# Da-Tsuchi/KLab_MultiModalModel

Hardware: AMD Instinct MI355X
Metric: caption-train samples/sec (224px img, 64-tok tgt) (higher is better)
Workload: dtype bf16; 1 GPU; BASELINE configs[1]: Swin-V2(C=64,(2,2,6,2),224,w7) frozen + T5-small, fwd+bwd+Adam, T5 dropout 0.1 on, random-init weights; global_batch=64, per_gpu_batch=64, src_len=9, tgt_len=64, parallelism=dp1, hipgraph=False, optimizer=klab.optim.FusedAdam (Adam update of ref/train.py:28, one kernel)

## Files before the change

include/klab_mm.h:

```cpp
#ifndef KLAB_MM_H
#define KLAB_MM_H
#include <stddef.h>
#include <stdint.h>

#ifdef __cplusplus
extern "C" {
#endif

#define KLAB_OK 0
#define KLAB_ERR_UNSUPPORTED (-2)
#define KLAB_ERR_BADARG (-3)

#define KLAB_F32 0
#define KLAB_BF16 1
#define KLAB_FP8 2

#define KLAB_ACT_NONE 0
#define KLAB_ACT_RELU 1
#define KLAB_ACT_GELU 2

#define KLAB_AUX_NONE 0
#define KLAB_AUX_NONZERO 1
#define KLAB_AUX_DGELU 2

// ... 77 lines not shown
int klab_t5_attn_fwd(const klab_attn_args* a, void* stream);
int klab_t5_attn_bwd(const klab_attn_args* a, void* stream);
typedef struct klab_attn_fused_args {
  const float* x; const float* gamma; float eps; int d_model;
  const void* w;
  void* xn; float* rstd;
  void* proj; long ldproj;
  int cross;
  klab_attn_args attn;
} klab_attn_fused_args;
int klab_t5_attn_fused_fwd(const klab_attn_fused_args* a, void* stream);
typedef struct klab_attn_bwd_fused_args {
  const void* dy; long lddy;
  const void* w;
  int d_model;
  klab_attn_args attn;
} klab_attn_bwd_fused_args;
int klab_t5_attn_bwd_fused(const klab_attn_bwd_fused_args* a, void* stream);
int klab_dbias_reduce(const void* ds_ws, int dtype, float* dbias, int nbatch, int H, int Lq, int Lk, void* stream);

typedef struct klab_swin_attn_args {
  int dtype;
  const void* qkv; void* ctx; const float* bias; const float* logit_scale; float* lse;
  int B, R, w, shift, H, C;
  const void* dctx; void* dqkv; float* dbias; float* dlogit_scale;
  void* bwd_ws; size_t bwd_ws_bytes;
  const float* bias_table; float* dbias_table;
  const float* v_bias; float* dv_bias;
} klab_swin_attn_args;
int klab_swin_attn_fwd(const klab_swin_attn_args* a, void* stream);
size_t klab_swin_attn_bwd_ws_bytes(int dtype, int B, int R, int w, int H, int C);
int klab_swin_qkv_attn_fused(const void* x, const void* wqkv, const float* bqkv, void* ctx, const float* bias, const float* logit_scale,
                             int dtype, int B, int R, int w, int shift, int H, int C, void* stream);
size_t klab_swin_bias_image_bytes(int w, int shift, int H);
int klab_swin_bias_image(const float* bias, float* image, int R, int w, int shift, int H, void* stream);
int klab_swin_qkv_attn_fused_img(const void* x, const void* wqkv, const float* bqkv, void* ctx, const float* image, const float* logit_scale,
                                 int dtype, int B, int R, int w, int shift, int H, int C, void* stream);
int klab_swin_attn_bwd(const klab_swin_attn_args* a, void* stream);
int klab_swin_cpb_bias(const float* coords, const int* index, const float* w0, const float* b0, const float* w2,
                       float* table, float* hidden, float* bias, int ntab, int n, int heads, int nhidden, void* stream);
int klab_swin_cpb_table(const float* coords, const float* w0, const float* b0, const float* w2, float* table, float* hidden,
                        float* bias_table, int ntab, int heads, int nhidden, void* stream);
int klab_swin_cpb_table_bwd(const float* dbias_table, const float* bias_table, const float* coords, const float* hidden, const float* w2,
                            float* dtable, float* dw0, float* db0, float* dw2, int ntab, int heads, int nhidden, void* stream);

typedef struct klab_image_desc { long long offset; int height, width; } klab_image_desc;
size_t klab_image_preprocess_ws_bytes(int n_images, int max_h, int mid);
int klab_image_preprocess(const unsigned char* src, const klab_image_desc* desc_dev, int n_images, int max_h, int max_w, int mid,
                          int out_size, int filter_a, int filter_b, double rescale, const float* mean3, const float* std3,
                          float* pixel_values, void* ws, size_t ws_bytes, void* stream);
#define KLAB_IMAGE_FLIP_LR 1
typedef struct klab_image_crop_desc { long long offset; int height, width, pitch, flags; } klab_image_crop_desc;
int klab_image_preprocess_crop(const unsigned char* src, const klab_image_crop_desc* desc_dev, int n_images, int max_crop_h,
                               int max_crop_w, int mid, int out_size, int filter_a, int filter_b, double rescale, const float* mean3,
                               const float* std3, float* pixel_values, void* ws, size_t ws_bytes, void* stream);

#define KLAB_JPEG_GRAY 0
#define KLAB_JPEG_YCC 1
#define KLAB_JPEG_RGB 2
typedef struct klab_jpeg_info {
  int width, height, ncomp, precision, progressive, supported, colour;
  int hmax, vmax, mcus_x, mcus_y;
  int hs[3], vs[3], bw[3], bh[3], tq[3];
  long long coef_blocks;
} klab_jpeg_info;
typedef struct klab_jpeg_item { klab_jpeg_info info; long long coef_block0; long long rgb_off; } klab_jpeg_item;
int klab_jpeg_read_info(const unsigned char* data, size_t n, klab_jpeg_info* info);
int klab_jpeg_entropy_decode(const unsigned char* data, size_t n, short* coefs, unsigned short* qt, klab_jpeg_info* info);
int klab_jpeg_entropy_decode_batch(const unsigned char* const* data, const size_t* sizes, int n, short* const* coefs,
                                   unsigned short* qt, klab_jpeg_info* infos, int* rcs, int n_threads);
size_t klab_jpeg_decode_ws_bytes(const klab_jpeg_item* items, int n);
int klab_jpeg_decode_device(const short* coefs_dev, const unsigned short* qt_dev, const klab_jpeg_item* items,
                            const klab_jpeg_item* items_dev, int n, unsigned char* rgb_dev, void* ws, size_t ws_bytes, void* stream);

int klab_cast_pack(const void* desc_dev, int ndesc, long total4, void* dst, int dtype, void* stream);
int klab_embed_fwd(const long long* ids, int shift_right, int L, int start_id, int pad_id, const float* table, int vocab,
                   float* out, int rows, int d, float drop_p, const uint32_t* seed_dev, uint32_t tag, int* err_flag,
                   void* stream);
int klab_embed_bwd(const long long* ids, int shift_right, int L, int start_id, int pad_id, const float* dh, float* dtable,
                   int vocab, int rows, int d, float drop_p, const uint32_t* seed_dev, uint32_t tag, void* stream);
int klab_relbias_fwd(const float* table, const int* bucket, float* bias, int heads, int Lq, int Lk, void* stream);
int klab_relbias_bwd(const float* dbias, const int* bucket, float* dtable, int heads, int Lq, int Lk, int nbuckets,
                     void* stream);
int klab_ce_count(const long long* labels, int rows, float* inv_n, void* stream);
int klab_ce_fwd(void* logits, long ld, int dtype, const long long* labels, int rows, int V, float* inv_n, float* loss_row,
                float* loss, int write_grad, void* stream);
int klab_ce_wsum(const long long* labels, const float* weights, int rows, float* inv_w, void* stream);
int klab_ce_fwd_opts(void* logits, long ld, int dtype, const long long* labels, const float* weights, int rows, int V, float eps, float z,
                     float* inv_w, float* loss_row, float* loss, int write_grad, void* stream);
int klab_im2col_patch(const float* pixels, void* out, int dtype, int B, int Cin, int Himg, int P, void* stream);
int klab_im2col_patch_ld(const float* pixels, void* out, int dtype, int B, int Cin, int Himg, int P, int ldo, void* stream);
int klab_merge_gather(const float* x, void* out, int dtype, int B, int R, int C, void* stream);
int klab_merge_scatter(const float* dmerged, float* dx, int B, int R, int C, void* stream);
int klab_colsum(const void* dy, long ld, int dtype, int M, int N, float* out, void* stream);
int klab_convert(const float* x, void* y, int dtype, long n, float scale, void* stream);
int klab_add_f32(float* y, const float* x, long n, void* stream);

int klab_gelu_fwd(const void* x, void* y, int dtype, long n, void* stream);
int klab_geglu_fwd(const void* ab, long ldab, void* h, long ldh, int dtype, int M, int F, float drop_p, const uint32_t* seed_dev,
                   uint32_t drop_tag, void* stream);
int klab_geglu_bwd(const void* dh, long lddh, const void* ab, long ldab, void* dab, long lddab, int dtype, int M, int F, float drop_p,
                   const uint32_t* seed_dev, uint32_t drop_tag, void* stream);
int klab_swin_proj_ln_fused(const void* x, const float* shortcut, const void* w, const float* b, const float* gamma, const float* beta,
                            float* out, void* outt, int dtype, int M, int C, float eps, void* stream);
int klab_swin_mlp_fused(const void* x, const float* shortcut, const void* w1, const float* b1, const void* w2, const float* b2,
                        const float* gamma, const float* beta, float* out, void* outt, int dtype, int M, int C, float eps,
                        void* stream);
int klab_swin_patch_embed_fused(const float* pixels, const void* w, int ldw, const float* bias, const float* gamma, const float* beta,
                                float* out, void* outt, int dtype, int B, int in_ch, int image_size, int patch, int C, float eps, void* stream);
int klab_swin_linear_ln_fused(const void* x, const float* shortcut, const void* w, const float* bias, const float* gamma,
                              const float* beta, float* out, void* outt, int dtype, int M, int K, int C, float eps, void* stream);
int klab_swin_cpb_bias_bwd(const float* dbias, const float* bias, const int* index, const float* coords, const float* hidden,
                           const float* w0, const float* w2, float* dtable, float* dw0, float* db0, float* dw2, int ntab, int n,
                           int heads, int nhidden, void* stream);
int klab_swin_cpb_bias_bwd_pz(const float* dbias, const float* bias, const int* index, const float* coords, const float* hidden,
                              const float* w0, const float* w2, float* dtable, float* dw0, float* db0, float* dw2, int ntab, int n,
                              int heads, int nhidden, int dtable_zeroed, void* stream);

typedef struct klab_swin_cfg {
  int image_size, patch, in_ch, embed_dim, n_stages;
  int depths[8], heads[8];
  int window;
  int pretrained_window[8];
  int mlp_ratio, qkv_bias;
  float ln_eps;
} klab_swin_cfg;
typedef struct klab_t5_cfg {
  int vocab, d_model, d_kv, n_heads, d_ff, n_layers, n_dec_layers, rel_buckets, rel_max_dist;
  float dropout, ln_eps;
  int start_id, pad_id, scale_decoder_outputs;
  int ffn_gated;
  int tie_lm_head;
} klab_t5_cfg;
typedef struct klab_model_cfg {
  klab_swin_cfg swin;
  klab_t5_cfg lang, main;
  int dtype;
  int train_swin;
} klab_model_cfg;
typedef struct klab_engine klab_engine;

int klab_sizeof_t5_cfg(void);
int klab_sizeof_model_cfg(void);
int klab_sizeof_sample_args(void);
int klab_sizeof_logits_proc_args(void);
int klab_sizeof_gen_cfg(void);
klab_engine* klab_engine_create(const klab_model_cfg* cfg);
void klab_engine_destroy(klab_engine* e);
int klab_engine_num_params(const klab_engine* e, int model);
int klab_engine_param_info(const klab_engine* e, int model, int i, char* name, int name_cap, long* shape4, int* ndim,
                           long* grad_off );
long klab_engine_grad_elems(const klab_engine* e, int model);
int klab_engine_num_buckets(const klab_engine* e, int segment);
int klab_engine_bucket(const klab_engine* e, int segment, int i, long* off, long* len);
int klab_engine_bucket_wait(klab_engine* e, int segment, int i, void* stream);
int klab_engine_set_bucket_events(klab_engine* e, int on);
int klab_engine_segment(const klab_engine* e, int seg, int* model, long* off, long* len);
int klab_engine_set_captions(klab_engine* e, int n);
size_t klab_engine_workspace_bytes(klab_engine* e, int B, int Ls, int Lt);
size_t klab_engine_workspace_bytes_n(klab_engine* e, int B, int Ls, int Lt, int n);
int klab_engine_bind(klab_engine* e, int B, int Ls, int Lt, void* workspace, size_t ws_bytes, const void* const* swin_params,
                     const void* const* lang_params, const void* const* main_params, float* main_grads, float* swin_grads,
                     const int* lang_bucket, const int* enc_bucket, const int* dec_bucket, const void* const* swin_coords,
                     const void* const* swin_index, void* stream);
int klab_engine_forward(klab_engine* e, const float* pixels, const long long* src_ids, const long long* tgt_ids, int training,
                        uint32_t seed, int want_grad, void* stream);
int klab_engine_set_graph(klab_engine* e, int on);
int klab_engine_get_rng(klab_engine* e, uint32_t* base, uint32_t* counter, void* stream);
int klab_engine_set_rng(klab_engine* e, uint32_t base, uint32_t counter, void* stream);
int klab_engine_adam_step(klab_engine* e, float* m, float* v, float lr, float beta1, float beta2, float eps, float weight_decay,
                          float bias_corr1, float bias_corr2, void* stream);
int klab_adam_step(const void* desc_dev, int ndesc, long total4, const float* grads, float* m, float* v, void* arena, int dtype, float lr,
// ... 149 lines not shown
```

klab_multimodalmodel_amd/_lib.py:

```python
import ctypes as C
import os

HERE = os.path.dirname(os.path.abspath(__file__))
LIB_PATH = os.environ.get("KLAB_LIB", os.path.join(HERE, "libklab_mm.so"))

F32, BF16, FP8 = 0, 1, 2
ACT_NONE, ACT_RELU, ACT_GELU = 0, 1, 2
AUX_NONE, AUX_NONZERO, AUX_DGELU = 0, 1, 2
ERR_UNSUPPORTED, ERR_BADARG = -2, -3

vp, i32, i64, f32, u32 = C.c_void_p, C.c_int, C.c_long, C.c_float, C.c_uint32


class GemmArgs(C.Structure):
    _fields_ = [("M", i32), ("N", i32), ("K", i32), ("dtype", i32),
                ("A", vp), ("lda", i64), ("a_kmajor", i32),
                ("B", vp), ("ldb", i64), ("b_kmajor", i32),
                ("C", vp), ("ldc", i64), ("c_dtype", i32), ("accumulate", i32),
                ("alpha", f32), ("alpha_dev", vp), ("bias", vp), ("act", i32),
                ("aux", vp), ("ldaux", i64), ("aux_mode", i32), ("aux_scale", f32),
                ("residual", vp), ("ldr", i64), ("r_dtype", i32),
                ("drop_p", f32), ("seed_dev", vp), ("drop_tag", u32), ("name_tag", i32), ("atomic_ok", i32)]


# ... 80 lines not shown
GEN_PICK, GEN_SAMPLE, GEN_BEAM, GEN_FORCE = 0, 1, 2, 3


class GenCfg(C.Structure):
    _fields_ = [("mode", i32), ("n", i32), ("max_length", i32), ("eos_id", i32), ("pad_id", i32),
                ("temperature", f32), ("top_k", i32), ("top_p", f32), ("seed", C.c_uint64),
                ("length_penalty", f32), ("early_stopping", i32), ("procs", C.POINTER(LogitsProcCfg)), ("want_logprobs", i32)]


SIGNATURES = {
    "klab_version": [],
    "klab_gemm": [C.POINTER(GemmArgs), vp],
    "klab_gemm_probe_enable": [i32],
    "klab_gemm_probe_read": [vp, vp, vp],
    "klab_rmsnorm_fwd": [vp, vp, vp, i32, vp, vp, i32, i32, f32, i32, i32, i32, f32, vp, u32, vp],
    "klab_rmsnorm_bwd": [vp, vp, vp, vp, vp, vp, vp, i32, vp, i32, i32, i32, i32, i32, f32, u32, f32, u32, vp, vp],
    "klab_rmsnorm_bwd_part": [vp, vp, vp, vp, vp, vp, vp, i32, vp, i32, i32, i32, i32, i32, f32, u32, f32, u32, vp, vp],
    "klab_rmsnorm_part_rows": [i32],
    "klab_colpart_reduce": [vp, i64, i32, i32, vp, i32, vp],
    "klab_adam_step": [vp, i32, i64, vp, vp, vp, vp, i32, f32, f32, f32, f32, f32, f32, f32, vp],
    "klab_adam_step_range": [vp, i32, i64, i64, vp, vp, vp, vp, i32, f32, f32, f32, f32, f32, f32, f32, vp],
    "klab_adamw_step_range": [vp, i32, vp, C.POINTER(AdamWGroup), i32, i64, i64, vp, vp, vp, vp, i32, vp],
    "klab_ema_update_range": [vp, i32, i64, i64, vp, f32, vp],
    "klab_ema_swap_range": [vp, i32, i64, i64, vp, vp, i32, vp],
    "klab_adafactor_plan": [i32, vp, vp, vp, vp, vp],
    "klab_adafactor_step": [vp, i32, i64, i64, vp, vp, vp, vp, vp, vp, i32, f32, f32, f32, f32, f32, f32, f32, f32, f32, i32, vp],
    "klab_grad_norm_chunk": [],
    "klab_grad_norm": [vp, i32, i32, vp, i64, vp, vp],
    "klab_grad_clip": [vp, i32, vp, f32, vp, vp],
    "klab_layernorm_fwd": [vp, i32, vp, vp, vp, vp, vp, i32, vp, vp, i32, i32, f32, i32, i32, i32, f32, vp, u32, vp],
    "klab_layernorm_bwd": [vp, vp, i32, vp, vp, vp, vp, vp, vp, i32, i32, i32, i32, i32, f32, vp, u32, vp],
    "klab_rmsnorm_fwd_q8": [vp, vp, vp, vp, vp, vp, i32, i32, f32, f32, vp, u32, vp],
    "klab_layernorm_fwd_q8": [vp, vp, vp, vp, vp, vp, vp, vp, vp, vp, i32, i32, f32, vp],
    "klab_gelu_fwd": [vp, vp, i32, i64, vp],
    "klab_gelu_fwd_q8": [vp, vp, vp, vp, i32, i32, vp],
    "klab_geglu_fwd": [vp, i64, vp, i64, i32, i32, i32, f32, vp, u32, vp],
    "klab_geglu_bwd": [vp, i64, vp, i64, vp, i64, i32, i32, i32, f32, vp, u32, vp],
    "klab_layernorm_bwd_bias": [vp, vp, i32, vp, vp, vp, vp, vp, vp, vp, i32, i32, i32, i32, i32, f32, vp, u32, vp],
    "klab_t5_attn_fwd": [C.POINTER(AttnArgs), vp],
    "klab_t5_attn_bwd": [C.POINTER(AttnArgs), vp],
    "klab_t5_attn_fused_fwd": [C.POINTER(AttnFusedArgs), vp],
    "klab_t5_attn_bwd_fused": [C.POINTER(AttnBwdFusedArgs), vp],
    "klab_t5_beam_decode_attn": [i32, vp, i64, vp, vp, i64, i64, i32, vp, i64, vp, i64, vp, i64, i32, i32, i32, i32, vp],
    "klab_t5_decode_attn_map": [i32, vp, i64, i32, vp, i64, i64, i32, vp, i64, vp, vp, i64, i32, i32, i32, i32, vp],
    "klab_beam_topk": [i32, vp, i64, i32, vp, i32, i32, i32, vp, vp, vp, vp, vp],
    "klab_beam_update": [C.POINTER(BeamUpdateArgs), i32, vp],
    "klab_beam_init": [C.POINTER(BeamUpdateArgs), i32, i32, vp],
    "klab_beam_copy_rows": [i32, vp, i64, i32, vp, i64, i32, i32, vp],
    "klab_sample_rows": [C.POINTER(SampleArgs), vp],
    "klab_logits_process_rows": [C.POINTER(LogitsProcArgs), vp],
    "klab_gen_finalize": [vp, i64, vp, i64, i32, i32, i32, i32, f32, i32, vp, vp, vp, vp],
    "klab_sizeof_sample_args": [],
    "klab_sizeof_logits_proc_args": [],
    "klab_sizeof_gen_cfg": [],
    "klab_force_rows": [C.POINTER(ForceArgs), vp],
    "klab_sizeof_force_args": [],
    "klab_beam_topk_scores": [vp, i64, i32, vp, i32, i32, i32, vp, vp, vp, vp, vp],
    "klab_dbias_reduce": [vp, i32, vp, i32, i32, i32, i32, vp],
    "klab_swin_mlp_fused": [vp, vp, vp, vp, vp, vp, vp, vp, vp, vp, i32, i32, i32, f32, vp],
    "klab_gemm_grouped": [vp, i32, vp],
    "klab_gemm_grouped_tiles": [vp, i32, i32, vp],
    "klab_gemm_fp8": [C.POINTER(GemmArgs), vp, vp, i64, vp],
    "klab_quant_fp8_rows": [vp, i64, i32, i32, vp, i64, vp, vp],
    "klab_quant_fp8_arena": [vp, i32, i64, vp, vp, vp, vp],
    "klab_swin_qkv_attn_fused": [vp, vp, vp, vp, vp, vp, i32, i32, i32, i32, i32, i32, i32, vp],
    "klab_swin_bias_image_bytes": [i32, i32, i32],
    "klab_swin_bias_image": [vp, vp, i32, i32, i32, i32, vp],
    "klab_swin_qkv_attn_fused_img": [vp, vp, vp, vp, vp, vp, i32, i32, i32, i32, i32, i32, i32, vp],
    "klab_swin_linear_ln_fused": [vp, vp, vp, vp, vp, vp, vp, vp, i32, i32, i32, i32, f32, vp],
    "klab_swin_patch_embed_fused": [vp, vp, i32, vp, vp, vp, vp, vp, i32, i32, i32, i32, i32, i32, f32, vp],
    "klab_swin_proj_ln_fused": [vp, vp, vp, vp, vp, vp, vp, vp, i32, i32, i32, f32, vp],
    "klab_swin_attn_fwd": [C.POINTER(SwinAttnArgs), vp],
    "klab_swin_attn_bwd": [C.POINTER(SwinAttnArgs), vp],
    "klab_swin_attn_bwd_ws_bytes": [i32, i32, i32, i32, i32, i32],
    "klab_swin_cpb_bias": [vp, vp, vp, vp, vp, vp, vp, vp, i32, i32, i32, i32, vp],
    "klab_swin_cpb_table": [vp, vp, vp, vp, vp, vp, vp, i32, i32, i32, vp],
    "klab_swin_cpb_table_bwd": [vp, vp, vp, vp, vp, vp, vp, vp, vp, i32, i32, i32, vp],
    "klab_swin_cpb_bias_bwd_pz": [vp, vp, vp, vp, vp, vp, vp, vp, vp, vp, vp, i32, i32, i32, i32, i32, vp],
    "klab_cast_pack": [vp, i32, i64, vp, i32, vp],
    "klab_embed_fwd": [vp, i32, i32, i32, i32, vp, i32, vp, i32, i32, f32, vp, u32, vp, vp],
    "klab_embed_bwd": [vp, i32, i32, i32, i32, vp, vp, i32, i32, i32, f32, vp, u32, vp],
    "klab_relbias_fwd": [vp, vp, vp, i32, i32, i32, vp],
    "klab_relbias_bwd": [vp, vp, vp, i32, i32, i32, i32, vp],
    "klab_ce_fwd": [vp, i64, i32, vp, i32, i32, vp, vp, vp, i32, vp],
    "klab_ce_count": [vp, i32, vp, vp],
    "klab_ce_wsum": [vp, vp, i32, vp, vp],
    "klab_ce_fwd_opts": [vp, i64, i32, vp, vp, i32, i32, f32, f32, vp, vp, vp, i32, vp],
    "klab_engine_set_loss_options": [vp, f32, f32, vp],
    "klab_engine_set_captions": [vp, i32],
    "klab_im2col_patch": [vp, vp, i32, i32, i32, i32, i32, vp],
    "klab_im2col_patch_ld": [vp, vp, i32, i32, i32, i32, i32, i32, vp],
    "klab_merge_gather": [vp, vp, i32, i32, i32, i32, vp],
    "klab_merge_scatter": [vp, vp, i32, i32, i32, vp],
    "klab_colsum": [vp, i64, i32, i32, i32, vp, vp],
    "klab_convert": [vp, vp, i32, i64, f32, vp],
    "klab_add_f32": [vp, vp, i64, vp],
    "klab_image_preprocess_ws_bytes": [i32, i32, i32],
    "klab_segv_trace_install": [i32],
    "klab_segv_set_context": [C.c_char_p],
    "klab_image_preprocess": [vp, vp, i32, i32, i32, i32, i32, i32, i32, C.c_double, vp, vp, vp, vp, C.c_size_t, vp],
    "klab_image_preprocess_crop": [vp, vp, i32, i32, i32, i32, i32, i32, i32, C.c_double, vp, vp, vp, vp, C.c_size_t, vp],
    "klab_jpeg_read_info": [vp, C.c_size_t, vp],
    "klab_jpeg_entropy_decode": [vp, C.c_size_t, vp, vp, vp],
    "klab_jpeg_entropy_decode_batch": [vp, vp, i32, vp, vp, vp, vp, i32],
    "klab_jpeg_decode_ws_bytes": [vp, i32],
    "klab_jpeg_decode_device": [vp, vp, vp, vp, i32, vp, vp, C.c_size_t, vp],
}


class JpegInfo(C.Structure):
    _fields_ = [("width", i32), ("height", i32), ("ncomp", i32), ("precision", i32), ("progressive", i32), ("supported", i32),
                ("colour", i32), ("hmax", i32), ("vmax", i32), ("mcus_x", i32), ("mcus_y", i32), ("hs", i32 * 3), ("vs", i32 * 3),
                ("bw", i32 * 3), ("bh", i32 * 3), ("tq", i32 * 3), ("coef_blocks", C.c_longlong)]


class JpegItem(C.Structure):
    _fields_ = [("info", JpegInfo), ("coef_block0", C.c_longlong), ("rgb_off", C.c_longlong)]

_lib = None


class KlabError(RuntimeError):
    pass


def load():
    global _lib
    if _lib is not None:
        return _lib
    if not os.path.exists(LIB_PATH):
        raise KlabError(f"{LIB_PATH} is missing: run `python -m klab_multimodalmodel_amd.build` "
                        "(hipcc --offload-arch=gfx950). There is no CPU fallback.")
    import torch
    lib = C.CDLL(LIB_PATH)
    for name, argt in SIGNATURES.items():
        fn = getattr(lib, name)
        fn.argtypes = argt
        fn.restype = C.c_size_t if name.endswith("_bytes") else i32
    _lib = lib
    return lib


def check(rc, what=""):
    if rc == 0:
        return
    if rc == ERR_UNSUPPORTED:
        raise NotImplementedError(f"klab: unsupported shape/alignment in {what}")
    if rc == ERR_BADARG:
        raise ValueError(f"klab: bad argument to {what}")
    raise KlabError(f"klab: {what} failed with hipError {rc}")


def ptr(t):
    return None if t is None else t.data_ptr()


def dtype_code(torch_dtype):
    import torch
    if torch_dtype == torch.float32:
        return F32
    if torch_dtype == torch.bfloat16:
        return BF16
    if torch_dtype == "fp8":
        return FP8
    raise ValueError(f"unsupported dtype {torch_dtype}")


def stream_ptr():
    import torch
    return torch.cuda.current_stream().cuda_stream
# ... 1 lines not shown
```

klab_multimodalmodel_amd/csrc/ce_opts.hip:

```cpp
#include <math.h>

#include "common.h"
#include "klab_mm.h"

namespace klab {
namespace {

struct CeOpts {
  float ome;
  float epsv;
  float z;
};

__global__ __launch_bounds__(256) void ce_wsum_kernel(const long long* __restrict__ labels, const float* __restrict__ weights, int rows,
                                                      float* __restrict__ inv_w) {
  __shared__ float red[4];
  float a = 0.f;
  for (int i = threadIdx.x; i < rows; i += 256) a += labels[i] != -100 ? (weights ? weights[i] : 1.f) : 0.f;
  a = wave_sum(a);
  if ((threadIdx.x & 63) == 0) red[threadIdx.x >> 6] = a;
  __syncthreads();
  if (threadIdx.x == 0) {
    const float W = red[0] + red[1] + red[2] + red[3];
    inv_w[0] = W > 0.f ? 1.f / W : 0.f;
  }
}

__device__ __forceinline__ float row_loss(float lse, float xlab, float sx, const CeOpts& o) {
  float l = lse - o.ome * xlab;
  l -= o.epsv * sx;
  l += (o.z * lse) * lse;
  return l;
}

struct GradCoef {
  float gk, ge, k, g;
};
__device__ __forceinline__ GradCoef grad_coef(float lse, float g, const CeOpts& o) {
  const float k = 1.f + 2.f * (o.z * lse);
  return GradCoef{g * k, g * o.epsv, k, g};
}
__device__ __forceinline__ float grad_at_label(float pr, const GradCoef& q, const CeOpts& o) {
  float t = pr * q.k - o.ome;
  t -= o.epsv;
  return t * q.g;
}

template <typename T, bool SX>
__global__ __launch_bounds__(256) void ce_opts_kernel(T* __restrict__ logits, long ld, const long long* __restrict__ labels,
                                                      const float* __restrict__ weights, int V, CeOpts o, const float* __restrict__ inv_w,
                                                      float* __restrict__ loss_row, int write_grad) {
  constexpr int VEC = Vec16<T>::N;
  using VT = typename Vec16<T>::type;
  __shared__ float red[12];
  const long row = blockIdx.x;
  const int tid = threadIdx.x;
  T* x = logits + row * ld;
  const long long lab = labels[row];
  const bool valid = lab != -100;
  const float g = write_grad && valid ? (weights ? weights[row] : 1.f) * inv_w[0] : 0.f;
  float m = -INFINITY, s = 0.f, sx = 0.f;
  for (int c = tid * VEC; c < V; c += 256 * VEC) {
    VT v = *reinterpret_cast<const VT*>(x + c);
    float mx = to_f32(v[0]);
#pragma unroll
    for (int u = 1; u < VEC; ++u) mx = fmaxf(mx, to_f32(v[u]));
    const float mn = fmaxf(m, mx);
    float a = 0.f;
#pragma unroll
    for (int u = 0; u < VEC; ++u) {
      a += __expf(to_f32(v[u]) - mn);
      if constexpr (SX) sx += to_f32(v[u]);
    }
    s = s * __expf(m - mn) + a;
    m = mn;
  }
  float wm = wave_max(m);
  float ws = wave_sum(m == -INFINITY ? 0.f : s * __expf(m - wm));
  const float wx = SX ? wave_sum(sx) : 0.f;
  if ((tid & 63) == 0) { red[tid >> 6] = wm; red[4 + (tid >> 6)] = ws; red[8 + (tid >> 6)] = wx; }
  __syncthreads();
  const float bm = fmaxf(fmaxf(red[0], red[1]), fmaxf(red[2], red[3]));
  float bs = 0.f;
#pragma unroll
  for (int w = 0; w < 4; ++w) bs += red[w] == -INFINITY ? 0.f : red[4 + w] * __expf(red[w] - bm);
  const float lse = bm + __logf(bs);
  const float bsx = red[8] + red[9] + red[10] + red[11];
  if (tid == 0) loss_row[row] = valid ? row_loss(lse, to_f32(x[lab]), bsx, o) : 0.f;
  if (!write_grad) return;
  __syncthreads();
  const GradCoef q = grad_coef(lse, g, o);
  const int labi = (int)lab;
  for (int c = tid * VEC; c < V; c += 256 * VEC) {
    VT v = *reinterpret_cast<const VT*>(x + c);
    VT out;
#pragma unroll
    for (int u = 0; u < VEC; ++u) out[u] = from_f32<T>(__expf(to_f32(v[u]) - lse) * q.gk - q.ge);
    const unsigned at = (unsigned)(labi - c);
    if (at < (unsigned)VEC) {
#pragma unroll
      for (int u = 0; u < VEC; ++u)
        if (u == (int)at) out[u] = from_f32<T>(grad_at_label(__expf(to_f32(v[u]) - lse), q, o));
    }
    *reinterpret_cast<VT*>(x + c) = out;
  }
}

template <typename T, int NIT, bool SX>
__global__ __launch_bounds__(256) void ce_opts_onepass_kernel(T* __restrict__ logits, long ld, const long long* __restrict__ labels,
                                                              const float* __restrict__ weights, int V, CeOpts o,
                                                              const float* __restrict__ inv_w, float* __restrict__ loss_row, int write_grad) {
  constexpr int VEC = Vec16<T>::N;
  using VT = typename Vec16<T>::type;
  __shared__ float red[12];
  __shared__ float xlab;
  const long row = blockIdx.x;
  const int tid = threadIdx.x;
  T* x = logits + row * ld;
  const long long lab = labels[row];
  const int labi = (int)lab;
  const bool valid = lab != -100;
  VT v[NIT];
#pragma unroll
  for (int it = 0; it < NIT; ++it) {
    const int c = (it * 256 + tid) * VEC;
    if (c < V) v[it] = *reinterpret_cast<const VT*>(x + c);
  }
  const float g = write_grad && valid ? (weights ? weights[row] : 1.f) * inv_w[0] : 0.f;
  float m = -INFINITY;
#pragma unroll
  for (int it = 0; it < NIT; ++it) {
    const int c = (it * 256 + tid) * VEC;
    if (c < V) {
#pragma unroll
      for (int u = 0; u < VEC; ++u) m = fmaxf(m, to_f32(v[it][u]));
    }
  }
  const float wm = wave_max(m);
  if ((tid & 63) == 0) red[tid >> 6] = wm;
  __syncthreads();
  const float bm = fmaxf(fmaxf(red[0], red[1]), fmaxf(red[2], red[3]));
  float sum = 0.f, sx = 0.f;
#pragma unroll
  for (int it = 0; it < NIT; ++it) {
    const int c = (it * 256 + tid) * VEC;
    if (c < V) {
#pragma unroll
      for (int u = 0; u < VEC; ++u) {
        const float xv = to_f32(v[it][u]);
        sum += __expf(xv - bm);
        if constexpr (SX) sx += xv;
      }
      const unsigned at = (unsigned)(labi - c);
      if (at < (unsigned)VEC) {
#pragma unroll
        for (int u = 0; u < VEC; ++u)
          if (u == (int)at) xlab = to_f32(v[it][u]);
      }
    }
  }
  const float ws = wave_sum(sum);
  const float wx = SX ? wave_sum(sx) : 0.f;
  if ((tid & 63) == 0) { red[4 + (tid >> 6)] = ws; red[8 + (tid >> 6)] = wx; }
  __syncthreads();
  const float lse = bm + __logf(red[4] + red[5] + red[6] + red[7]);
  const float bsx = red[8] + red[9] + red[10] + red[11];
  if (tid == 0) loss_row[row] = valid ? row_loss(lse, xlab, bsx, o) : 0.f;
  if (!write_grad) return;
  const GradCoef q = grad_coef(lse, g, o);
#pragma unroll
  for (int it = 0; it < NIT; ++it) {
    const int c = (it * 256 + tid) * VEC;
    if (c < V) {
      VT out;
#pragma unroll
      for (int u = 0; u < VEC; ++u) out[u] = from_f32<T>(__expf(to_f32(v[it][u]) - lse) * q.gk - q.ge);
      const unsigned at = (unsigned)(labi - c);
      if (at < (unsigned)VEC) {
#pragma unroll
        for (int u = 0; u < VEC; ++u)
          if (u == (int)at) out[u] = from_f32<T>(grad_at_label(__expf(to_f32(v[it][u]) - lse), q, o));
      }
      *reinterpret_cast<VT*>(x + c) = out;
    }
  }
}

__global__ __launch_bounds__(256) void ce_wreduce_kernel(const float* __restrict__ loss_row, const float* __restrict__ weights, int rows,
                                                         const float* __restrict__ inv_w, float* __restrict__ loss) {
  __shared__ float red[4];
  float a = 0.f;
  for (int i = threadIdx.x; i < rows; i += 256) a += weights ? weights[i] * loss_row[i] : loss_row[i];
  a = wave_sum(a);
  if ((threadIdx.x & 63) == 0) red[threadIdx.x >> 6] = a;
  __syncthreads();
  if (threadIdx.x == 0) loss[0] = (red[0] + red[1] + red[2] + red[3]) * inv_w[0];
}

template <bool SX>
void launch_rows(void* logits, long ld, int dtype, const long long* labels, const float* weights, int rows, int V, const CeOpts& o,
                 const float* inv_w, float* loss_row, int write_grad, hipStream_t s) {
  if (dtype == KLAB_BF16 && V <= 256 * 8 * 16 && V > 256 * 8 * 8)
    hipLaunchKernelGGL((ce_opts_onepass_kernel<bf16_t, 16, SX>), dim3(rows), dim3(256), 0, s, (bf16_t*)logits, ld, labels, weights, V, o, inv_w, loss_row, write_grad);
  else if (dtype == KLAB_BF16 && V <= 256 * 8 * 8)
    hipLaunchKernelGGL((ce_opts_onepass_kernel<bf16_t, 8, SX>), dim3(rows), dim3(256), 0, s, (bf16_t*)logits, ld, labels, weights, V, o, inv_w, loss_row, write_grad);
  else if (dtype == KLAB_BF16)
    hipLaunchKernelGGL((ce_opts_kernel<bf16_t, SX>), dim3(rows), dim3(256), 0, s, (bf16_t*)logits, ld, labels, weights, V, o, inv_w, loss_row, write_grad);
  else
    hipLaunchKernelGGL((ce_opts_kernel<float, SX>), dim3(rows), dim3(256), 0, s, (float*)logits, ld, labels, weights, V, o, inv_w, loss_row, write_grad);
}

}
}

using namespace klab;

extern "C" int klab_ce_wsum(const long long* labels, const float* weights, int rows, float* inv_w, void* stream) {
  if (!labels || !inv_w || rows <= 0) return KLAB_ERR_BADARG;
  hipLaunchKernelGGL(ce_wsum_kernel, dim3(1), dim3(256), 0, (hipStream_t)stream, labels, weights, rows, inv_w);
  KLAB_LAUNCH_CHECK();
  return KLAB_OK;
}

extern "C" int klab_ce_fwd_opts(void* logits, long ld, int dtype, const long long* labels, const float* weights, int rows, int V, float eps,
                                float z, float* inv_w, float* loss_row, float* loss, int write_grad, void* stream) {
  if (!logits || !labels || !inv_w || !loss_row || !loss || rows <= 0 || V <= 0) return KLAB_ERR_BADARG;
  if (!(eps >= 0.f && eps < 1.f) || !(z >= 0.f) || !isfinite(z)) return KLAB_ERR_BADARG;
  const int vec = dtype == KLAB_BF16 ? 8 : 4;
  if (V % vec || ld % vec) return KLAB_ERR_UNSUPPORTED;
  hipStream_t s = (hipStream_t)stream;
  if (!(write_grad & 2)) {
    hipLaunchKernelGGL(ce_wsum_kernel, dim3(1), dim3(256), 0, s, labels, weights, rows, inv_w);
    KLAB_LAUNCH_CHECK();
  }
  write_grad &= 1;
  const CeOpts o{1.f - eps, eps / (float)V, z};
  if (eps != 0.f) launch_rows<true>(logits, ld, dtype, labels, weights, rows, V, o, inv_w, loss_row, write_grad, s);
  else launch_rows<false>(logits, ld, dtype, labels, weights, rows, V, o, inv_w, loss_row, write_grad, s);
  KLAB_LAUNCH_CHECK();
  hipLaunchKernelGGL(ce_wreduce_kernel, dim3(1), dim3(256), 0, s, loss_row, weights, rows, inv_w, loss);
  KLAB_LAUNCH_CHECK();
  return KLAB_OK;
}
```

klab_multimodalmodel_amd/csrc/common.h:

```cpp
#pragma once
#include <hip/hip_runtime.h>
#include <stdint.h>
#include <stdlib.h>

#define KLAB_OK 0
#define KLAB_ERR_UNSUPPORTED (-2)
#define KLAB_ERR_BADARG (-3)

#define KLAB_F32 0
#define KLAB_BF16 1

typedef __bf16 bf16_t;
typedef __attribute__((ext_vector_type(8))) __bf16 bf16x8;
typedef __attribute__((ext_vector_type(4))) __bf16 bf16x4;
typedef __attribute__((ext_vector_type(4))) float f32x4;

#define KLAB_LAUNCH_CHECK()                          \
  do {                                               \
    hipError_t e__ = hipGetLastError();              \
    if (e__ != hipSuccess) return (int)e__;          \
  } while (0)

namespace klab {

inline bool env_on(const char* name) {
  const char* v = getenv(name);
  return !v || atoi(v) != 0;
}

int ensure_dyn_lds(const void* kernel, size_t bytes);

constexpr int ZERO_RANGES_MAX = 16;
int zero_ranges(float* const* ptrs, const long* counts, int n, hipStream_t s);

template <typename T> struct TypeTag;
template <> struct TypeTag<float> { static constexpr int id = KLAB_F32; };
template <> struct TypeTag<bf16_t> { static constexpr int id = KLAB_BF16; };

__device__ __forceinline__ float to_f32(float x) { return x; }
__device__ __forceinline__ float to_f32(bf16_t x) { return (float)x; }
template <typename T> __device__ __forceinline__ T from_f32(float x);
template <> __device__ __forceinline__ float from_f32<float>(float x) { return x; }
template <> __device__ __forceinline__ bf16_t from_f32<bf16_t>(float x) { return (bf16_t)x; }

__device__ __forceinline__ uint32_t mix32(uint32_t x) {
  x ^= x >> 16; x *= 0x85EBCA6Bu; x ^= x >> 13; x *= 0xC2B2AE35u; x ^= x >> 16;
  return x;
}
struct DropCtx {
  uint32_t key;
  uint32_t thresh;
  float scale;
  bool on;
};
__device__ __forceinline__ DropCtx make_drop(const uint32_t* seed_dev, uint32_t tag, float p) {
  DropCtx d;
  d.on = (p > 0.f) && (seed_dev != nullptr);
  d.key = 0; d.thresh = 0; d.scale = 1.f;
  if (d.on) {
    d.key = mix32(seed_dev[0] * 0x9E3779B1u + tag * 0x7FEB352Du + 0x165667B1u);
    double t = (double)p * 4294967296.0;
    d.thresh = t >= 4294967295.0 ? 0xFFFFFFFFu : (uint32_t)t;
    d.scale = 1.f / (1.f - p);
  }
  return d;
}
__device__ __forceinline__ float drop_mult(const DropCtx& d, uint64_t idx) {
  if (!d.on) return 1.f;
  uint32_t h = mix32((uint32_t)idx * 0x9E3779B1u + d.key);
  const uint32_t hi = (uint32_t)(idx >> 32);
  if (hi) h = mix32(h ^ (hi * 0x85EBCA77u + 0x27D4EB2Fu));
  return h < d.thresh ? 0.f : d.scale;
}
__device__ __forceinline__ DropCtx drop_slab(DropCtx d, uint32_t slab) {
  if (d.on) d.key = mix32(d.key ^ (slab * 0x85EBCA77u + 0x27D4EB2Fu));
  return d;
}
__device__ __forceinline__ float drop_mult32(const DropCtx& d, uint32_t off) {
  if (!d.on) return 1.f;
  return mix32(off * 0x9E3779B1u + d.key) < d.thresh ? 0.f : d.scale;
}
__device__ __forceinline__ float drop_mult32_nb(const DropCtx& d, uint32_t off) {
  return mix32(off * 0x9E3779B1u + d.key) < d.thresh ? 0.f : d.scale;
}

__device__ __forceinline__ float wave_sum(float v) {
#pragma unroll
  for (int o = 32; o > 0; o >>= 1) v += __shfl_xor(v, o, 64);
  return v;
}
__device__ __forceinline__ float wave_max(float v) {
#pragma unroll
  for (int o = 32; o > 0; o >>= 1) v = fmaxf(v, __shfl_xor(v, o, 64));
  return v;
}
template <int G> __device__ __forceinline__ float group_sum(float v) {
#pragma unroll
  for (int o = G / 2; o > 0; o >>= 1) v += __shfl_xor(v, o, 64);
  return v;
}
template <int G> __device__ __forceinline__ float group_max(float v) {
#pragma unroll
  for (int o = G / 2; o > 0; o >>= 1) v = fmaxf(v, __shfl_xor(v, o, 64));
  return v;
}

__device__ __forceinline__ float gelu_erf(float x) { return 0.5f * x * (1.f + erff(x * 0.70710678118654752440f)); }
__device__ __forceinline__ float erf_fast(float x) {
  const float ax = fabsf(x);
  const float t = __frcp_rn(fmaf(0.3275911f, ax, 1.f));
  float pl = fmaf(1.061405429f, t, -1.453152027f);
  pl = fmaf(pl, t, 1.421413741f);
  pl = fmaf(pl, t, -0.284496736f);
  pl = fmaf(pl, t, 0.254829592f);
  const float y = 1.f - pl * t * __expf(-ax * ax);
  return copysignf(y, x);
}
typedef __attribute__((ext_vector_type(2))) float f32x2;
template <typename V> __device__ __forceinline__ V gelu_poly(V x) {
  V s = x * x;
  s = __builtin_elementwise_min(s, V(20.48f));
  V q = V(7.318504830e-11f);
  q = q * s + V(-7.769299870e-09f);
  q = q * s + V(3.614930506e-07f);
  q = q * s + V(-9.785327165e-06f);
  q = q * s + V(1.732400560e-04f);
  q = q * s + V(-2.146258019e-03f);
  q = q * s + V(1.943818480e-02f);
  q = q * s + V(-1.324543953e-01f);
  q = q * s + V(7.977233529e-01f);
  V e = __builtin_elementwise_max(__builtin_elementwise_min(x * q, V(1.f)), V(-1.f));
  const V hx = x * V(0.5f);
  return hx * e + hx;
}
template <typename T> __device__ __forceinline__ float gelu_for(float x) {
  if constexpr (sizeof(T) == 2) return gelu_poly<float>(x);
  else return gelu_erf(x);
}
__device__ __forceinline__ float gelu_erf_grad(float x) {
  float cdf = 0.5f * (1.f + erff(x * 0.70710678118654752440f));
  float pdf = 0.39894228040143267794f * __expf(-0.5f * x * x);
  return cdf + x * pdf;
}

template <typename T> struct Vec16;
template <> struct Vec16<float> { typedef f32x4 type; static constexpr int N = 4; };
template <> struct Vec16<bf16_t> { typedef bf16x8 type; static constexpr int N = 8; };

}
```

klab_multimodalmodel_amd/csrc/engine.cpp:

```cpp
#include <hip/hip_runtime.h>
#include <math.h>
#include <stdio.h>
#include <string.h>

#include <algorithm>
#include <string>
#include <utility>
#include <vector>

#include "gemm_shared.h"
#include "klab_mm.h"

namespace {

#define RC(x)                 \
  do {                        \
    int rc__ = (x);           \
    if (rc__ != 0) return rc__; \
  } while (0)

struct ParamInfo {
  std::string name;
  std::vector<long> shape;
  long numel = 0;
// ... 51 lines not shown
};
struct ForcedTable {
  const long long* tok = nullptr;
  long ld = 0;
  int n = 0;
};
struct AttnMaps {
  float* p = nullptr;
  size_t bytes = 0;
};
struct GenRun {
  klab_gen_cfg cfg{};
  ProcSet lp;
  ForcedTable forced;
  AttnMaps maps;
  int cur = 0;
};

}

struct klab_engine {
  klab_model_cfg cfg;
  std::vector<ParamInfo> P[3];
  SwinIdx si; T5Idx li, mi;
  long grad_elems[3] = {0, 0, 0};
  long seg_zero_off[3] = {0, 0, 0}, seg_zero_len[3] = {0, 0, 0};
  long seg_off[3] = {0, 0, 0}, seg_len[3] = {0, 0, 0};
  long warena_elems = 0, farena_elems = 0;
  long kvall_w_off = -1, kvall_g_off = -1;
  struct Bucket { long off, len; };
  std::vector<Bucket> buckets[3];
  std::vector<hipEvent_t> bucket_ev[3];
  bool bucket_ev_live[3] = {false, false, false};
  bool bucket_events_on = false;
  int pe_k0 = 0, pe_kp = 0;
  bool bound = false;
  int B = 0, Ls = 0, Lt = 0, Le = 0, Nimg = 0;
  int ncap_next = 1, ncap = 1, Bd = 0;
  size_t es = 4;
  std::vector<const float*> W[3];
  float* G[3] = {nullptr, nullptr, nullptr};
  void* warena = nullptr; float* farena = nullptr;
  bool fp8 = false;
  void* w8 = nullptr; float* wscale = nullptr; void* qdesc = nullptr; int n_qdesc = 0; long q_rows = 0;
  void* x8 = nullptr; float* xscale = nullptr; long x8_bytes = 0, xscale_rows = 0;
  void* x8s = nullptr; float* xscales = nullptr; long x8s_bytes = 0, xscales_rows = 0;
  const void* q8_src[2] = {nullptr, nullptr}; int q8_rows[2] = {0, 0}, q8_k[2] = {0, 0};
  void* cast_desc = nullptr; int n_cast = 0; long cast_total4 = 0;
  void* adam_desc = nullptr; int n_adam = 0; long adam_total4 = 0, adam_split4 = 0;
  std::vector<long> adam_ptrs; int n_adam_seg0 = 0;
  void* af_desc = nullptr; int n_af = 0; long af_totals[4] = {0, 0, 0, 0};
  float* rms_part = nullptr; long rms_part_stride = 0; float** rms_dst_dev[2] = {nullptr, nullptr}; int rms_ncalls[2] = {0, 0};
  void* cast_desc_frozen = nullptr; int n_cast_frozen = 0; long cast_total4_frozen = 0;
  bool frozen_valid = false;
  void* fcast_desc = nullptr; int n_fcast = 0; long fcast_total4 = 0;
  uint32_t* seed_dev = nullptr; int* err_dev = nullptr;
  const int *enc_bucket = nullptr, *dec_bucket = nullptr, *lang_bucket = nullptr;
  std::vector<const float*> swin_coords; std::vector<const int*> swin_index; std::vector<int> swin_ntab;
  T5StackBufs lang, enc, dec;
  GenRun gen;
  ForcedTable forced_armed;
  AttnMaps attn_armed;
  void* kv_all = nullptr; void* dkv_all = nullptr;
  void* logits = nullptr; float *loss_row = nullptr, *inv_n = nullptr, *loss = nullptr;
  float *dh_a = nullptr, *dh_b = nullptr, *dxn = nullptr, *denc = nullptr;
  void *dctx = nullptr, *ds_ws = nullptr;
  void* dh_ff = nullptr;
  std::vector<void*> dy_pool, dhmid_pool, dqkv_pool, dqc_pool;
  std::vector<hipEvent_t> evpool; int ev_next = 0;
  void *cols = nullptr, *pe_out = nullptr; float *pe_mean = nullptr, *pe_rstd = nullptr; float* x0 = nullptr; void* x0t = nullptr;
  std::vector<SwinStageBufs> sw;
  float *sw_fmean = nullptr, *sw_frstd = nullptr;
  float *sdh_a = nullptr, *sdh_b = nullptr, *sdm = nullptr; void *sdy = nullptr, *sdctx = nullptr, *sdqkv = nullptr, *sda = nullptr;
  void* sattn_ws = nullptr; size_t sattn_ws_bytes = 0;
  float *sdbias = nullptr, *sdtable = nullptr, *sdbtab = nullptr;
  long sdb_stride = 0, sdt_stride = 0; size_t sdz_bytes = 0;
  void *sdyA[2] = {nullptr, nullptr}, *sdyB[2] = {nullptr, nullptr}, *sdaP[2] = {nullptr, nullptr}, *sdqkvP[2] = {nullptr, nullptr};
  hipEvent_t swin_done_ev[2] = {nullptr, nullptr};
  hipStream_t side = nullptr; hipEvent_t ev_fork = nullptr, ev_join = nullptr;
  hipEvent_t ev_zero = nullptr;
  bool seg1_zeroed = false;
  bool dbias_zeroed[2] = {false, false};
  bool denc_in_dxn = false;
  float* loss_out = nullptr;
  float loss_eps = 0.f, loss_z = 0.f;
  const float* loss_w_armed = nullptr;
  float *loss_w_buf = nullptr, *inv_w = nullptr;
  bool bias_ready[3] = {false, false, false};
  bool dec_embed_ready = false;
  bool inv_n_ready = false;
  bool kv_wgrad_done = false;
  struct WritePlan {
    bool valid = false, graph = false, kv = false;
    bool head_store = false, any_store = false;
    std::vector<char> store[2];
    std::vector<std::pair<long, long>> stored;
    std::vector<std::pair<long, long>> clear[2];
  } wplan;
  hipStream_t own = nullptr; hipEvent_t ev_in = nullptr, ev_out = nullptr;
  bool use_graph = false;
  struct GraphSlot { hipGraphExec_t exec = nullptr; int uses = 0; bool failed = false; } gs[7];
  float* pixels_buf = nullptr; long long *src_buf = nullptr, *tgt_buf = nullptr; float* dloss_buf = nullptr;
  const float* pixels_cur = nullptr;
  uint32_t seed_base = 0; bool seed_set = false;
  bool probe_on = false;
  struct Probe { std::vector<hipEvent_t> a, b; std::vector<double> flops; int n = 0; } probe[2];
  float p_train = 0.f;
  const long long* last_tgt = nullptr;
};

namespace {

int add_param(std::vector<ParamInfo>& v, const std::string& name, std::vector<long> shape) {
  ParamInfo p;
  p.name = name; p.shape = shape; p.numel = 1;
  for (long s : shape) p.numel *= s;
  v.push_back(p);
  return (int)v.size() - 1;
}

void build_t5_params(const klab_t5_cfg& c, bool encoder_only, std::vector<ParamInfo>& v, T5Idx& ix) {
  const long d = c.d_model, inner = (long)c.n_heads * c.d_kv, ff = c.d_ff;
  ix.shared = add_param(v, "shared.weight", {c.vocab, d});
  ix.lm_head = (!encoder_only && !c.tie_lm_head) ? add_param(v, "lm_head.weight", {c.vocab, d}) : -1;
  ix.head = ix.lm_head >= 0 ? ix.lm_head : ix.shared;
  auto stack = [&](const char* pre, int nl, bool dec, std::vector<T5LayerIdx>& L, int& fin) {
    for (int i = 0; i < nl; ++i) {
      T5LayerIdx l;
      memset(&l, -1, sizeof(l));
      std::string bp = std::string(pre) + "block." + std::to_string(i) + ".";
      std::string ap = bp + "layer.0.SelfAttention.";
      l.q = add_param(v, ap + "q.weight", {inner, d});
      l.k = add_param(v, ap + "k.weight", {inner, d});
      l.v = add_param(v, ap + "v.weight", {inner, d});
      l.o = add_param(v, ap + "o.weight", {d, inner});
      if (i == 0) l.relb = add_param(v, ap + "relative_attention_bias.weight", {c.rel_buckets, c.n_heads});
      l.ln0 = add_param(v, bp + "layer.0.layer_norm.weight", {d});
      int li = 1;
      if (dec) {
        std::string cp = bp + "layer.1.EncDecAttention.";
        l.cq = add_param(v, cp + "q.weight", {inner, d});
        l.ck = add_param(v, cp + "k.weight", {inner, d});
        l.cv = add_param(v, cp + "v.weight", {inner, d});
        l.co = add_param(v, cp + "o.weight", {d, inner});
        l.ln1 = add_param(v, bp + "layer.1.layer_norm.weight", {d});
        li = 2;
      }
      std::string fp = bp + "layer." + std::to_string(li) + ".";
      if (c.ffn_gated) {
        l.wi = add_param(v, fp + "DenseReluDense.wi_0.weight", {ff, d});
        l.wi1 = add_param(v, fp + "DenseReluDense.wi_1.weight", {ff, d});
      } else {
        l.wi = add_param(v, fp + "DenseReluDense.wi.weight", {ff, d});
      }
      l.wo = add_param(v, fp + "DenseReluDense.wo.weight", {d, ff});
      l.ln2 = add_param(v, fp + "layer_norm.weight", {d});
      L.push_back(l);
    }
    fin = add_param(v, std::string(pre) + "final_layer_norm.weight", {d});
  };
  if (!encoder_only) stack("decoder.", c.n_dec_layers, true, ix.dec, ix.dec_final);
  stack("encoder.", c.n_layers, false, ix.enc, ix.enc_final);
}

void build_swin_params(const klab_swin_cfg& c, std::vector<ParamInfo>& v, SwinIdx& ix) {
  const long C0 = c.embed_dim;
// ... 732 lines not shown
        g.aux = b.hmid; g.ldaux = ff; g.aux_mode = KLAB_AUX_NONZERO; g.aux_scale = inv_keep;
        RC(klab_gemm(&g, c.ws()));
      }
      RC(wq.push(dhmid, ff, b.xn3, d, M, ff, d, G(l.wi), st));
      RC(linear_dgrad(c, dhmid, ff, M, ff, P[l.wi].warena_off, d, e->dxn, KLAB_F32));
    }
    {
      const uint32_t tprev = dec ? tag_of(stack_id, i, SITE_XOUT) : tag_of(stack_id, i, SITE_ATTN_OUT);
      dy = next_dy();
      RC(rms_bwd(e->dxn, s.h[j], W[l.ln2], b.rstd3, dh_cur, dh_oth, dy, l.ln2, 0.f, 0, p, tprev));
      float* t = dh_cur; dh_cur = dh_oth; dh_oth = t;
    }
    if (dec) {
      --j;
      void* dqc = e->dqc_pool[i];
      RC(wq.push(dy, d, b.ctx2, inner, M, d, inner, G(l.co), st));
      dctx_ready = false;
      klab_attn_args a;
      memset(&a, 0, sizeof(a));
      a.dtype = c.dt; a.q = b.qc; a.ldq = inner;
      a.k = eoff(c, (void*)kv_all, (long)i * 2 * inner); a.ldk = kv_ld;
      a.v = eoff(c, (void*)kv_all, (long)i * 2 * inner + inner); a.ldv = kv_ld;
      a.ctx = b.ctx2; a.ldo = inner; a.lse = b.lse2; a.B = B / qgrp; a.H = H; a.Lq = qgrp * Lq; a.Lk = Lkv; a.dk = dk;
      a.drop_p = p; a.seed_dev = e->seed_dev; a.drop_tag = tag_of(stack_id, i, SITE_XPROB);
      a.dctx = e->dctx; a.lddo = inner; a.dq = dqc; a.lddq = inner;
      a.dk_out = eoff(c, dkv_all, (long)i * 2 * inner); a.lddk = kv_ld;
      a.dv = eoff(c, dkv_all, (long)i * 2 * inner + inner); a.lddv = kv_ld;
      RC(attn_bwd(a, P[l.co].warena_off, qgrp == 1));
      if (kv_in_queue) {
        RC(wq.push(eoff(c, dkv_all, (long)i * 2 * inner), kv_ld, e->enc.out_t, d, (B / qgrp) * Lkv, 2 * inner, d, Gflat + e->kvall_g_off + (long)i * 2 * inner * d, st));
        e->kv_wgrad_done = true;
      }
      RC(wq.push(dqc, inner, b.xn2, d, M, inner, d, G(l.cq), st));
      RC(linear_dgrad(c, dqc, inner, M, inner, P[l.cq].warena_off, d, e->dxn, KLAB_F32));
      dy = next_dy();
      RC(rms_bwd(e->dxn, s.h[j], W[l.ln1], b.rstd2, dh_cur, dh_oth, dy, l.ln1, 0.f, 0, p, tag_of(stack_id, i, SITE_ATTN_OUT)));
      float* t = dh_cur; dh_cur = dh_oth; dh_oth = t;
    }
    --j;
    RC(wq.push(dy, d, b.ctx, inner, M, d, inner, G(l.o), st));
    dctx_ready = false;
    {
      klab_attn_args a;
      memset(&a, 0, sizeof(a));
      a.dtype = c.dt; a.q = b.qkv; a.ldq = 3 * inner; a.k = eoff(c, b.qkv, inner); a.ldk = 3 * inner;
      a.v = eoff(c, b.qkv, 2 * inner); a.ldv = 3 * inner; a.bias = s.bias; a.causal = dec ? 1 : 0;
      a.ctx = b.ctx; a.ldo = inner; a.lse = b.lse; a.B = B; a.H = H; a.Lq = Lq; a.Lk = Lq; a.dk = dk;
      a.drop_p = p; a.seed_dev = e->seed_dev; a.drop_tag = tag_of(stack_id, i, SITE_PROB);
      a.dctx = e->dctx; a.lddo = inner; a.dq = dqkv; a.lddq = 3 * inner;
      a.dk_out = eoff(c, dqkv, inner); a.lddk = 3 * inner; a.dv = eoff(c, dqkv, 2 * inner); a.lddv = 3 * inner;
      a.dbias = s.dbias;
      int arc = KLAB_ERR_UNSUPPORTED;
      if (c.dt == KLAB_BF16 && deferred == (int)L.size() - 1 - i) {
        a.ds_defer = 1;
        a.ds_ws = (char*)e->ds_ws + (size_t)deferred * B * H * Lq * ((Lq + 31) & ~31) * c.es;
        arc = attn_bwd(a, P[l.o].warena_off);
        if (arc == 0) ++deferred;
      }
      if (arc == KLAB_ERR_UNSUPPORTED) { a.ds_defer = 0; a.ds_ws = nullptr; arc = attn_bwd(a, P[l.o].warena_off); }
      RC(arc);
    }
    RC(wq.push(dqkv, 3 * inner, b.xn1, d, M, 3 * inner, d, G(l.q), st));
    RC(linear_dgrad(c, dqkv, 3 * inner, M, 3 * inner, P[l.q].warena_off, d, e->dxn, KLAB_F32));
    {
      const bool first = (i == 0);
      if (!first) dy = next_dy();
      RC(rms_bwd(e->dxn, s.h[j], W[l.ln0], b.rstd1, dh_cur, dh_oth, first ? nullptr : dy, l.ln0, 0.f, 0, first ? 0.f : p,
                 first ? 0u : tag_of(stack_id, i - 1, SITE_FFN_OUT)));
      float* t = dh_cur; dh_cur = dh_oth; dh_oth = t;
    }
    bool launched = false;
    RC(wq.flush(c, flush_at[i] != 0, &launched));
    pending_buckets.push_back((int)L.size() - 1 - i);
    if (launched) {
      const int seg = dec ? 0 : 1;
      for (int bi : pending_buckets)
        if (e->bucket_events_on && Gflat == e->G[2] && !e->use_graph && bi < (int)e->bucket_ev[seg].size())
          RC((int)hipEventRecord(e->bucket_ev[seg][bi], e->side));
      pending_buckets.clear();
      if (i == 0 && e->bucket_events_on && Gflat == e->G[2] && !e->use_graph && (int)L.size() - 1 < (int)e->bucket_ev[seg].size())
        e->bucket_ev_live[seg] = true;
    }
  }
  if (part_ok && rms_calls) {
    if (rms_calls != e->rms_ncalls[stk]) return KLAB_ERR_BADARG;
    RC(klab_colpart_reduce(e->rms_part, e->rms_part_stride, klab_rmsnorm_part_rows(M), d, e->rms_dst_dev[stk], rms_calls, c.ws()));
  }
  if (deferred) RC(klab_dbias_reduce(e->ds_ws, c.dt, s.dbias, deferred * B, H, Lq, Lq, c.ws()));
  RC(klab_relbias_bwd(s.dbias, s.bucket, G(L[0].relb), H, Lq, Lq, cfg.rel_buckets, c.ws()));
  *dh_out = dh_cur;
  return 0;
}

int swin_forward(const Ctx& c, const float* pixels, float p_in, bool refresh_bias) {
  klab_engine* e = c.e;
  const klab_swin_cfg& s = e->cfg.swin;
  const auto& P = e->P[0];
  const auto& W = e->W[0];
  const int B = e->B, R0 = s.image_size / s.patch, K0 = s.in_ch * s.patch * s.patch, C0 = s.embed_dim;
  const long M0 = (long)B * R0 * R0;
  const int Kp = e->pe_kp;
  (void)K0;
  static const bool fused_pe = klab::env_on("KLAB_SWIN_FUSED_EMBED");
  int perc = KLAB_ERR_UNSUPPORTED;
  if (!e->cfg.train_swin && fused_pe && !e->fp8 && Kp >= 64)
    perc = klab_swin_patch_embed_fused(pixels, woff(c, P[e->si.pew].warena_off), Kp, W[e->si.peb], W[e->si.penw], W[e->si.penb], e->x0, e->x0t, c.dt,
                                       B, s.in_ch, s.image_size, s.patch, C0, s.ln_eps, c.ws());
  if (perc != 0 && perc != KLAB_ERR_UNSUPPORTED) return perc;
  if (perc != 0) {
  RC(klab_im2col_patch_ld(pixels, e->cols, c.dt, B, s.in_ch, s.image_size, s.patch, Kp, c.ws()));
  {
    klab_gemm_args g = G0(c, (int)M0, C0, Kp, e->cols, Kp, 1, woff(c, P[e->si.pew].warena_off), Kp, 1, e->pe_out, C0, c.dt);
    g.bias = W[e->si.peb];
    RC(klab_gemm(&g, c.ws()));
  }
  RC(klab_layernorm_fwd(e->pe_out, c.dt, W[e->si.penw], W[e->si.penb], nullptr, e->x0, e->x0t, c.dt, e->pe_mean, e->pe_rstd, (int)M0, C0,
                        s.ln_eps, 0, 0, 0, 0.f, nullptr, 0, c.ws()));
  }
  float* x = e->x0;
  void* xt = e->x0t;
  long bias_off = 0;
  for (int st = 0; st < s.n_stages; ++st) {
    SwinStageBufs& sb = e->sw[st];
    for (size_t k = 0; k < sb.blk.size(); ++k) {
      SwinBlockBufs& q = sb.blk[k];
      const SwinBlockIdx& ix = e->si.st[st].blk[k];
      const int C = q.C, M = (int)q.M, F = s.mlp_ratio * C, n = q.w * q.w;
      q.x_in = x; q.xt_in = xt;
      if (refresh_bias) {
        if (q.btab)
          RC(klab_swin_cpb_table(e->swin_coords[st], W[ix.c0w], W[ix.c0b], W[ix.c2w], q.table, q.hidden, q.btab, e->swin_ntab[st], q.H, 512,
                                 c.ws()));
        else
          RC(klab_swin_cpb_bias(e->swin_coords[st], e->swin_index[st], W[ix.c0w], W[ix.c0b], W[ix.c2w], q.table, q.hidden, q.bias,
                                e->swin_ntab[st], n, q.H, 512, c.ws()));
        if (q.bimg) RC(klab_swin_bias_image(q.bias, q.bimg, q.R, q.w, q.shift, q.H, c.ws()));
      }
      const float* qkvb = ix.qb >= 0 ? e->farena + bias_off : nullptr;
      bias_off += 3 * C;
      int qrc = KLAB_ERR_UNSUPPORTED;
      if (q.bimg)
        qrc = klab_swin_qkv_attn_fused_img(xt, woff(c, P[ix.qw].warena_off), qkvb, q.ctx, q.bimg, W[ix.ls], c.dt, B, q.R, q.w, q.shift, q.H, C,
                                           c.ws());
      else if (!e->cfg.train_swin && q.bias)
        qrc = klab_swin_qkv_attn_fused(xt, woff(c, P[ix.qw].warena_off), qkvb, q.ctx, q.bias, W[ix.ls], c.dt, B, q.R, q.w, q.shift, q.H, C,
                                       c.ws());
      if (qrc != 0 && qrc != KLAB_ERR_UNSUPPORTED) return qrc;
      if (qrc != 0) {
        RC(linear_fwd(c, xt, M, C, P[ix.qw].warena_off, 3 * C, q.qkv, 3 * C, c.dt, qkvb));
        klab_swin_attn_args a;
        memset(&a, 0, sizeof(a));
        a.dtype = c.dt; a.qkv = q.qkv; a.ctx = q.ctx; a.bias = q.bias; a.bias_table = q.btab; a.logit_scale = W[ix.ls]; a.lse = q.lse;
        a.B = B; a.R = q.R; a.w = q.w; a.shift = q.shift; a.H = q.H; a.C = C;
        a.bwd_ws = e->sattn_ws; a.bwd_ws_bytes = e->sattn_ws_bytes;
        a.v_bias = qkvb ? qkvb + 2 * C : nullptr;
        RC(klab_swin_attn_fwd(&a, c.ws()));
      }
      int prc = KLAB_ERR_UNSUPPORTED;
      if (!e->cfg.train_swin)
        prc = klab_swin_proj_ln_fused(q.ctx, x, woff(c, P[ix.pw].warena_off), W[ix.pb], W[ix.ln1w], W[ix.ln1b], q.h1, q.h1t, c.dt, M, C, s.ln_eps,
                                      c.ws());
      if (prc != 0 && prc != KLAB_ERR_UNSUPPORTED) return prc;
      static const bool fused_lin_ln = klab::env_on("KLAB_SWIN_FUSED_LIN_LN");
      const bool wide_ln = !e->cfg.train_swin && !e->fp8 && fused_lin_ln;
      if (prc != 0 && wide_ln) {
        prc = klab_swin_linear_ln_fused(q.ctx, x, woff(c, P[ix.pw].warena_off), W[ix.pb], W[ix.ln1w], W[ix.ln1b], q.h1, q.h1t, c.dt, M, C, C,
                                        s.ln_eps, c.ws());
        if (prc != 0 && prc != KLAB_ERR_UNSUPPORTED) return prc;
      }
      if (prc != 0) {
        RC(linear_fwd(c, q.ctx, M, C, P[ix.pw].warena_off, C, q.po, C, c.dt, W[ix.pb]));
        RC(ln_fwd_for_linear(c, q.po, W[ix.ln1w], W[ix.ln1b], x, q.h1, q.h1t, q.mean1, q.rstd1, M, C, s.ln_eps));
// ... 153 lines not shown
}
extern "C" size_t klab_engine_workspace_bytes(klab_engine* e, int B, int Ls, int Lt) {
  return e ? klab_engine_workspace_bytes_n(e, B, Ls, Lt, e->ncap_next) : 0;
}

extern "C" int klab_engine_set_captions(klab_engine* e, int n) {
  if (!e || n < 1) return KLAB_ERR_BADARG;
  e->ncap_next = n;
  return KLAB_OK;
}

extern "C" int klab_engine_bind(klab_engine* e, int B, int Ls, int Lt, void* workspace, size_t ws_bytes, const void* const* swin_params,
                                const void* const* lang_params, const void* const* main_params, float* main_grads, float* swin_grads,
                                const int* lang_bucket, const int* enc_bucket, const int* dec_bucket, const void* const* swin_coords,
                                const void* const* swin_index, void* stream) {
  if (!e || !workspace || !swin_params || !lang_params || !main_params || !main_grads) return KLAB_ERR_BADARG;
  if (e->cfg.train_swin && !swin_grads) return KLAB_ERR_BADARG;
  uint32_t carry[3] = {0, 0, 0};
  bool carry_rng = false;
  if (e->bound) {
    e->bound = false;
    drain_engine(e);
    if (e->seed_set && e->seed_dev) carry_rng = hipMemcpy(carry, e->seed_dev, sizeof(carry), hipMemcpyDeviceToHost) == hipSuccess;
  }
  const size_t need = plan_workspace(e, workspace, B, Ls, Lt);
  e->ncap_next = 1;
  if (need > ws_bytes) return KLAB_ERR_BADARG;
  const void* const* src[3] = {swin_params, lang_params, main_params};
  for (int m = 0; m < 3; ++m) {
    e->W[m].resize(e->P[m].size());
    for (size_t i = 0; i < e->P[m].size(); ++i) {
      e->W[m][i] = (const float*)src[m][i];
      if (!e->W[m][i]) return KLAB_ERR_BADARG;
    }
  }
  e->G[0] = swin_grads; e->G[2] = main_grads;
  e->lang_bucket = lang_bucket; e->enc_bucket = enc_bucket; e->dec_bucket = dec_bucket;
  e->lang.bucket = lang_bucket; e->enc.bucket = enc_bucket; e->dec.bucket = dec_bucket;
  const klab_swin_cfg& s = e->cfg.swin;
  e->swin_coords.resize(s.n_stages); e->swin_index.resize(s.n_stages); e->swin_ntab.resize(s.n_stages);
  const int R0 = s.image_size / s.patch;
  for (int st = 0; st < s.n_stages; ++st) {
    e->swin_coords[st] = (const float*)swin_coords[st];
    e->swin_index[st] = (const int*)swin_index[st];
    const int R = R0 >> st, w = R < s.window ? R : s.window;
    if (w <= 0) return KLAB_ERR_UNSUPPORTED;
    e->swin_ntab[st] = (2 * w - 1) * (2 * w - 1);
  }
  hipStream_t hs = (hipStream_t)stream;
  for (int grp = 0; grp < 2; ++grp) {
    std::vector<long> d;
    long pre = 0; int n = 0;
    for (int m = 0; m < 3; ++m) {
      const bool frozen = (m == 1) || (m == 0 && !e->cfg.train_swin);
      if (frozen != (grp == 1)) continue;
      for (size_t i = 0; i < e->P[m].size(); ++i) {
        const ParamInfo& p = e->P[m][i];
        if (p.warena_off < 0) continue;
        if (p.numel % 4) return KLAB_ERR_UNSUPPORTED;
        if (m == 0 && (int)i == e->si.pew && e->pe_kp != e->pe_k0) {
          if (e->pe_k0 % 4) return KLAB_ERR_UNSUPPORTED;
          for (int r = 0; r < e->cfg.swin.embed_dim; ++r) {
            d.push_back((long)(e->W[m][i] + (long)r * e->pe_k0)); d.push_back(p.warena_off + (long)r * e->pe_kp); d.push_back(pre);
            pre += e->pe_k0 / 4; ++n;
          }
          continue;
        }
        d.push_back((long)e->W[m][i]); d.push_back(p.warena_off); d.push_back(pre);
        pre += p.numel / 4; ++n;
      }
    }
    const size_t grp_cap = e->P[0].size() + e->P[1].size() + e->P[2].size() + e->cfg.swin.embed_dim + 1;
    void* dst = grp == 0 ? e->cast_desc : (void*)((char*)e->cast_desc + sizeof(long) * 3 * grp_cap);
    if (grp == 1) { e->cast_desc_frozen = dst; e->n_cast_frozen = n; e->cast_total4_frozen = pre; }
    if (n == 0) { if (grp == 0) { e->n_cast = 0; e->cast_total4 = 0; } continue; }
    hipError_t er0 = hipMemcpyAsync(dst, d.data(), d.size() * sizeof(long), hipMemcpyHostToDevice, hs);
    if (er0 != hipSuccess) return (int)er0;
    er0 = hipStreamSynchronize(hs);
    if (er0 != hipSuccess) return (int)er0;
    if (grp == 1) continue;
    e->n_cast = n; e->cast_total4 = pre;
  }
  e->frozen_valid = false;
  e->seg1_zeroed = e->dbias_zeroed[0] = e->dbias_zeroed[1] = e->denc_in_dxn = false;
  e->bias_ready[0] = e->bias_ready[1] = e->bias_ready[2] = e->dec_embed_ready = e->inv_n_ready = e->kv_wgrad_done = false;
  e->wplan.valid = false;
  e->loss_out = nullptr;
  e->loss_w_armed = nullptr;
  e->forced_armed = ForcedTable();
  e->attn_armed = AttnMaps();
  e->gen.maps = AttnMaps();
  if (e->pe_kp != e->pe_k0)
    RC((int)hipMemsetAsync((char*)e->warena + (size_t)e->P[0][e->si.pew].warena_off * e->es, 0,
                           (size_t)e->cfg.swin.embed_dim * e->pe_kp * e->es, hs));
  {
    std::vector<long> d;
    long pre = 0; int n = 0;
    for (size_t i = 0; i < e->P[0].size(); ++i) {
      const ParamInfo& p = e->P[0][i];
      if (p.farena_off < 0) continue;
      if (p.numel % 4) return KLAB_ERR_UNSUPPORTED;
      d.push_back((long)e->W[0][i]); d.push_back(p.farena_off); d.push_back(pre);
      pre += p.numel / 4; ++n;
    }
    e->n_fcast = n; e->fcast_total4 = pre;
    RC((int)hipMemsetAsync(e->farena, 0, (size_t)e->farena_elems * 4, hs));
    if (n) {
      hipError_t er = hipMemcpyAsync(e->fcast_desc, d.data(), d.size() * sizeof(long), hipMemcpyHostToDevice, hs);
      if (er != hipSuccess) return (int)er;
      er = hipStreamSynchronize(hs);
      if (er != hipSuccess) return (int)er;
    }
  }
  if (e->fp8) {
    std::vector<long> d;
    long row0 = 0; int n = 0;
    for (int m = 0; m < 3; ++m)
      for (size_t i = 0; i < e->P[m].size(); ++i) {
        const ParamInfo& p = e->P[m][i];
        if (p.warena_off < 0 || p.shape.empty() || (m == 0 && (int)i == e->si.pew)) continue;
        const long rows = p.shape[0], K = p.numel / rows;
        if (!fp8_weight_ok(K) || (p.warena_off & 15)) continue;
        d.push_back(p.warena_off); d.push_back(rows); d.push_back(K); d.push_back(row0);
        row0 += rows; ++n;
      }
    e->n_qdesc = n; e->q_rows = row0;
    if (n) {
      hipError_t er = hipMemcpyAsync(e->qdesc, d.data(), d.size() * sizeof(long), hipMemcpyHostToDevice, hs);
      if (er != hipSuccess) return (int)er;
      er = hipStreamSynchronize(hs);
      if (er != hipSuccess) return (int)er;
    }
  }
  std::vector<long> adam_tab;
  {
    std::vector<long> d;
    long pre = 0; int n = 0;
    bool ok = true;
    for (int seg = 0; seg < 2 && ok; ++seg) {
      if (seg == 1) { e->adam_split4 = pre; e->n_adam_seg0 = n; }
      for (size_t i = 0; i < e->P[2].size(); ++i) {
        const ParamInfo& p = e->P[2][i];
        if (p.grad_off < 0 || (p.grad_off >= e->seg_off[1]) != (seg == 1)) continue;
        if (p.numel % 4 || (p.grad_off & 3) || (p.warena_off >= 0 && (p.warena_off & 3))) { ok = false; break; }
        d.push_back((long)e->W[2][i]); d.push_back(p.grad_off); d.push_back(p.warena_off); d.push_back(pre);
        pre += p.numel / 4; ++n;
      }
    }
    e->n_adam = ok ? n : 0; e->adam_total4 = pre;
    e->adam_ptrs.clear();
    for (int k = 0; k < e->n_adam; ++k) e->adam_ptrs.push_back(d[(size_t)k * 4]);
    if (e->n_adam) {
      hipError_t er = hipMemcpyAsync(e->adam_desc, d.data(), d.size() * sizeof(long), hipMemcpyHostToDevice, hs);
      if (er != hipSuccess) return (int)er;
    }
    adam_tab.swap(d);
  }
  {
    std::vector<long> rows, cols, idx;
    std::vector<int> fact;
    for (int seg = 0; seg < 2; ++seg)
      for (size_t i = 0; i < e->P[2].size(); ++i) {
        const ParamInfo& p = e->P[2][i];
        if (p.grad_off < 0 || (p.grad_off >= e->seg_off[1]) != (seg == 1)) continue;
        const long c = p.shape.empty() ? 1 : p.shape.back();
        fact.push_back(p.shape.size() >= 2); rows.push_back(p.shape.size() >= 2 ? p.numel / c : 1);
        cols.push_back(p.shape.size() >= 2 ? c : p.numel); idx.push_back((long)i);
      }
    const int n = (int)idx.size();
    std::vector<long> plan((size_t)n * 4), d;
    e->n_af = 0;
    if (e->n_adam == n && n > 0 && klab_adafactor_plan(n, rows.data(), cols.data(), fact.data(), plan.data(), e->af_totals) == KLAB_OK) {
      for (int k = 0; k < n; ++k) {
        const ParamInfo& p = e->P[2][idx[k]];
        const long v[10] = {(long)e->W[2][idx[k]], p.grad_off, p.warena_off, rows[k], cols[k], plan[k * 4 + 0], plan[k * 4 + 1],
                            plan[k * 4 + 2], plan[k * 4 + 3], (long)fact[k]};
        d.insert(d.end(), v, v + 10);
      }
      hipError_t er = hipMemcpyAsync(e->af_desc, d.data(), d.size() * sizeof(long), hipMemcpyHostToDevice, hs);
      if (er != hipSuccess) return (int)er;
      e->n_af = n;
    }
    if (e->n_adam) {
      hipError_t er = hipStreamSynchronize(hs);
      if (er != hipSuccess) return (int)er;
    }
  }
  for (int st = 0; st < 2; ++st) {
    const bool dec = st == 1;
    const auto& L = dec ? e->mi.dec : e->mi.enc;
    std::vector<float*> dst;
    float* Gm = e->G[2];
    dst.push_back(Gm + e->P[2][dec ? e->mi.dec_final : e->mi.enc_final].grad_off);
    for (int i = (int)L.size() - 1; i >= 0; --i) {
      dst.push_back(Gm + e->P[2][L[i].ln2].grad_off);
      if (dec) dst.push_back(Gm + e->P[2][L[i].ln1].grad_off);
      dst.push_back(Gm + e->P[2][L[i].ln0].grad_off);
    }
    e->rms_ncalls[st] = (int)dst.size();
    hipError_t er = hipMemcpyAsync(e->rms_dst_dev[st], dst.data(), dst.size() * sizeof(float*), hipMemcpyHostToDevice, hs);
    if (er != hipSuccess) return (int)er;
    er = hipStreamSynchronize(hs);
    if (er != hipSuccess) return (int)er;
  }
  RC((int)hipMemsetAsync(e->seed_dev, 0, 512, hs));
  for (auto& g : e->gs) {
    if (g.exec) hipGraphExecDestroy(g.exec);
    g = klab_engine::GraphSlot();
  }
  e->seed_set = false;
  if (carry_rng) {
    RC((int)hipMemcpyAsync(e->seed_dev, carry, sizeof(carry), hipMemcpyHostToDevice, hs));
    RC((int)hipStreamSynchronize(hs));
    e->seed_set = true;
  }
  if (!e->side) {
    RC((int)hipStreamCreateWithFlags(&e->side, hipStreamNonBlocking));
    RC((int)hipEventCreateWithFlags(&e->ev_fork, hipEventDisableTiming));
    RC((int)hipEventCreateWithFlags(&e->ev_join, hipEventDisableTiming));
    RC((int)hipEventCreateWithFlags(&e->ev_zero, hipEventDisableTiming));
    RC((int)hipStreamCreateWithFlags(&e->own, hipStreamNonBlocking));
    e->evpool.resize(256);
    for (auto& ev : e->evpool) RC((int)hipEventCreateWithFlags(&ev, hipEventDisableTiming));
    RC((int)hipEventCreateWithFlags(&e->ev_in, hipEventDisableTiming));
    RC((int)hipEventCreateWithFlags(&e->ev_out, hipEventDisableTiming));
    for (auto& ev : e->swin_done_ev) RC((int)hipEventCreateWithFlags(&ev, hipEventDisableTiming));
    for (int sg = 0; sg < 3; ++sg) {
      e->bucket_ev[sg].assign(e->buckets[sg].size(), nullptr);
      for (auto& ev : e->bucket_ev[sg]) RC((int)hipEventCreateWithFlags(&ev, hipEventDisableTiming));
    }
  }
  for (int sg = 0; sg < 3; ++sg) e->bucket_ev_live[sg] = false;
  e->bound = true;
  return 0;
}

namespace {

__global__ void seed_set_kernel(uint32_t* st, uint32_t base) { st[1] = base; st[2] = 0; }
__global__ void seed_restore_kernel(uint32_t* st, uint32_t base, uint32_t counter) { st[1] = base; st[2] = counter; }
__global__ void seed_step_kernel(uint32_t* st) {
  const uint32_t n = st[2] + 1;
  st[2] = n;
  uint32_t x = st[1] + 0x9E3779B1u * n;
  x ^= x >> 16; x *= 0x85EBCA6Bu; x ^= x >> 13; x *= 0xC2B2AE35u; x ^= x >> 16;
  st[0] = x;
}

inline hipStream_t enter_stream(klab_engine* e, hipStream_t caller, int& rc) {
  rc = 0;
  if (!e->use_graph || caller != nullptr) return caller;
  rc = (int)hipEventRecord(e->ev_in, caller);
  if (!rc) rc = (int)hipStreamWaitEvent(e->own, e->ev_in, 0);
  return e->own;
}
inline int leave_stream(klab_engine* e, hipStream_t caller, hipStream_t used) {
  if (used == caller) return 0;
  int rc = (int)hipEventRecord(e->ev_out, used);
  if (!rc) rc = (int)hipStreamWaitEvent(caller, e->ev_out, 0);
  return rc;
}

template <typename F>
int run_graphed(klab_engine* e, int slot, hipStream_t s, F body) {
  klab_engine::GraphSlot& g = e->gs[slot];
  if (!e->use_graph || g.failed) return body();
  if (g.exec) return (int)hipGraphLaunch(g.exec, s);
  if (g.uses++ == 0) return body();
  hipError_t er = hipStreamBeginCapture(s, hipStreamCaptureModeThreadLocal);
  if (er != hipSuccess) { g.failed = true; return body(); }
  const int rc = body();
  hipGraph_t graph = nullptr;
  er = hipStreamEndCapture(s, &graph);
  if (rc != 0 || er != hipSuccess || !graph) {
    if (graph) hipGraphDestroy(graph);
    g.failed = true;
    return rc != 0 ? rc : body();
  }
  er = hipGraphInstantiate(&g.exec, graph, nullptr, nullptr, 0);
  hipGraphDestroy(graph);
  if (er != hipSuccess) { g.exec = nullptr; g.failed = true; return body(); }
  return (int)hipGraphLaunch(g.exec, s);
}

int forward_part_a(klab_engine* e, hipStream_t stream, float p, bool refresh_frozen, bool trainable_current, bool encoder_current = false) {
  Ctx c{e, stream, e->cfg.dtype, e->es};
  const klab_model_cfg& cfg = e->cfg;
  const float* pixels = e->pixels_cur;
  const long long *src_ids = e->src_buf, *tgt_ids = e->tgt_buf;
  hipLaunchKernelGGL(seed_step_kernel, dim3(1), dim3(1), 0, c.s, e->seed_dev);
  if (e->n_cast && !trainable_current) RC(klab_cast_pack(e->cast_desc, e->n_cast, e->cast_total4, e->warena, c.dt, c.ws()));
  if (refresh_frozen || e->cfg.train_swin) {
    if (refresh_frozen && e->n_cast_frozen)
      RC(klab_cast_pack(e->cast_desc_frozen, e->n_cast_frozen, e->cast_total4_frozen, e->warena, c.dt, c.ws()));
    if (e->n_fcast) RC(klab_cast_pack(e->fcast_desc, e->n_fcast, e->fcast_total4, e->farena, KLAB_F32, c.ws()));
  }
  if (e->fp8 && e->n_qdesc) RC(klab_quant_fp8_arena(e->qdesc, e->n_qdesc, e->q_rows, e->warena, e->w8, e->wscale, c.ws()));
  const int B = e->B, Bd = e->Bd, d = cfg.main.d_model;
  if (!encoder_current) {
  RC((int)hipEventRecord(e->ev_fork, c.s));
  RC(swin_forward(c, pixels, p, refresh_frozen || e->cfg.train_swin));
  RC((int)hipStreamWaitEvent(e->side, e->ev_fork, 0));
  {
    Ctx cs{e, e->side, e->cfg.dtype, e->es};
    static const bool early = klab::env_on("KLAB_EARLY_SMALL");
    if (early && !e->use_graph) {
      const int H = cfg.main.n_heads;
      RC(klab_relbias_fwd(e->W[2][e->mi.enc[0].relb], e->enc.bucket, e->enc.bias, H, e->enc.Lseq, e->enc.Lseq, cs.ws()));
      RC(klab_relbias_fwd(e->W[2][e->mi.dec[0].relb], e->dec.bucket, e->dec.bias, H, e->dec.Lseq, e->dec.Lseq, cs.ws()));
      e->bias_ready[STACK_ENC] = e->bias_ready[STACK_DEC] = true;
      RC(klab_embed_fwd(tgt_ids, 1, e->Lt, cfg.main.start_id, cfg.main.pad_id, e->W[2][e->mi.shared], cfg.main.vocab, e->dec.h[0], Bd * e->Lt, d, p,
                        e->seed_dev, tag_of(STACK_DEC, 0, SITE_IN), e->err_dev, cs.ws()));
      e->dec_embed_ready = true;
      RC(klab_ce_count(tgt_ids, Bd * e->Lt, e->inv_n, cs.ws()));
      e->inv_n_ready = true;
    }
    RC(klab_embed_fwd(src_ids, 0, e->Ls, 0, 0, e->W[1][e->li.shared], cfg.lang.vocab, e->lang.h[0], B * e->Ls, d, 0.f, nullptr, 0, e->err_dev,
                      cs.ws()));
    RC(t5_stack_forward(cs, cfg.lang, e->P[1], e->W[1], e->li.enc, e->li.enc_final, e->lang, false, STACK_LANG, 0.f, B, nullptr, 0, 0,
                        e->enc.h[0], e->Ls, e->Le, e->Nimg, p));
    RC((int)hipEventRecord(e->ev_join, e->side));
  }
  RC((int)hipStreamWaitEvent(c.s, e->ev_join, 0));
  RC(t5_stack_forward(c, cfg.main, e->P[2], e->W[2], e->mi.enc, e->mi.enc_final, e->enc, false, STACK_ENC, p, B, nullptr, 0, 0, nullptr, 0, 0, 0,
                      p));
  }
  const int inner = cfg.main.n_heads * cfg.main.d_kv, nld = cfg.main.n_dec_layers;
  if (e->dec_embed_ready) e->dec_embed_ready = false;
  else RC(klab_embed_fwd(tgt_ids, 1, e->Lt, cfg.main.start_id, cfg.main.pad_id, e->W[2][e->mi.shared], cfg.main.vocab, e->dec.h[0], Bd * e->Lt, d, p,
                         e->seed_dev, tag_of(STACK_DEC, 0, SITE_IN), e->err_dev, c.ws()));
  if (!encoder_current)
    RC(linear_fwd(c, e->enc.out_t, B * e->Le, d, e->kvall_w_off, nld * 2 * inner, e->kv_all, (long)nld * 2 * inner, c.dt));
  RC(t5_stack_forward(c, cfg.main, e->P[2], e->W[2], e->mi.dec, e->mi.dec_final, e->dec, true, STACK_DEC, p, Bd, e->kv_all, e->Le,
                      (long)nld * 2 * inner, nullptr, 0, 0, 0, p, e->ncap));
  return 0;
}

}

extern "C" int klab_engine_adam_step(klab_engine* e, float* m, float* v, float lr, float beta1, float beta2, float eps, float weight_decay,
                                     float bias_corr1, float bias_corr2, void* stream) {
  if (!e || !e->bound || !m || !v || !e->G[2]) return KLAB_ERR_BADARG;
  if (!e->n_adam) return KLAB_ERR_UNSUPPORTED;
  return klab_adam_step(e->adam_desc, e->n_adam, e->adam_total4, e->G[2], m, v, e->warena, e->cfg.dtype, lr, beta1, beta2, eps, weight_decay,
                        bias_corr1, bias_corr2, stream);
}

extern "C" int klab_engine_adafactor_state_elems(klab_engine* e, long* state_elems, long* scalar_elems, long* scratch_elems) {
  if (!e || !state_elems || !scalar_elems || !scratch_elems) return KLAB_ERR_BADARG;
  if (!e->n_af) return KLAB_ERR_UNSUPPORTED;
  *state_elems = e->af_totals[0]; *scalar_elems = e->af_totals[3]; *scratch_elems = e->af_totals[2];
  return KLAB_OK;
}

extern "C" int klab_engine_adafactor_layout(klab_engine* e, int max_n, long* out) {
  if (!e || !out) return KLAB_ERR_BADARG;
  if (!e->n_af) return KLAB_ERR_UNSUPPORTED;
  if (max_n < e->n_af) return KLAB_ERR_BADARG;
  hipError_t er = hipMemcpy(out, e->af_desc, sizeof(long) * 10 * e->n_af, hipMemcpyDeviceToHost);
  return er != hipSuccess ? (int)er : e->n_af;
}

extern "C" int klab_engine_adafactor_step(klab_engine* e, float* state, float* m, float* scalars, float* scratch, float beta2t,
                                          float one_minus_beta2t, float eps0, float eps1, float rel_step, float clip_threshold, float beta1,
                                          float one_minus_beta1, float weight_decay, int scale_parameter, void* stream) {
  if (!e || !e->bound || !state || !scalars || !scratch || !e->G[2]) return KLAB_ERR_BADARG;
  if (!e->n_af) return KLAB_ERR_UNSUPPORTED;
  return klab_adafactor_step(e->af_desc, e->n_af, e->af_totals[0], e->af_totals[1], e->G[2], state, m, scalars, scratch, e->warena, e->cfg.dtype,
                             beta2t, one_minus_beta2t, eps0, eps1, rel_step, clip_threshold, beta1, one_minus_beta1, weight_decay, scale_parameter, stream);
}

extern "C" int klab_engine_adam_step_segment(klab_engine* e, int segment, float* m, float* v, float lr, float beta1, float beta2, float eps,
                                             float weight_decay, float bias_corr1, float bias_corr2, void* stream) {
  if (!e || !e->bound || !m || !v || !e->G[2] || segment < 0 || segment > 1) return KLAB_ERR_BADARG;
  if (!e->n_adam) return KLAB_ERR_UNSUPPORTED;
  const long b4 = segment == 0 ? 0 : e->adam_split4, e4 = segment == 0 ? e->adam_split4 : e->adam_total4;
  return klab_adam_step_range(e->adam_desc, e->n_adam, b4, e4, e->G[2], m, v, e->warena, e->cfg.dtype, lr, beta1, beta2, eps, weight_decay,
                              bias_corr1, bias_corr2, stream);
}

extern "C" int klab_engine_adam_layout(klab_engine* e, int max_n, long* param_ptrs, int* n_segment0) {
  if (!e || !e->bound || !param_ptrs || !n_segment0) return KLAB_ERR_BADARG;
  if (!e->n_adam) return KLAB_ERR_UNSUPPORTED;
  if (max_n < e->n_adam) return KLAB_ERR_BADARG;
  for (int k = 0; k < e->n_adam; ++k) param_ptrs[k] = e->adam_ptrs[k];
  *n_segment0 = e->n_adam_seg0;
  return e->n_adam;
}

extern "C" int klab_engine_adamw_step(klab_engine* e, int segment, float* m, float* v, const int* group_of_dev, const klab_adamw_group* groups,
                                      int ngroups, void* stream) {
  if (!e || !e->bound || !m || !v || !e->G[2] || segment < -1 || segment > 1) return KLAB_ERR_BADARG;
  if (!e->n_adam) return KLAB_ERR_UNSUPPORTED;
  const long b4 = segment == 1 ? e->adam_split4 : 0, e4 = segment == 0 ? e->adam_split4 : e->adam_total4;
  return klab_adamw_step_range(e->adam_desc, e->n_adam, group_of_dev, groups, ngroups, b4, e4, e->G[2], m, v, e->warena, e->cfg.dtype, stream);
}

extern "C" int klab_engine_ema_update(klab_engine* e, float* ema, float w, void* stream) {
  if (!e || !e->bound || !ema) return KLAB_ERR_BADARG;
  if (!e->n_adam) return KLAB_ERR_UNSUPPORTED;
  return klab_ema_update_range(e->adam_desc, e->n_adam, 0, e->adam_total4, ema, w, stream);
}

extern "C" int klab_engine_ema_swap(klab_engine* e, float* ema, void* stream) {
  if (!e || !e->bound || !ema) return KLAB_ERR_BADARG;
  if (!e->n_adam) return KLAB_ERR_UNSUPPORTED;
  return klab_ema_swap_range(e->adam_desc, e->n_adam, 0, e->adam_total4, ema, e->warena, e->cfg.dtype, stream);
}

extern "C" int klab_engine_get_rng(klab_engine* e, uint32_t* base, uint32_t* counter, void* stream) {
  if (!e || !e->bound || !base || !counter) return KLAB_ERR_BADARG;
  uint32_t st[3] = {0, 0, 0};
  RC((int)hipMemcpyAsync(st, e->seed_dev, sizeof(st), hipMemcpyDeviceToHost, (hipStream_t)stream));
  RC((int)hipStreamSynchronize((hipStream_t)stream));
  *base = e->seed_set ? st[1] : e->seed_base;
  *counter = e->seed_set ? st[2] : 0;
  return KLAB_OK;
}
extern "C" int klab_engine_set_rng(klab_engine* e, uint32_t base, uint32_t counter, void* stream) {
  if (!e || !e->bound) return KLAB_ERR_BADARG;
  hipLaunchKernelGGL(seed_restore_kernel, dim3(1), dim3(1), 0, (hipStream_t)stream, e->seed_dev, base, counter);
  e->seed_base = base; e->seed_set = true;
  return KLAB_OK;
}

extern "C" int klab_engine_set_graph(klab_engine* e, int on) {
  if (!e) return KLAB_ERR_BADARG;
  e->use_graph = on != 0;
  return 0;
}

extern "C" int klab_engine_forward(klab_engine* e, const float* pixels, const long long* src_ids, const long long* tgt_ids, int training,
                                   uint32_t seed, int want_grad, void* stream) {
  if (!e || !e->bound || !pixels || !src_ids || !tgt_ids) return KLAB_ERR_BADARG;
  int erc = 0;
  const hipStream_t xs = enter_stream(e, (hipStream_t)stream, erc);
  if (erc) return erc;
  Ctx c{e, xs, e->cfg.dtype, e->es};
  const klab_model_cfg& cfg = e->cfg;
  const float p = (training & 1) ? cfg.main.dropout : 0.f;
  const bool refresh_frozen = !((training & 2) && e->frozen_valid);
  e->p_train = p;
  e->last_tgt = e->tgt_buf;
  const int B = e->B, d = cfg.main.d_model;
  if (e->use_graph) {
    RC((int)hipMemcpyAsync(e->pixels_buf, pixels, (size_t)B * cfg.swin.in_ch * cfg.swin.image_size * cfg.swin.image_size * 4,
                           hipMemcpyDeviceToDevice, c.s));
    e->pixels_cur = e->pixels_buf;
  } else {
    e->pixels_cur = pixels;
  }
  RC((int)hipMemcpyAsync(e->src_buf, src_ids, (size_t)B * e->Ls * 8, hipMemcpyDeviceToDevice, c.s));
  RC((int)hipMemcpyAsync(e->tgt_buf, tgt_ids, (size_t)e->Bd * e->Lt * 8, hipMemcpyDeviceToDevice, c.s));
  const float* loss_w = nullptr;
  if (e->loss_w_armed) {
    const float* src_w = e->loss_w_armed;
    e->loss_w_armed = nullptr;
    RC((int)hipMemcpyAsync(e->loss_w_buf, src_w, (size_t)e->Bd * e->Lt * 4, hipMemcpyDeviceToDevice, c.s));
    loss_w = e->loss_w_buf;
  }
  if (!e->seed_set || seed != e->seed_base) {
    hipLaunchKernelGGL(seed_set_kernel, dim3(1), dim3(1), 0, c.s, e->seed_dev, seed);
    e->seed_base = seed; e->seed_set = true;
  }
  const bool tcur = (training & 4) && !e->use_graph;
  const bool ecur = (training & 8) && !(training & 1) && !want_grad && !e->use_graph && e->frozen_valid && !refresh_frozen;
  if (refresh_frozen) {
    RC(forward_part_a(e, c.s, p, true, tcur));
    e->frozen_valid = true;
  } else if (ecur) {
    RC(forward_part_a(e, c.s, p, false, true, true));
  } else {
    RC(run_graphed(e, (training & 1) ? 1 : 0, c.s, [&]() { return forward_part_a(e, c.s, p, false, tcur); }));
  }
  {
    const int Md = e->Bd * e->Lt, V = cfg.main.vocab;
    klab_gemm_args g = G0(c, Md, V, d, e->dec.out_t, d, 1, woff(c, e->P[2][e->mi.head].warena_off), d, 1, e->logits, V, c.dt);
    g.alpha = cfg.main.scale_decoder_outputs ? 1.f / sqrtf((float)d) : 1.f;
    g.name_tag = 1;
    klab_engine::Probe& pr = e->probe[0];
    const bool probe = e->probe_on && pr.n < (int)pr.a.size();
    if (probe) { klab::tl_launch_probe.a = pr.a[pr.n]; klab::tl_launch_probe.b = pr.b[pr.n]; }
    RC(fwd_gemm(c, g, e->P[2][e->mi.head].warena_off));
    if (probe) {
      if (klab::tl_launch_probe.a) klab::tl_launch_probe.a = nullptr;
      else pr.flops[pr.n++] = 2.0 * Md * (double)V * d;
    }
    const bool counted = e->inv_n_ready && !e->use_graph;
    e->inv_n_ready = false;
    float* loss_dst = e->loss_out && !e->use_graph ? e->loss_out : e->loss;
    e->loss_out = nullptr;
    if (!loss_w && e->loss_eps == 0.f && e->loss_z == 0.f) {
      RC(run_graphed(e, want_grad ? 3 : 2, c.s, [&]() {
        return klab_ce_fwd(e->logits, V, c.dt, e->tgt_buf, Md, V, e->inv_n, e->loss_row, loss_dst, (want_grad ? 1 : 0) | (counted ? 2 : 0), c.ws());
      }));
    } else {
      RC(klab_ce_wsum(e->tgt_buf, loss_w, Md, e->inv_w, c.ws()));
      RC(klab_ce_fwd_opts(e->logits, V, c.dt, e->tgt_buf, loss_w, Md, V, e->loss_eps, e->loss_z, e->inv_w, e->loss_row, loss_dst,
                          (want_grad ? 1 : 0) | 2, c.ws()));
    }
  }
  return leave_stream(e, (hipStream_t)stream, xs);
}

extern "C" int klab_engine_probe_enable(klab_engine* e, int on) {
  if (!e) return KLAB_ERR_BADARG;
  if (on && e->probe[0].a.empty()) {
    const size_t cap[2] = {1024, 16384};
    for (int ch = 0; ch < 2; ++ch) {
      klab_engine::Probe& pr = e->probe[ch];
      pr.a.assign(cap[ch], nullptr); pr.b.assign(cap[ch], nullptr); pr.flops.assign(cap[ch], 0.0);
      for (size_t i = 0; i < cap[ch]; ++i)
        if (hipEventCreate(&pr.a[i]) != hipSuccess || hipEventCreate(&pr.b[i]) != hipSuccess) return KLAB_ERR_UNSUPPORTED;
    }
  }
  e->probe_on = on != 0;
  if (on) for (auto& pr : e->probe) pr.n = 0;
  return 0;
}
extern "C" int klab_engine_probe_read(klab_engine* e, int channel, int* launches, float* total_ms, double* flops_total) {
  if (!e || channel < 0 || channel > 1) return KLAB_ERR_BADARG;
  klab_engine::Probe& pr = e->probe[channel];
  float tot = 0.f;
  double fl = 0;
  for (int i = 0; i < pr.n; ++i) {
    float ms = 0.f;
    hipError_t er = hipEventElapsedTime(&ms, pr.a[i], pr.b[i]);
    if (er != hipSuccess) return (int)er;
    tot += ms;
    fl += pr.flops[i];
  }
  if (launches) *launches = pr.n;
  if (total_ms) *total_ms = tot;
  if (flops_total) *flops_total = fl;
  return 0;
}
extern "C" const float* klab_engine_loss_ptr(const klab_engine* e) { return e ? e->loss : nullptr; }
extern "C" int klab_engine_set_loss_out(klab_engine* e, float* out) {
  if (!e) return KLAB_ERR_BADARG;
  e->loss_out = e->use_graph ? nullptr : out;
  return e->loss_out ? 1 : 0;
}
extern "C" int klab_engine_set_loss_options(klab_engine* e, float eps, float z, const float* weights) {
  if (!e || !(eps >= 0.f && eps < 1.f) || !(z >= 0.f) || !isfinite(z)) return KLAB_ERR_BADARG;
  if (weights && !e->bound) return KLAB_ERR_BADARG;
  e->loss_eps = eps; e->loss_z = z;
  e->loss_w_armed = weights;
  return KLAB_OK;
}
extern "C" const int* klab_engine_err_ptr(const klab_engine* e) { return e ? e->err_dev : nullptr; }
extern "C" const uint32_t* klab_engine_rng_ptr(const klab_engine* e) { return e ? e->seed_dev : nullptr; }

extern "C" const void* klab_engine_buffer(const klab_engine* e, const char* name, long* rows, long* cols, int* dtype) {
  if (!e || !e->bound || !name) return nullptr;
  const int d = e->cfg.main.d_model;
  auto set = [&](long r, long c2, int dt) { if (rows) *rows = r; if (cols) *cols = c2; if (dtype) *dtype = dt; };
  if (!strcmp(name, "encoder_input")) { set((long)e->B * e->Le, d, KLAB_F32); return e->enc.h[0]; }
  if (!strcmp(name, "encoder_out")) { set((long)e->B * e->Le, d, e->cfg.dtype); return e->enc.out_t; }
  if (!strcmp(name, "decoder_out")) { set((long)e->Bd * e->Lt, d, e->cfg.dtype); return e->dec.out_t; }
  if (!strcmp(name, "logits")) { set((long)e->Bd * e->Lt, e->cfg.main.vocab, e->cfg.dtype); return e->logits; }
  if (!strcmp(name, "loss_row")) { set((long)e->Bd * e->Lt, 1, KLAB_F32); return e->loss_row; }
  return nullptr;
}

namespace {
struct DecodeRows {
  int M;
  float* h[2]; float* rstd;
  void *xn, *q, *ctx, *hmid, *out, *logits;
  void* ab = nullptr;
  void* cache; long cache_layer; int cache_rows;
  int kv_group = 1; const int* kv_slot = nullptr; long slot_ld = 0;
  float* maps = nullptr; const int* done = nullptr;
};

int decode_rows(klab_engine* e, const Ctx& c, int t, const long long* tokens, const DecodeRows& r) {
  const klab_t5_cfg& cfg = e->cfg.main;
  const auto& P = e->P[2];
  const auto& W = e->W[2];
  const int M = r.M, Lt = e->Lt, Le = e->Le, d = cfg.d_model, H = cfg.n_heads, dk = cfg.d_kv, inner = H * dk, ff = cfg.d_ff;
  const int nld = cfg.n_dec_layers;
  const long kv_ld = (long)nld * 2 * inner;
// ... 393 lines not shown
  if (w.head_store) w.stored.push_back({P[e->mi.head].grad_off, (long)cfg.vocab * d});
  for (int stk = 0; stk < 2; ++stk) {
    const bool dec = stk == 1;
    const std::vector<T5LayerIdx>& L = dec ? e->mi.dec : e->mi.enc;
    const WgradRelease rel = wgrad_release_plan(e, cfg, (int)L.size(), dec, dec && e->dkv_all != nullptr, e->G[2]);
    w.store[stk] = rel.store;
    for (size_t i = 0; i < L.size(); ++i) {
      if (!rel.store[i]) continue;
      const T5LayerIdx& l = L[i];
      w.stored.push_back({P[l.wo].grad_off, d * ff});
      w.stored.push_back({P[l.wi].grad_off, (cfg.ffn_gated ? 2 * ff : ff) * d});
      w.stored.push_back({P[l.o].grad_off, d * inner});
      w.stored.push_back({P[l.q].grad_off, 3 * inner * d});
      if (dec) {
        w.stored.push_back({P[l.co].grad_off, d * inner});
        w.stored.push_back({P[l.cq].grad_off, inner * d});
        if (rel.kv_in_queue) w.stored.push_back({e->kvall_g_off + (long)i * 2 * inner * d, 2 * inner * d});
      }
    }
  }
  std::sort(w.stored.begin(), w.stored.end());
  w.any_store = !w.stored.empty();
  for (int seg = 0; seg < 2; ++seg) {
    const long end = e->seg_off[seg] + e->seg_len[seg];
    long cur = e->seg_off[seg];
    for (const auto& s : w.stored) {
      if (s.first + s.second <= cur || s.first >= end) continue;
      if (s.first > cur) w.clear[seg].push_back({cur, s.first - cur});
      cur = s.first + s.second;
    }
    if (cur < end) w.clear[seg].push_back({cur, end - cur});
  }
  w.valid = true;
}
static bool wgrad_write_plan_current(const klab_engine* e) {
  return e->wplan.valid && e->wplan.graph == e->use_graph && e->wplan.kv == (e->dkv_all != nullptr);
}
static int clear_planned(klab_engine* e, int seg_lo, int seg_hi, bool with_dbias, hipStream_t s) {
  std::vector<float*> zp;
  std::vector<long> zn;
  for (int seg = seg_lo; seg <= seg_hi; ++seg)
    for (const auto& r : e->wplan.clear[seg]) { zp.push_back(e->G[2] + r.first); zn.push_back(r.second); }
  if (with_dbias) {
    const long H = e->cfg.main.n_heads;
    zp.push_back((float*)e->dec.dbias); zn.push_back(H * e->Lt * e->Lt);
    zp.push_back((float*)e->enc.dbias); zn.push_back(H * e->Le * e->Le);
  }
  return klab::zero_ranges(zp.data(), zn.data(), (int)zp.size(), s);
}

static int backward_segment(klab_engine* e, int segment, const float* dloss_dev, void* stream) {
  Ctx c{e, (hipStream_t)stream, e->cfg.dtype, e->es};
  const klab_model_cfg& cfg = e->cfg;
  const int B = e->B, d = cfg.main.d_model, inner = cfg.main.n_heads * cfg.main.d_kv, nld = cfg.main.n_dec_layers;
  const float p = e->p_train;
  float* Gm = e->G[2];
  e->bucket_ev_live[segment] = false;
  if (segment == 0) {
    e->ev_next = 0;
    const int Md = e->Bd * e->Lt, V = cfg.main.vocab;
    const float alpha = cfg.main.scale_decoder_outputs ? 1.f / sqrtf((float)d) : 1.f;
    Ctx cs{e, e->side, c.dt, c.es};
    static const bool zero_side = klab::env_on("KLAB_ZERO_ON_SIDE");
    const bool zside = zero_side && !e->use_graph;
    if (!wgrad_write_plan_current(e)) wgrad_write_plan(e);
    const bool ranged = e->wplan.any_store;
    if (zside) {
      RC(side_after_main(c));
      if (ranged) RC(clear_planned(e, 0, 1, true, e->side));
      else {
        RC((int)hipMemsetAsync(Gm + e->seg_off[0], 0, (size_t)e->seg_len[0] * 4, e->side));
        RC((int)hipMemsetAsync(Gm + e->seg_off[1], 0, (size_t)e->seg_len[1] * 4, e->side));
        RC((int)hipMemsetAsync(e->dec.dbias, 0, (size_t)cfg.main.n_heads * e->Lt * e->Lt * 4, e->side));
        RC((int)hipMemsetAsync(e->enc.dbias, 0, (size_t)cfg.main.n_heads * e->Le * e->Le * 4, e->side));
      }
      RC((int)hipEventRecord(e->ev_zero, e->side));
      e->seg1_zeroed = e->dbias_zeroed[0] = e->dbias_zeroed[1] = true;
    } else if (ranged) {
      RC(clear_planned(e, 0, 0, false, c.s));
    } else {
      RC((int)hipMemsetAsync(Gm + e->seg_off[0], 0, (size_t)e->seg_len[0] * 4, c.s));
    }
    {
      RC((int)hipMemsetAsync(e->dxn, 0, (size_t)Md * d * 4, c.s));
      klab_gemm_args g = G0(c, Md, d, V, e->logits, V, 1, woff(c, e->P[2][e->mi.head].warena_off), d, 0, e->dxn, d, KLAB_F32);
      g.alpha = alpha; g.alpha_dev = dloss_dev; g.accumulate = 1; g.atomic_ok = 1;
      RC(klab_gemm(&g, c.ws()));
    }
    if (zside) RC((int)hipStreamWaitEvent(c.s, e->ev_zero, 0));
    RC(side_after_main(c));
    {
      klab_gemm_args g = G0(cs, V, d, Md, e->logits, V, 0, e->dec.out_t, d, 0, Gm + e->P[2][e->mi.head].grad_off, d, KLAB_F32);
      g.alpha = alpha; g.alpha_dev = dloss_dev; g.accumulate = e->wplan.head_store ? 0 : 1; g.atomic_ok = 1;
      RC(klab_gemm(&g, cs.ws()));
    }
    float* dh0 = nullptr;
    RC(t5_stack_backward(c, cfg.main, e->P[2], e->W[2], Gm, e->mi.dec, e->mi.dec_final, e->dec, true, STACK_DEC, p, e->Bd, e->kv_all, e->dkv_all,
                         e->Le, (long)nld * 2 * inner, &dh0, e->ncap));
    RC(side_after_main(c));
    RC(klab_embed_bwd(e->last_tgt, 1, e->Lt, cfg.main.start_id, cfg.main.pad_id, dh0, Gm + e->P[2][e->mi.shared].grad_off, V, Md, d, p,
                      e->seed_dev, tag_of(STACK_DEC, 0, SITE_IN), cs.ws()));
    const int Me = B * e->Le, Nkv = nld * 2 * inner;
    if (e->kv_wgrad_done) e->kv_wgrad_done = false;
    else RC(linear_wgrad(cs, e->dkv_all, Nkv, e->enc.out_t, d, Me, Nkv, d, Gm + e->kvall_g_off));
    e->denc_in_dxn = !e->use_graph;
    RC(linear_dgrad(c, e->dkv_all, Nkv, Me, Nkv, e->kvall_w_off, d, e->denc_in_dxn ? e->dxn : e->denc, KLAB_F32));
    return main_after_side(c);
  }
  if (segment == 1) {
    e->ev_next = 0;
    if (!wgrad_write_plan_current(e)) { wgrad_write_plan(e); e->seg1_zeroed = false; }
    if (e->seg1_zeroed) e->seg1_zeroed = false;
    else if (e->wplan.any_store) RC(clear_planned(e, 1, 1, false, c.s));
    else RC((int)hipMemsetAsync(Gm + e->seg_off[1], 0, (size_t)e->seg_len[1] * 4, c.s));
    const int Me = B * e->Le;
    if (e->denc_in_dxn) e->denc_in_dxn = false;
    else RC((int)hipMemcpyAsync(e->dxn, e->denc, (size_t)Me * d * 4, hipMemcpyDeviceToDevice, c.s));
    float* dh0 = nullptr;
    RC(t5_stack_backward(c, cfg.main, e->P[2], e->W[2], Gm, e->mi.enc, e->mi.enc_final, e->enc, false, STACK_ENC, p, B, nullptr, nullptr, 0, 0,
                         &dh0));
    if (cfg.train_swin) RC((int)hipMemcpyAsync(e->denc, dh0, (size_t)Me * d * 4, hipMemcpyDeviceToDevice, c.s));
    return main_after_side(c);
  }
  if (segment == 2) {
    if (!cfg.train_swin) return 0;
    return swin_backward(c, e->denc, p);
  }
  return KLAB_ERR_BADARG;
}


extern "C" int klab_engine_backward(klab_engine* e, int segment, const float* dloss_dev, void* stream) {
  if (!e || !e->bound || segment < 0 || segment > 2) return KLAB_ERR_BADARG;
  int erc = 0;
  const hipStream_t s = enter_stream(e, (hipStream_t)stream, erc);
  if (erc) return erc;
  const float* dl = e->dloss_buf;
  if (segment == 0) {
    if (dloss_dev && !e->use_graph) dl = dloss_dev;
    else if (dloss_dev) RC((int)hipMemcpyAsync(e->dloss_buf, dloss_dev, 4, hipMemcpyDeviceToDevice, s));
    else { static const float one = 1.f; RC((int)hipMemcpyAsync(e->dloss_buf, &one, 4, hipMemcpyHostToDevice, s)); }
  }
  RC(run_graphed(e, 4 + segment, s, [&]() { return backward_segment(e, segment, dl, (void*)s); }));
  return leave_stream(e, (hipStream_t)stream, s);
}

namespace {

int swin_backward(const Ctx& c, const float* dh0, float p_in) {
  klab_engine* e = c.e;
  const klab_swin_cfg& s = e->cfg.swin;
  const auto& P = e->P[0];
  const auto& W = e->W[0];
  float* Gs = e->G[0];
  auto G = [&](int pi) { return Gs + P[pi].grad_off; };
  const int B = e->B, R0 = s.image_size / s.patch, C0 = s.embed_dim;
  RC((int)hipMemsetAsync(Gs + e->seg_off[2], 0, (size_t)e->seg_len[2] * 4, c.s));
  RC((int)hipMemsetAsync(e->sdbias, 0, e->sdz_bytes, c.s));
  const int last = s.n_stages - 1;
  const int Cl = C0 << last;
  const SwinStageBufs& lsb = e->sw[last];
  const float* xlast = lsb.blk.empty() ? (last > 0 ? e->sw[last - 1].xm : e->x0) : lsb.blk.back().h2;
  float* dh = e->sdh_a;
  float* dh2 = e->sdh_b;
  RC(klab_layernorm_bwd(dh0, xlast, KLAB_F32, W[e->si.lnw], e->sw_fmean, e->sw_frstd, dh, G(e->si.lnw), G(e->si.lnb), B * e->Nimg, Cl,
                        e->Nimg, e->Le, 0, p_in, e->seed_dev, tag_of(STACK_ENC, 0, SITE_IN), c.ws()));
  long bias_off_total = 0;
  for (int st = 0; st < s.n_stages; ++st) bias_off_total += 3L * (C0 << st) * s.depths[st];
  long bias_off = bias_off_total;
  (void)bias_off;
  int swin_bucket = 0, blk_no = 0;
  const bool side_on = e->sdyA[0] != nullptr;
  const Ctx cs{e, e->side, c.dt, c.es};
  for (int st = last; st >= 0; --st) {
    SwinStageBufs& sb = e->sw[st];
    const int R = R0 >> st, C = C0 << st;
    if (st < last) {
      const long M2 = (long)B * (R / 2) * (R / 2);
      RC(klab_layernorm_bwd(dh, sb.mo, c.dt, W[e->si.st[st].mnw], sb.mmean, sb.mrstd, e->sdy, G(e->si.st[st].mnw), G(e->si.st[st].mnb), (int)M2,
                            2 * C, 0, 0, 0, 0.f, nullptr, 0, c.ws()));
      RC(linear_wgrad(c, e->sdy, 2 * C, sb.mg, 4 * C, (int)M2, 2 * C, 4 * C, G(e->si.st[st].redw)));
      RC(linear_dgrad(c, e->sdy, 2 * C, (int)M2, 2 * C, P[e->si.st[st].redw].warena_off, 4 * C, e->sdm, KLAB_F32));
      RC(klab_merge_scatter(e->sdm, dh2, B, R, C, c.ws()));
      float* t = dh; dh = dh2; dh2 = t;
    }
    for (int k = (int)sb.blk.size() - 1; k >= 0; --k) {
      SwinBlockBufs& q = sb.blk[k];
      const SwinBlockIdx& ix = e->si.st[st].blk[k];
      const int M = (int)q.M, F = s.mlp_ratio * C, n = q.w * q.w;
      const int par = blk_no & 1;
      if (side_on && blk_no >= 2) RC((int)hipStreamWaitEvent(c.s, e->swin_done_ev[par], 0));
      void* dyA = side_on ? e->sdyA[par] : e->sdy;
      void* dyB = side_on ? e->sdyB[par] : e->sdy;
// ... 91 lines not shown
```

klab_multimodalmodel_amd/csrc/misc.hip:

```cpp
#include <math.h>

#include <map>
#include <mutex>

#include "common.h"
#include "klab_mm.h"

namespace klab {

int ensure_dyn_lds(const void* kernel, size_t bytes) {
  static std::mutex mu;
  static std::map<const void*, size_t> set;
  if (bytes > 160 * 1024) return KLAB_ERR_UNSUPPORTED;
  std::lock_guard<std::mutex> g(mu);
  auto it = set.find(kernel);
  if (it != set.end() && it->second >= bytes) return KLAB_OK;
  hipError_t e = hipFuncSetAttribute(kernel, hipFuncAttributeMaxDynamicSharedMemorySize, (int)bytes);
  if (e != hipSuccess) return (int)e;
  set[kernel] = bytes;
  return KLAB_OK;
}

struct CastDesc { const float* src; long dst_off; long n4_prefix; };

// ... 75 lines not shown
    for (int u = 0; u < U; ++u)
      if (pp[u]) {
        f32x4 po, mo, vo;
#pragma unroll
        for (int i = 0; i < 4; ++i) {
          const float g = gv[u][i] + h.weight_decay * pv[u][i];
          mo[i] = mv[u][i] + (1.f - h.beta1) * (g - mv[u][i]);
          vo[i] = h.beta2 * vv[u][i] + (1.f - h.beta2) * g * g;
          const float denom = sqrtf(vo[i]) * h.inv_sqrt_bc2 + h.eps;
          po[i] = pv[u][i] - h.lr_over_bc1 * (mo[i] / denom);
        }
        __builtin_nontemporal_store(po, reinterpret_cast<f32x4*>(pp[u]));
        __builtin_nontemporal_store(mo, reinterpret_cast<f32x4*>(m + go[u]));
        __builtin_nontemporal_store(vo, reinterpret_cast<f32x4*>(v + go[u]));
        if (ao[u] >= 0) {
          if constexpr (sizeof(T) == 2) *reinterpret_cast<bf16x4*>(arena + ao[u]) = bf16x4{(bf16_t)po[0], (bf16_t)po[1], (bf16_t)po[2], (bf16_t)po[3]};
          else *reinterpret_cast<f32x4*>(arena + ao[u]) = po;
        }
      }
  }
}

__global__ __launch_bounds__(256) void embed_fwd_kernel(const long long* __restrict__ ids, int shift_right, int L, int start_id, int pad_id,
                                                        const float* __restrict__ table, int vocab, float* __restrict__ out, int rows, int d,
                                                        float p, const uint32_t* seed, uint32_t tag, int* __restrict__ err) {
  const int lane = threadIdx.x & 63;
  const DropCtx dc = make_drop(seed, tag, p);
  for (long row = (long)blockIdx.x * 4 + (threadIdx.x >> 6); row < rows; row += (long)gridDim.x * 4) {
    long long id;
    if (shift_right) {
      const int t = row % L;
      id = t == 0 ? start_id : ids[row - 1];
      if (id == -100) id = pad_id;
    } else {
      id = ids[row];
    }
    if (id < 0 || id >= vocab) { if (lane == 0 && err) atomicOr(err, 1); id = 0; }
    const float* src = table + id * d;
    for (int c = lane * 4; c < d; c += 256) {
      f32x4 v = *reinterpret_cast<const f32x4*>(src + c);
#pragma unroll
      for (int i = 0; i < 4; ++i) v[i] *= drop_mult(dc, (uint64_t)row * d + c + i);
      *reinterpret_cast<f32x4*>(out + row * d + c) = v;
    }
  }
}

__global__ __launch_bounds__(256) void embed_bwd_kernel(const long long* __restrict__ ids, int shift_right, int L, int start_id, int pad_id,
                                                        const float* __restrict__ dh, float* __restrict__ dtable, int vocab, int rows, int d,
                                                        float p, const uint32_t* seed, uint32_t tag) {
  const int lane = threadIdx.x & 63;
  const DropCtx dc = make_drop(seed, tag, p);
  for (long row = (long)blockIdx.x * 4 + (threadIdx.x >> 6); row < rows; row += (long)gridDim.x * 4) {
    long long id;
    if (shift_right) {
      const int t = row % L;
      id = t == 0 ? start_id : ids[row - 1];
      if (id == -100) id = pad_id;
    } else {
      id = ids[row];
    }
    if (id < 0 || id >= vocab) continue;
    float* dst = dtable + id * d;
    for (int c = lane; c < d; c += 64) atomicAdd(dst + c, dh[row * d + c] * drop_mult(dc, (uint64_t)row * d + c));
  }
}

__global__ void relbias_fwd_kernel(const float* __restrict__ table, const int* __restrict__ bucket, float* __restrict__ bias, int H, int LL) {
  const long idx = (long)blockIdx.x * blockDim.x + threadIdx.x;
  if (idx >= (long)H * LL) return;
  const int h = idx / LL, ij = idx % LL;
  bias[idx] = table[bucket[ij] * H + h];
}
__global__ void relbias_bwd_kernel(const float* __restrict__ dbias, const int* __restrict__ bucket, float* __restrict__ dtable, int H, int LL, int nb) {
  __shared__ float acc[64];
  const int h = blockIdx.x;
  for (int i = threadIdx.x; i < 64; i += blockDim.x) acc[i] = 0.f;
  __syncthreads();
  for (int ij = threadIdx.x; ij < LL; ij += blockDim.x) atomicAdd(&acc[bucket[ij]], dbias[(long)h * LL + ij]);
  __syncthreads();
  for (int i = threadIdx.x; i < nb; i += blockDim.x) atomicAdd(dtable + i * H + h, acc[i]);
}

__global__ void ce_count_kernel(const long long* __restrict__ labels, int rows, float* __restrict__ inv_n) {
  __shared__ int red[4];
  int c = 0;
  for (int i = threadIdx.x; i < rows; i += blockDim.x) c += labels[i] != -100;
  for (int o = 32; o > 0; o >>= 1) c += __shfl_xor(c, o, 64);
  if ((threadIdx.x & 63) == 0) red[threadIdx.x >> 6] = c;
  __syncthreads();
  if (threadIdx.x == 0) {
    const int n = red[0] + red[1] + red[2] + red[3];
    inv_n[0] = n > 0 ? 1.f / (float)n : 0.f;
  }
}

template <typename T>
__global__ __launch_bounds__(256) void ce_fwd_kernel(T* __restrict__ logits, long ld, const long long* __restrict__ labels, int V,
                                                     const float* __restrict__ inv_n, float* __restrict__ loss_row, int write_grad) {
  constexpr int VEC = Vec16<T>::N;
  using VT = typename Vec16<T>::type;
  __shared__ float red[8];
  const long row = blockIdx.x;
  const int tid = threadIdx.x;
  T* x = logits + row * ld;
  const long long lab = labels[row];
  float m = -INFINITY, s = 0.f;
  for (int c = tid * VEC; c < V; c += 256 * VEC) {
    VT v = *reinterpret_cast<const VT*>(x + c);
    float mx = to_f32(v[0]);
#pragma unroll
    for (int u = 1; u < VEC; ++u) mx = fmaxf(mx, to_f32(v[u]));
    const float mn = fmaxf(m, mx);
    float a = 0.f;
#pragma unroll
    for (int u = 0; u < VEC; ++u) a += __expf(to_f32(v[u]) - mn);
    s = s * __expf(m - mn) + a;
    m = mn;
  }
  float wm = wave_max(m);
  float ws = wave_sum(m == -INFINITY ? 0.f : s * __expf(m - wm));
  if ((tid & 63) == 0) { red[tid >> 6] = wm; red[4 + (tid >> 6)] = ws; }
  __syncthreads();
  const float bm = fmaxf(fmaxf(red[0], red[1]), fmaxf(red[2], red[3]));
  float bs = 0.f;
#pragma unroll
  for (int w = 0; w < 4; ++w) bs += red[w] == -INFINITY ? 0.f : red[4 + w] * __expf(red[w] - bm);
  const float lse = bm + __logf(bs);
  const bool valid = lab != -100;
  if (tid == 0) loss_row[row] = valid ? (lse - to_f32(x[lab])) : 0.f;
  if (!write_grad) return;
  __syncthreads();
  const float g = valid ? inv_n[0] : 0.f;
  for (int c = tid * VEC; c < V; c += 256 * VEC) {
    VT v = *reinterpret_cast<const VT*>(x + c);
    VT o;
#pragma unroll
    for (int u = 0; u < VEC; ++u) {
      float pr = __expf(to_f32(v[u]) - lse);
      if (c + u == lab) pr -= 1.f;
      o[u] = from_f32<T>(pr * g);
    }
    *reinterpret_cast<VT*>(x + c) = o;
  }
}

template <typename T, int NIT>
__global__ __launch_bounds__(256) void ce_fwd_onepass_kernel(T* __restrict__ logits, long ld, const long long* __restrict__ labels, int V,
                                                             const float* __restrict__ inv_n, float* __restrict__ loss_row, int write_grad) {
  constexpr int VEC = Vec16<T>::N;
  using VT = typename Vec16<T>::type;
  __shared__ float red[8];
  __shared__ float xlab;
  const long row = blockIdx.x;
  const int tid = threadIdx.x;
  T* x = logits + row * ld;
  const long long lab = labels[row];
  VT v[NIT];
#pragma unroll
  for (int it = 0; it < NIT; ++it) {
    const int c = (it * 256 + tid) * VEC;
    if (c < V) v[it] = *reinterpret_cast<const VT*>(x + c);
  }
  float m = -INFINITY;
#pragma unroll
  for (int it = 0; it < NIT; ++it) {
    const int c = (it * 256 + tid) * VEC;
    if (c < V) {
#pragma unroll
      for (int u = 0; u < VEC; ++u) m = fmaxf(m, to_f32(v[it][u]));
    }
  }
  const float wm = wave_max(m);
  if ((tid & 63) == 0) red[tid >> 6] = wm;
  __syncthreads();
  const float bm = fmaxf(fmaxf(red[0], red[1]), fmaxf(red[2], red[3]));
  float sum = 0.f;
#pragma unroll
  for (int it = 0; it < NIT; ++it) {
    const int c = (it * 256 + tid) * VEC;
    if (c < V) {
#pragma unroll
      for (int u = 0; u < VEC; ++u) {
        sum += __expf(to_f32(v[it][u]) - bm);
        if (c + u == lab) xlab = to_f32(v[it][u]);
      }
    }
  }
  const float ws = wave_sum(sum);
  if ((tid & 63) == 0) red[4 + (tid >> 6)] = ws;
  __syncthreads();
  const float lse = bm + __logf(red[4] + red[5] + red[6] + red[7]);
  const bool valid = lab != -100;
  if (tid == 0) loss_row[row] = valid ? (lse - xlab) : 0.f;
  if (!write_grad) return;
  const float g = valid ? inv_n[0] : 0.f;
#pragma unroll
  for (int it = 0; it < NIT; ++it) {
    const int c = (it * 256 + tid) * VEC;
    if (c < V) {
      VT o;
#pragma unroll
      for (int u = 0; u < VEC; ++u) {
        float pr = __expf(to_f32(v[it][u]) - lse);
        if (c + u == lab) pr -= 1.f;
        o[u] = from_f32<T>(pr * g);
      }
      *reinterpret_cast<VT*>(x + c) = o;
    }
  }
}

__global__ void ce_reduce_kernel(const float* __restrict__ loss_row, int rows, const float* __restrict__ inv_n, float* __restrict__ loss) {
  __shared__ float red[4];
  float a = 0.f;
  for (int i = threadIdx.x; i < rows; i += blockDim.x) a += loss_row[i];
  a = wave_sum(a);
  if ((threadIdx.x & 63) == 0) red[threadIdx.x >> 6] = a;
  __syncthreads();
  if (threadIdx.x == 0) loss[0] = (red[0] + red[1] + red[2] + red[3]) * inv_n[0];
}

template <typename T>
__global__ __launch_bounds__(256) void im2col_kernel(const float* __restrict__ pix, T* __restrict__ out, int B, int Cin, int Himg, int P) {
  const int R = Himg / P;
  const int K = Cin * P * P;
  const long total = (long)B * R * R * K;
  for (long idx = (long)blockIdx.x * blockDim.x + threadIdx.x; idx < total; idx += (long)gridDim.x * blockDim.x) {
    const int k = idx % K;
    const long t = idx / K;
    const int px = k % P, py = (k / P) % P, c = k / (P * P);
    const int x = t % R, y = (t / R) % R;
    const long b = t / ((long)R * R);
    out[idx] = from_f32<T>(pix[((b * Cin + c) * Himg + (y * P + py)) * Himg + (x * P + px)]);
  }
}

template <typename T>
__global__ __launch_bounds__(256) void im2col4_kernel(const float* __restrict__ pix, T* __restrict__ out, int B, int Cin, int Himg, int ldo) {
  const int R = Himg / 4;
  const long npatch = (long)B * R * R;
  for (long t = (long)blockIdx.x * blockDim.x + threadIdx.x; t < npatch; t += (long)gridDim.x * blockDim.x) {
    const int x = t % R, y = (t / R) % R;
    const long b = t / ((long)R * R);
    T* o = out + t * ldo;
    for (int c = 0; c < Cin; ++c) {
      f32x4 v[4];
#pragma unroll
      for (int py = 0; py < 4; ++py) v[py] = *reinterpret_cast<const f32x4*>(pix + ((b * Cin + c) * Himg + (y * 4 + py)) * Himg + x * 4);
      if constexpr (sizeof(T) == 2) {
        *reinterpret_cast<bf16x8*>(o + c * 16) = bf16x8{(bf16_t)v[0][0], (bf16_t)v[0][1], (bf16_t)v[0][2], (bf16_t)v[0][3],
                                                        (bf16_t)v[1][0], (bf16_t)v[1][1], (bf16_t)v[1][2], (bf16_t)v[1][3]};
        *reinterpret_cast<bf16x8*>(o + c * 16 + 8) = bf16x8{(bf16_t)v[2][0], (bf16_t)v[2][1], (bf16_t)v[2][2], (bf16_t)v[2][3],
                                                            (bf16_t)v[3][0], (bf16_t)v[3][1], (bf16_t)v[3][2], (bf16_t)v[3][3]};
      } else {
#pragma unroll
        for (int py = 0; py < 4; ++py) *reinterpret_cast<f32x4*>(o + c * 16 + py * 4) = v[py];
      }
    }
    for (int k = Cin * 16; k < ldo; k += 8) {
      if constexpr (sizeof(T) == 2) *reinterpret_cast<bf16x8*>(o + k) = bf16x8{};
      else { *reinterpret_cast<f32x4*>(o + k) = f32x4{0.f, 0.f, 0.f, 0.f}; *reinterpret_cast<f32x4*>(o + k + 4) = f32x4{0.f, 0.f, 0.f, 0.f}; }
    }
  }
}

template <typename T>
__global__ __launch_bounds__(256) void merge_gather_kernel(const float* __restrict__ x, T* __restrict__ out, int B, int R, int C) {
  const int R2 = R / 2;
  const long total4 = (long)B * R2 * R2 * C;
  for (long g = (long)blockIdx.x * blockDim.x + threadIdx.x; g < total4; g += (long)gridDim.x * blockDim.x) {
    const int c4 = g % C;
    const long t = g / C;
    const int q = (c4 * 4) / C, c = (c4 * 4) % C;
    const int dy = q & 1, dx = q >> 1;
    const int x2 = t % R2, y2 = (t / R2) % R2;
    const long b = t / ((long)R2 * R2);
    const f32x4 v = *reinterpret_cast<const f32x4*>(x + ((b * R + (2 * y2 + dy)) * R + (2 * x2 + dx)) * C + c);
    T* o = out + t * 4L * C + c4 * 4;
    if constexpr (sizeof(T) == 2) *reinterpret_cast<bf16x4*>(o) = bf16x4{(bf16_t)v[0], (bf16_t)v[1], (bf16_t)v[2], (bf16_t)v[3]};
    else *reinterpret_cast<f32x4*>(o) = v;
  }
}
__global__ __launch_bounds__(256) void merge_scatter_kernel(const float* __restrict__ dm, float* __restrict__ dx, int B, int R, int C) {
  const int R2 = R / 2;
  const long total4 = (long)B * R2 * R2 * C;
  for (long g = (long)blockIdx.x * blockDim.x + threadIdx.x; g < total4; g += (long)gridDim.x * blockDim.x) {
    const int c4 = g % C;
    const long t = g / C;
    const int q = (c4 * 4) / C, c = (c4 * 4) % C;
    const int dy = q & 1, dxo = q >> 1;
    const int x2 = t % R2, y2 = (t / R2) % R2;
    const long b = t / ((long)R2 * R2);
    *reinterpret_cast<f32x4*>(dx + ((b * R + (2 * y2 + dy)) * R + (2 * x2 + dxo)) * C + c) =
        *reinterpret_cast<const f32x4*>(dm + t * 4L * C + c4 * 4);
  }
}

template <typename T>
// ... 99 lines not shown
  return KLAB_OK;
}

}

using namespace klab;

extern "C" int klab_cast_pack(const void* desc_dev, int ndesc, long total4, void* dst, int dtype, void* stream) {
  if (!desc_dev || !dst || ndesc <= 0) return KLAB_ERR_BADARG;
  hipStream_t s = (hipStream_t)stream;
  if (dtype == KLAB_BF16)
    hipLaunchKernelGGL(cast_pack_kernel<bf16_t>, dim3(stream_grid((total4 + 7) / 8)), dim3(256), 0, s, (const CastDesc*)desc_dev, ndesc, total4, (bf16_t*)dst);
  else
    hipLaunchKernelGGL(cast_pack_kernel<float>, dim3(stream_grid((total4 + 7) / 8)), dim3(256), 0, s, (const CastDesc*)desc_dev, ndesc, total4, (float*)dst);
  KLAB_LAUNCH_CHECK();
  return KLAB_OK;
}

extern "C" int klab_adam_step_range(const void* desc_dev, int ndesc, long begin4, long end4, const float* grads, float* m, float* v, void* arena,
                                    int dtype, float lr, float beta1, float beta2, float eps, float weight_decay, float bias_corr1,
                                    float bias_corr2, void* stream) {
  if (!desc_dev || ndesc <= 0 || !grads || !m || !v || !arena || bias_corr1 <= 0.f || bias_corr2 <= 0.f || begin4 < 0 || end4 < begin4)
    return KLAB_ERR_BADARG;
  if (end4 == begin4) return KLAB_OK;
  AdamHyper h{lr / bias_corr1, beta1, beta2, eps, weight_decay, 1.f / sqrtf(bias_corr2)};
  hipStream_t s = (hipStream_t)stream;
  constexpr int ADAM_GRID = 1024;
  constexpr int U = 4;
  long gl = ((end4 - begin4 + U - 1) / U + 255) / 256;
  const unsigned grid = (unsigned)(gl < 1 ? 1 : (gl > ADAM_GRID ? ADAM_GRID : gl));
  if (dtype == KLAB_BF16)
    hipLaunchKernelGGL((adam_step_kernel<bf16_t, U>), dim3(grid), dim3(256), 0, s, (const AdamDesc*)desc_dev, ndesc, begin4, end4, grads, m, v,
                       (bf16_t*)arena, h);
  else
    hipLaunchKernelGGL((adam_step_kernel<float, U>), dim3(grid), dim3(256), 0, s, (const AdamDesc*)desc_dev, ndesc, begin4, end4, grads, m, v,
                       (float*)arena, h);
  KLAB_LAUNCH_CHECK();
  return KLAB_OK;
}
extern "C" int klab_adam_step(const void* desc_dev, int ndesc, long total4, const float* grads, float* m, float* v, void* arena, int dtype,
                              float lr, float beta1, float beta2, float eps, float weight_decay, float bias_corr1, float bias_corr2,
                              void* stream) {
  return klab_adam_step_range(desc_dev, ndesc, 0, total4, grads, m, v, arena, dtype, lr, beta1, beta2, eps, weight_decay, bias_corr1, bias_corr2,
                              stream);
}

extern "C" int klab_embed_fwd(const long long* ids, int shift_right, int L, int start_id, int pad_id, const float* table, int vocab,
                              float* out, int rows, int d, float drop_p, const uint32_t* seed_dev, uint32_t tag, int* err_flag,
                              void* stream) {
  if (!ids || !table || !out || (d & 3)) return KLAB_ERR_BADARG;
  if (rows <= 0) return KLAB_OK;
  hipLaunchKernelGGL(embed_fwd_kernel, dim3(stream_grid((long)rows * 64)), dim3(256), 0, (hipStream_t)stream, ids, shift_right, L, start_id,
                     pad_id, table, vocab, out, rows, d, drop_p, seed_dev, tag, err_flag);
  KLAB_LAUNCH_CHECK();
  return KLAB_OK;
}

extern "C" int klab_embed_bwd(const long long* ids, int shift_right, int L, int start_id, int pad_id, const float* dh, float* dtable,
                              int vocab, int rows, int d, float drop_p, const uint32_t* seed_dev, uint32_t tag, void* stream) {
  if (!ids || !dh || !dtable) return KLAB_ERR_BADARG;
  if (rows <= 0) return KLAB_OK;
  hipLaunchKernelGGL(embed_bwd_kernel, dim3(stream_grid((long)rows * 64)), dim3(256), 0, (hipStream_t)stream, ids, shift_right, L, start_id,
                     pad_id, dh, dtable, vocab, rows, d, drop_p, seed_dev, tag);
  KLAB_LAUNCH_CHECK();
  return KLAB_OK;
}

extern "C" int klab_relbias_fwd(const float* table, const int* bucket, float* bias, int heads, int Lq, int Lk, void* stream) {
  if (!table || !bucket || !bias) return KLAB_ERR_BADARG;
  const long tot = (long)heads * Lq * Lk;
  hipLaunchKernelGGL(relbias_fwd_kernel, dim3((unsigned)((tot + 255) / 256)), dim3(256), 0, (hipStream_t)stream, table, bucket, bias, heads, Lq * Lk);
  KLAB_LAUNCH_CHECK();
  return KLAB_OK;
}

extern "C" int klab_relbias_bwd(const float* dbias, const int* bucket, float* dtable, int heads, int Lq, int Lk, int nbuckets, void* stream) {
  if (!dbias || !bucket || !dtable) return KLAB_ERR_BADARG;
  if (nbuckets > 64) return KLAB_ERR_UNSUPPORTED;
  hipLaunchKernelGGL(relbias_bwd_kernel, dim3(heads), dim3(256), 0, (hipStream_t)stream, dbias, bucket, dtable, heads, Lq * Lk, nbuckets);
  KLAB_LAUNCH_CHECK();
  return KLAB_OK;
}

extern "C" int klab_ce_count(const long long* labels, int rows, float* inv_n, void* stream) {
  if (!labels || !inv_n || rows <= 0) return KLAB_ERR_BADARG;
  hipLaunchKernelGGL(ce_count_kernel, dim3(1), dim3(256), 0, (hipStream_t)stream, labels, rows, inv_n);
  KLAB_LAUNCH_CHECK();
  return KLAB_OK;
}

extern "C" int klab_ce_fwd(void* logits, long ld, int dtype, const long long* labels, int rows, int V, float* inv_n, float* loss_row,
                           float* loss, int write_grad, void* stream) {
  if (!logits || !labels || !inv_n || !loss_row || !loss) return KLAB_ERR_BADARG;
  const int vec = dtype == KLAB_BF16 ? 8 : 4;
  if (V % vec || ld % vec) return KLAB_ERR_UNSUPPORTED;
  hipStream_t s = (hipStream_t)stream;
  if (!(write_grad & 2)) {
    hipLaunchKernelGGL(ce_count_kernel, dim3(1), dim3(256), 0, s, labels, rows, inv_n);
    KLAB_LAUNCH_CHECK();
  }
  write_grad &= 1;
  if (dtype == KLAB_BF16 && V <= 256 * 8 * 16 && V > 256 * 8 * 8)
    hipLaunchKernelGGL((ce_fwd_onepass_kernel<bf16_t, 16>), dim3(rows), dim3(256), 0, s, (bf16_t*)logits, ld, labels, V, inv_n, loss_row, write_grad);
  else if (dtype == KLAB_BF16 && V <= 256 * 8 * 8)
    hipLaunchKernelGGL((ce_fwd_onepass_kernel<bf16_t, 8>), dim3(rows), dim3(256), 0, s, (bf16_t*)logits, ld, labels, V, inv_n, loss_row, write_grad);
  else if (dtype == KLAB_BF16)
    hipLaunchKernelGGL(ce_fwd_kernel<bf16_t>, dim3(rows), dim3(256), 0, s, (bf16_t*)logits, ld, labels, V, inv_n, loss_row, write_grad);
  else
    hipLaunchKernelGGL(ce_fwd_kernel<float>, dim3(rows), dim3(256), 0, s, (float*)logits, ld, labels, V, inv_n, loss_row, write_grad);
  KLAB_LAUNCH_CHECK();
  hipLaunchKernelGGL(ce_reduce_kernel, dim3(1), dim3(256), 0, s, loss_row, rows, inv_n, loss);
  KLAB_LAUNCH_CHECK();
  return KLAB_OK;
}

extern "C" int klab_im2col_patch(const float* pixels, void* out, int dtype, int B, int Cin, int Himg, int P, void* stream) {
  if (!pixels || !out || Himg % P) return KLAB_ERR_BADARG;
  const long total = (long)B * (Himg / P) * (Himg / P) * Cin * P * P;
  hipStream_t s = (hipStream_t)stream;
  if (dtype == KLAB_BF16) hipLaunchKernelGGL(im2col_kernel<bf16_t>, dim3(stream_grid(total)), dim3(256), 0, s, pixels, (bf16_t*)out, B, Cin, Himg, P);
  else hipLaunchKernelGGL(im2col_kernel<float>, dim3(stream_grid(total)), dim3(256), 0, s, pixels, (float*)out, B, Cin, Himg, P);
  KLAB_LAUNCH_CHECK();
  return KLAB_OK;
}

extern "C" int klab_im2col_patch_ld(const float* pixels, void* out, int dtype, int B, int Cin, int Himg, int P, int ldo, void* stream) {
  if (!pixels || !out || Himg % P || ldo < Cin * P * P) return KLAB_ERR_BADARG;
  if (P != 4 || (Himg & 3) || (ldo & 7) || ((uintptr_t)pixels & 15) || ((uintptr_t)out & 15)) {
    if (ldo == Cin * P * P) return klab_im2col_patch(pixels, out, dtype, B, Cin, Himg, P, stream);
    return KLAB_ERR_UNSUPPORTED;
  }
  const long npatch = (long)B * (Himg / 4) * (Himg / 4);
  hipStream_t s = (hipStream_t)stream;
  if (dtype == KLAB_BF16) hipLaunchKernelGGL(im2col4_kernel<bf16_t>, dim3(stream_grid(npatch)), dim3(256), 0, s, pixels, (bf16_t*)out, B, Cin, Himg, ldo);
  else hipLaunchKernelGGL(im2col4_kernel<float>, dim3(stream_grid(npatch)), dim3(256), 0, s, pixels, (float*)out, B, Cin, Himg, ldo);
  KLAB_LAUNCH_CHECK();
  return KLAB_OK;
}

extern "C" int klab_merge_gather(const float* x, void* out, int dtype, int B, int R, int C, void* stream) {
  if (!x || !out || (R & 1) || (C & 3)) return KLAB_ERR_BADARG;
  const long total4 = (long)B * (R / 2) * (R / 2) * C;
  hipStream_t s = (hipStream_t)stream;
  if (dtype == KLAB_BF16) hipLaunchKernelGGL(merge_gather_kernel<bf16_t>, dim3(stream_grid(total4)), dim3(256), 0, s, x, (bf16_t*)out, B, R, C);
  else hipLaunchKernelGGL(merge_gather_kernel<float>, dim3(stream_grid(total4)), dim3(256), 0, s, x, (float*)out, B, R, C);
  KLAB_LAUNCH_CHECK();
  return KLAB_OK;
}

extern "C" int klab_merge_scatter(const float* dmerged, float* dx, int B, int R, int C, void* stream) {
  if (!dmerged || !dx || (R & 1) || (C & 3)) return KLAB_ERR_BADARG;
  const long total4 = (long)B * (R / 2) * (R / 2) * C;
  hipLaunchKernelGGL(merge_scatter_kernel, dim3(stream_grid(total4)), dim3(256), 0, (hipStream_t)stream, dmerged, dx, B, R, C);
  KLAB_LAUNCH_CHECK();
  return KLAB_OK;
}

extern "C" int klab_colsum(const void* dy, long ld, int dtype, int M, int N, float* out, void* stream) {
  if (!dy || !out) return KLAB_ERR_BADARG;
  int gy = (M + 255) / 256;
  gy = gy < 1 ? 1 : (gy > 256 ? 256 : gy);
  dim3 grid((N + 63) / 64, gy);
  hipStream_t s = (hipStream_t)stream;
  if (dtype == KLAB_BF16 && (N & 7) == 0 && (ld & 7) == 0 && ((uintptr_t)dy & 15) == 0) {
    int g8 = (M + 127) / 128;
    const int want = 2048 / (int)grid.x;
    g8 = g8 < 1 ? 1 : (g8 > want ? (want < 1 ? 1 : want) : g8);
    hipLaunchKernelGGL(colsum8_kernel, dim3(grid.x, g8), dim3(256), 0, s, (const bf16_t*)dy, ld, M, N, out);
    KLAB_LAUNCH_CHECK();
    return KLAB_OK;
  }
  if (dtype == KLAB_BF16) hipLaunchKernelGGL(colsum_kernel<bf16_t>, grid, dim3(256), 0, s, (const bf16_t*)dy, ld, M, N, out);
  else hipLaunchKernelGGL(colsum_kernel<float>, grid, dim3(256), 0, s, (const float*)dy, ld, M, N, out);
  KLAB_LAUNCH_CHECK();
  return KLAB_OK;
}

extern "C" int klab_convert(const float* x, void* y, int dtype, long n, float scale, void* stream) {
  if (!x || !y || (n & 3)) return KLAB_ERR_BADARG;
  hipStream_t s = (hipStream_t)stream;
  if (dtype == KLAB_BF16) hipLaunchKernelGGL(convert_kernel<bf16_t>, dim3(stream_grid(n / 4)), dim3(256), 0, s, x, (bf16_t*)y, n / 4, scale);
  else hipLaunchKernelGGL(convert_kernel<float>, dim3(stream_grid(n / 4)), dim3(256), 0, s, x, (float*)y, n / 4, scale);
  KLAB_LAUNCH_CHECK();
  return KLAB_OK;
}

extern "C" int klab_add_f32(float* y, const float* x, long n, void* stream) {
  if (!x || !y || (n & 3)) return KLAB_ERR_BADARG;
  hipLaunchKernelGGL(add_f32_kernel, dim3(stream_grid(n / 4)), dim3(256), 0, (hipStream_t)stream, y, x, n / 4);
  KLAB_LAUNCH_CHECK();
  return KLAB_OK;
}

__global__ __launch_bounds__(256) void gelu_fwd_q8_kernel(const bf16_t* __restrict__ x, bf16_t* __restrict__ y, unsigned char* __restrict__ y8,
                                                          float* __restrict__ yscale, int rows, int F) {
  constexpr int MAXV = 8;
// ... 61 lines not shown
```

klab_multimodalmodel_amd/ops.py:

```python
import ctypes as C

import torch

from . import _lib as L


def _seed_ptr(seed):
    return None if seed is None else seed.data_ptr()


def _gemm_args(A, B, C_out, *, M, N, K, a_kmajor=True, b_kmajor=True, lda=None, ldb=None, ldc=None, alpha=1.0,
               alpha_dev=None, bias=None, act=L.ACT_NONE, aux=None, aux_mode=L.AUX_NONE, aux_scale=1.0, residual=None,
               drop_p=0.0, seed=None, tag=0, accumulate=False, atomic_ok=False, name_tag=0):
    a = L.GemmArgs()
    a.atomic_ok, a.name_tag = int(atomic_ok), name_tag
    a.M, a.N, a.K = M, N, K
    a.dtype = L.dtype_code(A.dtype)
    assert B.dtype == A.dtype
    a.A, a.lda, a.a_kmajor = A.data_ptr(), (lda if lda is not None else A.stride(0)), int(a_kmajor)
    a.B, a.ldb, a.b_kmajor = B.data_ptr(), (ldb if ldb is not None else B.stride(0)), int(b_kmajor)
    a.C, a.ldc, a.c_dtype = C_out.data_ptr(), (ldc if ldc is not None else C_out.stride(0)), L.dtype_code(C_out.dtype)
    a.accumulate = int(accumulate)
    a.alpha = alpha
    a.alpha_dev = L.ptr(alpha_dev)
# ... 331 lines not shown
    a = _swin_args(qkv, ctx, bias, logit_scale, lse, B, R, w, shift, H, C, bias_table, v_bias)
    if mfma and (w * w > 64 or R % w):
        nbytes = lib.klab_swin_attn_bwd_ws_bytes(a.dtype, B, R, w, H, C)
        if nbytes:
            ws = torch.empty(nbytes, dtype=torch.uint8, device=qkv.device)
            a.bwd_ws, a.bwd_ws_bytes = ws.data_ptr(), nbytes
    L.check(lib.klab_swin_attn_fwd(C_byref(a), L.stream_ptr()), "klab_swin_attn_fwd")


def swin_attn_bwd(qkv, ctx, bias, logit_scale, lse, dctx, dqkv, dbias=None, dlogit_scale=None, *, B, R, w, shift, H, C, mfma=True,
                  bias_table=None, dbias_table=None, v_bias=None, dv_bias=None):
    import torch
    lib = L.load()
    a = _swin_args(qkv, ctx, bias, logit_scale, lse, B, R, w, shift, H, C, bias_table, v_bias, dv_bias)
    a.dbias_table = L.ptr(dbias_table)
    a.dctx, a.dqkv, a.dbias, a.dlogit_scale = dctx.data_ptr(), dqkv.data_ptr(), L.ptr(dbias), L.ptr(dlogit_scale)
    nbytes = lib.klab_swin_attn_bwd_ws_bytes(a.dtype, B, R, w, H, C) if mfma else 0
    if nbytes:
        ws = torch.empty(nbytes, dtype=torch.uint8, device=qkv.device)
        a.bwd_ws, a.bwd_ws_bytes = ws.data_ptr(), nbytes
    L.check(lib.klab_swin_attn_bwd(C_byref(a), L.stream_ptr()), "klab_swin_attn_bwd")


C_byref = C.byref


def swin_cpb_bias(coords, index, w0, b0, w2, table, bias, hidden=None, *, n, heads):
    lib = L.load()
    L.check(lib.klab_swin_cpb_bias(coords.data_ptr(), index.data_ptr(), w0.data_ptr(), b0.data_ptr(), w2.data_ptr(),
                                   table.data_ptr(), L.ptr(hidden), bias.data_ptr(), coords.shape[0], n, heads, w0.shape[0],
                                   L.stream_ptr()), "klab_swin_cpb_bias")


def swin_cpb_table(coords, w0, b0, w2, table, bias_table, hidden=None, *, heads):
    lib = L.load()
    L.check(lib.klab_swin_cpb_table(coords.data_ptr(), w0.data_ptr(), b0.data_ptr(), w2.data_ptr(), table.data_ptr(), L.ptr(hidden),
                                    bias_table.data_ptr(), coords.shape[0], heads, w0.shape[0], L.stream_ptr()), "klab_swin_cpb_table")


def swin_cpb_table_bwd(dbias_table, bias_table, coords, hidden, w2, dtable, dw0, db0, dw2, *, heads):
    lib = L.load()
    L.check(lib.klab_swin_cpb_table_bwd(dbias_table.data_ptr(), bias_table.data_ptr(), coords.data_ptr(), hidden.data_ptr(), w2.data_ptr(),
                                        dtable.data_ptr(), dw0.data_ptr(), db0.data_ptr(), dw2.data_ptr(), coords.shape[0], heads,
                                        hidden.shape[1], L.stream_ptr()), "klab_swin_cpb_table_bwd")


def swin_cpb_bias_bwd(dbias, bias, index, coords, hidden, w2, dtable, dw0, db0, dw2, *, heads, n=None, ntab=None, nhidden=None,
                      dtable_zeroed=False, w0=None):
    lib = L.load()
    ntab = coords.shape[0] if ntab is None else ntab
    nhidden = hidden.shape[1] if nhidden is None else nhidden
    n = int(round(index.numel() ** 0.5)) if n is None else n
    L.check(lib.klab_swin_cpb_bias_bwd_pz(dbias.data_ptr(), bias.data_ptr(), index.data_ptr(), coords.data_ptr(), hidden.data_ptr(),
                                          L.ptr(w0), w2.data_ptr(), dtable.data_ptr(), dw0.data_ptr(), db0.data_ptr(), dw2.data_ptr(),
                                          ntab, n, heads, nhidden, 1 if dtable_zeroed else 0, L.stream_ptr()),
            "klab_swin_cpb_bias_bwd_pz")


def ce_fwd(logits, labels, inv_n, loss_row, loss, write_grad=True):
    lib = L.load()
    rows, V = logits.shape
    L.check(lib.klab_ce_fwd(logits.data_ptr(), logits.stride(0), L.dtype_code(logits.dtype), labels.data_ptr(), rows, V,
                            inv_n.data_ptr(), loss_row.data_ptr(), loss.data_ptr(), int(write_grad), L.stream_ptr()), "klab_ce_fwd")


def ce_count(labels, inv_n):
    lib = L.load()
    L.check(lib.klab_ce_count(labels.data_ptr(), labels.numel(), inv_n.data_ptr(), L.stream_ptr()), "klab_ce_count")


def ce_wsum(labels, weights, inv_w):
    lib = L.load()
    L.check(lib.klab_ce_wsum(labels.data_ptr(), L.ptr(weights), labels.numel(), inv_w.data_ptr(), L.stream_ptr()), "klab_ce_wsum")


def ce_fwd_opts(logits, labels, weights, inv_w, loss_row, loss, *, eps=0.0, z=0.0, write_grad=True):
    lib = L.load()
    rows, V = logits.shape
    L.check(lib.klab_ce_fwd_opts(logits.data_ptr(), logits.stride(0), L.dtype_code(logits.dtype), labels.data_ptr(), L.ptr(weights), rows, V,
                                 float(eps), float(z), inv_w.data_ptr(), loss_row.data_ptr(), loss.data_ptr(), int(write_grad),
                                 L.stream_ptr()), "klab_ce_fwd_opts")


def embed_fwd(ids, table, out, *, shift_right=False, L_seq=1, start_id=0, pad_id=0, drop_p=0.0, seed=None, tag=0, err=None):
    lib = L.load()
    rows, d = out.shape
    L.check(lib.klab_embed_fwd(ids.data_ptr(), int(shift_right), L_seq, start_id, pad_id, table.data_ptr(), table.shape[0],
                               out.data_ptr(), rows, d, drop_p, _seed_ptr(seed), tag, L.ptr(err), L.stream_ptr()), "klab_embed_fwd")


def embed_bwd(ids, dh, dtable, *, shift_right=False, L_seq=1, start_id=0, pad_id=0, drop_p=0.0, seed=None, tag=0):
    lib = L.load()
    rows, d = dh.shape
    L.check(lib.klab_embed_bwd(ids.data_ptr(), int(shift_right), L_seq, start_id, pad_id, dh.data_ptr(), dtable.data_ptr(),
                               dtable.shape[0], rows, d, drop_p, _seed_ptr(seed), tag, L.stream_ptr()), "klab_embed_bwd")


def relbias_fwd(table, bucket, bias):
    lib = L.load()
    H, Lq, Lk = bias.shape
    L.check(lib.klab_relbias_fwd(table.data_ptr(), bucket.data_ptr(), bias.data_ptr(), H, Lq, Lk, L.stream_ptr()), "klab_relbias_fwd")


def relbias_bwd(dbias, bucket, dtable):
    lib = L.load()
    H, Lq, Lk = dbias.shape
    L.check(lib.klab_relbias_bwd(dbias.data_ptr(), bucket.data_ptr(), dtable.data_ptr(), H, Lq, Lk, dtable.shape[0],
                                 L.stream_ptr()), "klab_relbias_bwd")


def im2col_patch(pixels, out, P):
    lib = L.load()
    B, Cin, Himg, _ = pixels.shape
    ldo = out.shape[-1]
    if ldo == Cin * P * P:
        L.check(lib.klab_im2col_patch(pixels.data_ptr(), out.data_ptr(), L.dtype_code(out.dtype), B, Cin, Himg, P, L.stream_ptr()),
                "klab_im2col_patch")
    else:
        L.check(lib.klab_im2col_patch_ld(pixels.data_ptr(), out.data_ptr(), L.dtype_code(out.dtype), B, Cin, Himg, P, ldo, L.stream_ptr()),
                "klab_im2col_patch_ld")


def merge_gather(x, out, *, B, R, C):
    lib = L.load()
    L.check(lib.klab_merge_gather(x.data_ptr(), out.data_ptr(), L.dtype_code(out.dtype), B, R, C, L.stream_ptr()), "klab_merge_gather")


def merge_scatter(dm, dx, *, B, R, C):
    lib = L.load()
    L.check(lib.klab_merge_scatter(dm.data_ptr(), dx.data_ptr(), B, R, C, L.stream_ptr()), "klab_merge_scatter")


def colsum(dy, out):
    lib = L.load()
    M, N = dy.shape
    L.check(lib.klab_colsum(dy.data_ptr(), dy.stride(0), L.dtype_code(dy.dtype), M, N, out.data_ptr(), L.stream_ptr()), "klab_colsum")


def convert(x, y, scale=1.0):
    lib = L.load()
    L.check(lib.klab_convert(x.data_ptr(), y.data_ptr(), L.dtype_code(y.dtype), x.numel(), scale, L.stream_ptr()), "klab_convert")


def add_f32(y, x):
    lib = L.load()
    assert y.dtype == x.dtype == torch.float32 and y.numel() == x.numel()
    L.check(lib.klab_add_f32(y.data_ptr(), x.data_ptr(), y.numel(), L.stream_ptr()), "klab_add_f32")


def cast_pack(desc, total4, dst):
    lib = L.load()
    assert desc.dtype == torch.int64 and desc.dim() == 2 and desc.shape[1] == 3 and desc.is_contiguous()
    L.check(lib.klab_cast_pack(desc.data_ptr(), desc.shape[0], int(total4), dst.data_ptr(), L.dtype_code(dst.dtype), L.stream_ptr()),
            "klab_cast_pack")


def quant_fp8_arena(desc, total_rows, arena_bf16, arena_fp8, scales):
    lib = L.load()
    assert desc.dtype == torch.int64 and desc.dim() == 2 and desc.shape[1] == 4 and desc.is_contiguous()
    L.check(lib.klab_quant_fp8_arena(desc.data_ptr(), desc.shape[0], int(total_rows), arena_bf16.data_ptr(), arena_fp8.data_ptr(),
                                     scales.data_ptr(), L.stream_ptr()), "klab_quant_fp8_arena")


def adam_step(desc, total4, grads, m, v, arena, *, lr, beta1=0.9, beta2=0.999, eps=1e-8, weight_decay=0.0, bias_corr1=1.0, bias_corr2=1.0,
              begin4=None, end4=None):
    lib = L.load()
    assert desc.dtype == torch.int64 and desc.dim() == 2 and desc.shape[1] == 4 and desc.is_contiguous()
    hyper = (float(lr), float(beta1), float(beta2), float(eps), float(weight_decay), float(bias_corr1), float(bias_corr2))
    if begin4 is None and end4 is None:
        L.check(lib.klab_adam_step(desc.data_ptr(), desc.shape[0], int(total4), grads.data_ptr(), m.data_ptr(), v.data_ptr(),
                                   arena.data_ptr(), L.dtype_code(arena.dtype), *hyper, L.stream_ptr()), "klab_adam_step")
    else:
        L.check(lib.klab_adam_step_range(desc.data_ptr(), desc.shape[0], int(begin4), int(end4), grads.data_ptr(), m.data_ptr(),
                                         v.data_ptr(), arena.data_ptr(), L.dtype_code(arena.dtype), *hyper, L.stream_ptr()),
                "klab_adam_step_range")


def adamw_step(desc, group_of, groups, grads, m, v, arena, *, begin4=0, end4=None, total4=None):
    lib = L.load()
    assert desc.dtype == torch.int64 and desc.dim() == 2 and desc.shape[1] == 4 and desc.is_contiguous()
    assert group_of.dtype == torch.int32 and group_of.is_contiguous() and group_of.numel() == desc.shape[0] and group_of.device == desc.device
    end4 = total4 if end4 is None else end4
    L.check(lib.klab_adamw_step_range(desc.data_ptr(), desc.shape[0], group_of.data_ptr(), L.adamw_groups(groups), len(groups), int(begin4),
                                      int(end4), grads.data_ptr(), m.data_ptr(), v.data_ptr(), arena.data_ptr(), L.dtype_code(arena.dtype),
                                      L.stream_ptr()), "klab_adamw_step_range")


def ema_update(desc, ema, w, *, begin4=0, end4=None, total4=None):
    lib = L.load()
    assert desc.dtype == torch.int64 and desc.dim() == 2 and desc.shape[1] == 4 and desc.is_contiguous()
    assert ema.dtype == torch.float32 and ema.is_contiguous()
# ... 237 lines not shown
```

Before: 12070 samples/s.

## Fuse stack-tail reductions, buffer clears into CE, and step-entry copies into single kernels

Adds a stack_tail kernel that merges the RMSNorm column-partial reduction, the deferred dbias slab reduction and the relative-bias backward into one launch, with a fallback to the separate kernels when the shapes are unsupported. The cross-entropy forward kernels gain an optional grid-wide zero-fill of a buffer, so a separate memset can be dropped. When graphs are off, the seed step and the src/tgt id copies are folded into one step_entry kernel. The loss reduce loop is also unrolled. The aim is fewer small launches and less launch overhead in a latency-bound step, at the cost of more complex kernels and an extra clear pass inside the CE kernels.

```diff
diff --git a/include/klab_mm.h b/include/klab_mm.h
--- a/include/klab_mm.h
+++ b/include/klab_mm.h
@@ -183,12 +183,18 @@
 int klab_relbias_fwd(const float* table, const int* bucket, float* bias, int heads, int Lq, int Lk, void* stream);
 int klab_relbias_bwd(const float* dbias, const int* bucket, float* dtable, int heads, int Lq, int Lk, int nbuckets,
                      void* stream);
+int klab_stack_tail(const void* ds_ws, int dtype, int nslab, float* dbias, const int* bucket, float* dtable, int heads, int Lq, int Lk,
+                    int nbuckets, const float* part, long call_stride, int nparts, int d, float* const* dst_dev, int ncalls, void* stream);
 int klab_ce_count(const long long* labels, int rows, float* inv_n, void* stream);
 int klab_ce_fwd(void* logits, long ld, int dtype, const long long* labels, int rows, int V, float* inv_n, float* loss_row,
                 float* loss, int write_grad, void* stream);
 int klab_ce_wsum(const long long* labels, const float* weights, int rows, float* inv_w, void* stream);
 int klab_ce_fwd_opts(void* logits, long ld, int dtype, const long long* labels, const float* weights, int rows, int V, float eps, float z,
                      float* inv_w, float* loss_row, float* loss, int write_grad, void* stream);
+int klab_ce_fwd_clear(void* logits, long ld, int dtype, const long long* labels, int rows, int V, float* inv_n, float* loss_row,
+                      float* loss, int write_grad, float* clear, long clear_n, void* stream);
+int klab_ce_fwd_opts_clear(void* logits, long ld, int dtype, const long long* labels, const float* weights, int rows, int V, float eps,
+                           float z, float* inv_w, float* loss_row, float* loss, int write_grad, float* clear, long clear_n, void* stream);
 int klab_im2col_patch(const float* pixels, void* out, int dtype, int B, int Cin, int Himg, int P, void* stream);
 int klab_im2col_patch_ld(const float* pixels, void* out, int dtype, int B, int Cin, int Himg, int P, int ldo, void* stream);
 int klab_merge_gather(const float* x, void* out, int dtype, int B, int R, int C, void* stream);
diff --git a/klab_multimodalmodel_amd/_lib.py b/klab_multimodalmodel_amd/_lib.py
--- a/klab_multimodalmodel_amd/_lib.py
+++ b/klab_multimodalmodel_amd/_lib.py
@@ -186,10 +186,13 @@
     "klab_embed_bwd": [vp, i32, i32, i32, i32, vp, vp, i32, i32, i32, f32, vp, u32, vp],
     "klab_relbias_fwd": [vp, vp, vp, i32, i32, i32, vp],
     "klab_relbias_bwd": [vp, vp, vp, i32, i32, i32, i32, vp],
+    "klab_stack_tail": [vp, i32, i32, vp, vp, vp, i32, i32, i32, i32, vp, i64, i32, i32, vp, i32, vp],
     "klab_ce_fwd": [vp, i64, i32, vp, i32, i32, vp, vp, vp, i32, vp],
     "klab_ce_count": [vp, i32, vp, vp],
     "klab_ce_wsum": [vp, vp, i32, vp, vp],
     "klab_ce_fwd_opts": [vp, i64, i32, vp, vp, i32, i32, f32, f32, vp, vp, vp, i32, vp],
+    "klab_ce_fwd_clear": [vp, i64, i32, vp, i32, i32, vp, vp, vp, i32, vp, i64, vp],
+    "klab_ce_fwd_opts_clear": [vp, i64, i32, vp, vp, i32, i32, f32, f32, vp, vp, vp, i32, vp, i64, vp],
     "klab_engine_set_loss_options": [vp, f32, f32, vp],
     "klab_engine_set_captions": [vp, i32],
     "klab_im2col_patch": [vp, vp, i32, i32, i32, i32, i32, vp],
diff --git a/klab_multimodalmodel_amd/csrc/ce_opts.hip b/klab_multimodalmodel_amd/csrc/ce_opts.hip
--- a/klab_multimodalmodel_amd/csrc/ce_opts.hip
+++ b/klab_multimodalmodel_amd/csrc/ce_opts.hip
@@ -49,7 +49,7 @@
 template <typename T, bool SX>
 __global__ __launch_bounds__(256) void ce_opts_kernel(T* __restrict__ logits, long ld, const long long* __restrict__ labels,
                                                       const float* __restrict__ weights, int V, CeOpts o, const float* __restrict__ inv_w,
-                                                      float* __restrict__ loss_row, int write_grad) {
+                                                      float* __restrict__ loss_row, int write_grad, float* __restrict__ clear, long clear_n) {
   constexpr int VEC = Vec16<T>::N;
   using VT = typename Vec16<T>::type;
   __shared__ float red[12];
@@ -59,6 +59,7 @@
   const long long lab = labels[row];
   const bool valid = lab != -100;
   const float g = write_grad && valid ? (weights ? weights[row] : 1.f) * inv_w[0] : 0.f;
+  if (write_grad) grid_clear_f32(clear, clear_n);
   float m = -INFINITY, s = 0.f, sx = 0.f;
   for (int c = tid * VEC; c < V; c += 256 * VEC) {
     VT v = *reinterpret_cast<const VT*>(x + c);
@@ -109,7 +110,8 @@
 template <typename T, int NIT, bool SX>
 __global__ __launch_bounds__(256) void ce_opts_onepass_kernel(T* __restrict__ logits, long ld, const long long* __restrict__ labels,
                                                               const float* __restrict__ weights, int V, CeOpts o,
-                                                              const float* __restrict__ inv_w, float* __restrict__ loss_row, int write_grad) {
+                                                              const float* __restrict__ inv_w, float* __restrict__ loss_row, int write_grad,
+                                                              float* __restrict__ clear, long clear_n) {
   constexpr int VEC = Vec16<T>::N;
   using VT = typename Vec16<T>::type;
   __shared__ float red[12];
@@ -127,6 +129,7 @@
     if (c < V) v[it] = *reinterpret_cast<const VT*>(x + c);
   }
   const float g = write_grad && valid ? (weights ? weights[row] : 1.f) * inv_w[0] : 0.f;
+  if (write_grad) grid_clear_f32(clear, clear_n);
   float m = -INFINITY;
 #pragma unroll
   for (int it = 0; it < NIT; ++it) {
@@ -199,15 +202,15 @@
 
 template <bool SX>
 void launch_rows(void* logits, long ld, int dtype, const long long* labels, const float* weights, int rows, int V, const CeOpts& o,
-                 const float* inv_w, float* loss_row, int write_grad, hipStream_t s) {
+                 const float* inv_w, float* loss_row, int write_grad, float* clear, long clear_n, hipStream_t s) {
   if (dtype == KLAB_BF16 && V <= 256 * 8 * 16 && V > 256 * 8 * 8)
-    hipLaunchKernelGGL((ce_opts_onepass_kernel<bf16_t, 16, SX>), dim3(rows), dim3(256), 0, s, (bf16_t*)logits, ld, labels, weights, V, o, inv_w, loss_row, write_grad);
+    hipLaunchKernelGGL((ce_opts_onepass_kernel<bf16_t, 16, SX>), dim3(rows), dim3(256), 0, s, (bf16_t*)logits, ld, labels, weights, V, o, inv_w, loss_row, write_grad, clear, clear_n);
   else if (dtype == KLAB_BF16 && V <= 256 * 8 * 8)
-    hipLaunchKernelGGL((ce_opts_onepass_kernel<bf16_t, 8, SX>), dim3(rows), dim3(256), 0, s, (bf16_t*)logits, ld, labels, weights, V, o, inv_w, loss_row, write_grad);
+    hipLaunchKernelGGL((ce_opts_onepass_kernel<bf16_t, 8, SX>), dim3(rows), dim3(256), 0, s, (bf16_t*)logits, ld, labels, weights, V, o, inv_w, loss_row, write_grad, clear, clear_n);
   else if (dtype == KLAB_BF16)
-    hipLaunchKernelGGL((ce_opts_kernel<bf16_t, SX>), dim3(rows), dim3(256), 0, s, (bf16_t*)logits, ld, labels, weights, V, o, inv_w, loss_row, write_grad);
+    hipLaunchKernelGGL((ce_opts_kernel<bf16_t, SX>), dim3(rows), dim3(256), 0, s, (bf16_t*)logits, ld, labels, weights, V, o, inv_w, loss_row, write_grad, clear, clear_n);
   else
-    hipLaunchKernelGGL((ce_opts_kernel<float, SX>), dim3(rows), dim3(256), 0, s, (float*)logits, ld, labels, weights, V, o, inv_w, loss_row, write_grad);
+    hipLaunchKernelGGL((ce_opts_kernel<float, SX>), dim3(rows), dim3(256), 0, s, (float*)logits, ld, labels, weights, V, o, inv_w, loss_row, write_grad, clear, clear_n);
 }
 
 }
@@ -222,8 +225,8 @@
   return KLAB_OK;
 }
 
-extern "C" int klab_ce_fwd_opts(void* logits, long ld, int dtype, const long long* labels, const float* weights, int rows, int V, float eps,
-                                float z, float* inv_w, float* loss_row, float* loss, int write_grad, void* stream) {
+static int ce_fwd_opts_launch(void* logits, long ld, int dtype, const long long* labels, const float* weights, int rows, int V, float eps,
+                              float z, float* inv_w, float* loss_row, float* loss, int write_grad, float* clear, long clear_n, void* stream) {
   if (!logits || !labels || !inv_w || !loss_row || !loss || rows <= 0 || V <= 0) return KLAB_ERR_BADARG;
   if (!(eps >= 0.f && eps < 1.f) || !(z >= 0.f) || !isfinite(z)) return KLAB_ERR_BADARG;
   const int vec = dtype == KLAB_BF16 ? 8 : 4;
@@ -235,10 +238,22 @@
   }
   write_grad &= 1;
   const CeOpts o{1.f - eps, eps / (float)V, z};
-  if (eps != 0.f) launch_rows<true>(logits, ld, dtype, labels, weights, rows, V, o, inv_w, loss_row, write_grad, s);
-  else launch_rows<false>(logits, ld, dtype, labels, weights, rows, V, o, inv_w, loss_row, write_grad, s);
+  if (eps != 0.f) launch_rows<true>(logits, ld, dtype, labels, weights, rows, V, o, inv_w, loss_row, write_grad, clear, clear_n, s);
+  else launch_rows<false>(logits, ld, dtype, labels, weights, rows, V, o, inv_w, loss_row, write_grad, clear, clear_n, s);
   KLAB_LAUNCH_CHECK();
   hipLaunchKernelGGL(ce_wreduce_kernel, dim3(1), dim3(256), 0, s, loss_row, weights, rows, inv_w, loss);
   KLAB_LAUNCH_CHECK();
   return KLAB_OK;
 }
+
+extern "C" int klab_ce_fwd_opts(void* logits, long ld, int dtype, const long long* labels, const float* weights, int rows, int V, float eps,
+                                float z, float* inv_w, float* loss_row, float* loss, int write_grad, void* stream) {
+  return ce_fwd_opts_launch(logits, ld, dtype, labels, weights, rows, V, eps, z, inv_w, loss_row, loss, write_grad, nullptr, 0, stream);
+}
+
+extern "C" int klab_ce_fwd_opts_clear(void* logits, long ld, int dtype, const long long* labels, const float* weights, int rows, int V,
+                                      float eps, float z, float* inv_w, float* loss_row, float* loss, int write_grad, float* clear,
+                                      long clear_n, void* stream) {
+  if (clear_n < 0 || (clear_n > 0 && !clear)) return KLAB_ERR_BADARG;
+  return ce_fwd_opts_launch(logits, ld, dtype, labels, weights, rows, V, eps, z, inv_w, loss_row, loss, write_grad, clear, clear_n, stream);
+}
diff --git a/klab_multimodalmodel_amd/csrc/common.h b/klab_multimodalmodel_amd/csrc/common.h
--- a/klab_multimodalmodel_amd/csrc/common.h
+++ b/klab_multimodalmodel_amd/csrc/common.h
@@ -105,6 +105,18 @@
   return v;
 }
 
+__device__ __forceinline__ void grid_clear_f32(float* p, long n) {
+  if (!p || n <= 0) return;
+  long head = (long)(((16 - ((uintptr_t)p & 15)) & 15) >> 2);
+  if (head > n) head = n;
+  const long n4 = (n - head) >> 2, rest = n - head - n4 * 4;
+  f32x4* p4 = reinterpret_cast<f32x4*>(p + head);
+  const long t = (long)blockIdx.x * blockDim.x + threadIdx.x, step = (long)gridDim.x * blockDim.x;
+  for (long i = t; i < n4; i += step) p4[i] = f32x4{0.f, 0.f, 0.f, 0.f};
+  if (t < head) p[t] = 0.f;
+  if (t < rest) p[head + n4 * 4 + t] = 0.f;
+}
+
 __device__ __forceinline__ float gelu_erf(float x) { return 0.5f * x * (1.f + erff(x * 0.70710678118654752440f)); }
 __device__ __forceinline__ float erf_fast(float x) {
   const float ax = fabsf(x);
diff --git a/klab_multimodalmodel_amd/csrc/engine.cpp b/klab_multimodalmodel_amd/csrc/engine.cpp
--- a/klab_multimodalmodel_amd/csrc/engine.cpp
+++ b/klab_multimodalmodel_amd/csrc/engine.cpp
@@ -157,6 +157,7 @@
   bool seg1_zeroed = false;
   bool dbias_zeroed[2] = {false, false};
   bool denc_in_dxn = false;
+  bool dxn_cleared = false;
   float* loss_out = nullptr;
   float loss_eps = 0.f, loss_z = 0.f;
   const float* loss_w_armed = nullptr;
@@ -1055,12 +1056,18 @@
         e->bucket_ev_live[seg] = true;
     }
   }
-  if (part_ok && rms_calls) {
-    if (rms_calls != e->rms_ncalls[stk]) return KLAB_ERR_BADARG;
-    RC(klab_colpart_reduce(e->rms_part, e->rms_part_stride, klab_rmsnorm_part_rows(M), d, e->rms_dst_dev[stk], rms_calls, c.ws()));
-  }
-  if (deferred) RC(klab_dbias_reduce(e->ds_ws, c.dt, s.dbias, deferred * B, H, Lq, Lq, c.ws()));
-  RC(klab_relbias_bwd(s.dbias, s.bucket, G(L[0].relb), H, Lq, Lq, cfg.rel_buckets, c.ws()));
+  const bool parts = part_ok && rms_calls;
+  if (parts && rms_calls != e->rms_ncalls[stk]) return KLAB_ERR_BADARG;
+  const int trc = klab_stack_tail(deferred ? e->ds_ws : nullptr, c.dt, deferred * B, s.dbias, s.bucket, G(L[0].relb), H, Lq, Lq, cfg.rel_buckets,
+                                  parts ? e->rms_part : nullptr, e->rms_part_stride, parts ? klab_rmsnorm_part_rows(M) : 0, d,
+                                  parts ? e->rms_dst_dev[stk] : nullptr, parts ? rms_calls : 0, c.ws());
+  if (trc == KLAB_ERR_UNSUPPORTED) {
+    if (parts) RC(klab_colpart_reduce(e->rms_part, e->rms_part_stride, klab_rmsnorm_part_rows(M), d, e->rms_dst_dev[stk], rms_calls, c.ws()));
+    if (deferred) RC(klab_dbias_reduce(e->ds_ws, c.dt, s.dbias, deferred * B, H, Lq, Lq, c.ws()));
+    RC(klab_relbias_bwd(s.dbias, s.bucket, G(L[0].relb), H, Lq, Lq, cfg.rel_buckets, c.ws()));
+  } else {
+    RC(trc);
+  }
   *dh_out = dh_cur;
   return 0;
 }
@@ -1380,7 +1387,7 @@
     e->n_cast = n; e->cast_total4 = pre;
   }
   e->frozen_valid = false;
-  e->seg1_zeroed = e->dbias_zeroed[0] = e->dbias_zeroed[1] = e->denc_in_dxn = false;
+  e->seg1_zeroed = e->dbias_zeroed[0] = e->dbias_zeroed[1] = e->denc_in_dxn = e->dxn_cleared = false;
   e->bias_ready[0] = e->bias_ready[1] = e->bias_ready[2] = e->dec_embed_ready = e->inv_n_ready = e->kv_wgrad_done = false;
   e->wplan.valid = false;
   e->loss_out = nullptr;
@@ -1545,6 +1552,21 @@
   st[0] = x;
 }
 
+__global__ __launch_bounds__(256) void step_entry_kernel(const long long* __restrict__ src, long long* __restrict__ src_buf, int n_src,
+                                                         const long long* __restrict__ tgt, long long* __restrict__ tgt_buf, int n_tgt,
+                                                         uint32_t* st) {
+  const int t = blockIdx.x * 256 + threadIdx.x;
+  if (t < n_src) src_buf[t] = src[t];
+  else if (t < n_src + n_tgt) tgt_buf[t - n_src] = tgt[t - n_src];
+  if (t == 0) {
+    const uint32_t n = st[2] + 1;
+    st[2] = n;
+    uint32_t x = st[1] + 0x9E3779B1u * n;
+    x ^= x >> 16; x *= 0x85EBCA6Bu; x ^= x >> 13; x *= 0xC2B2AE35u; x ^= x >> 16;
+    st[0] = x;
+  }
+}
+
 inline hipStream_t enter_stream(klab_engine* e, hipStream_t caller, int& rc) {
   rc = 0;
   if (!e->use_graph || caller != nullptr) return caller;
@@ -1581,12 +1603,13 @@
   return (int)hipGraphLaunch(g.exec, s);
 }
 
-int forward_part_a(klab_engine* e, hipStream_t stream, float p, bool refresh_frozen, bool trainable_current, bool encoder_current = false) {
+int forward_part_a(klab_engine* e, hipStream_t stream, float p, bool refresh_frozen, bool trainable_current, bool encoder_current = false,
+                   bool seed_stepped = false) {
   Ctx c{e, stream, e->cfg.dtype, e->es};
   const klab_model_cfg& cfg = e->cfg;
   const float* pixels = e->pixels_cur;
   const long long *src_ids = e->src_buf, *tgt_ids = e->tgt_buf;
-  hipLaunchKernelGGL(seed_step_kernel, dim3(1), dim3(1), 0, c.s, e->seed_dev);
+  if (!seed_stepped) hipLaunchKernelGGL(seed_step_kernel, dim3(1), dim3(1), 0, c.s, e->seed_dev);
   if (e->n_cast && !trainable_current) RC(klab_cast_pack(e->cast_desc, e->n_cast, e->cast_total4, e->warena, c.dt, c.ws()));
   if (refresh_frozen || e->cfg.train_swin) {
     if (refresh_frozen && e->n_cast_frozen)
@@ -1748,8 +1771,11 @@
   } else {
     e->pixels_cur = pixels;
   }
-  RC((int)hipMemcpyAsync(e->src_buf, src_ids, (size_t)B * e->Ls * 8, hipMemcpyDeviceToDevice, c.s));
-  RC((int)hipMemcpyAsync(e->tgt_buf, tgt_ids, (size_t)e->Bd * e->Lt * 8, hipMemcpyDeviceToDevice, c.s));
+  const bool entry = !e->use_graph;
+  if (!entry) {
+    RC((int)hipMemcpyAsync(e->src_buf, src_ids, (size_t)B * e->Ls * 8, hipMemcpyDeviceToDevice, c.s));
+    RC((int)hipMemcpyAsync(e->tgt_buf, tgt_ids, (size_t)e->Bd * e->Lt * 8, hipMemcpyDeviceToDevice, c.s));
+  }
   const float* loss_w = nullptr;
   if (e->loss_w_armed) {
     const float* src_w = e->loss_w_armed;
@@ -1761,15 +1787,21 @@
     hipLaunchKernelGGL(seed_set_kernel, dim3(1), dim3(1), 0, c.s, e->seed_dev, seed);
     e->seed_base = seed; e->seed_set = true;
   }
+  if (entry) {
+    const int n_src = B * e->Ls, n_tgt = e->Bd * e->Lt;
+    hipLaunchKernelGGL(step_entry_kernel, dim3((unsigned)((n_src + n_tgt + 255) / 256)), dim3(256), 0, c.s, src_ids, e->src_buf, n_src, tgt_ids,
+                       e->tgt_buf, n_tgt, e->seed_dev);
+    KLAB_LAUNCH_CHECK();
+  }
   const bool tcur = (training & 4) && !e->use_graph;
   const bool ecur = (training & 8) && !(training & 1) && !want_grad && !e->use_graph && e->frozen_valid && !refresh_frozen;
   if (refresh_frozen) {
-    RC(forward_part_a(e, c.s, p, true, tcur));
+    RC(forward_part_a(e, c.s, p, true, tcur, false, entry));
     e->frozen_valid = true;
   } else if (ecur) {
-    RC(forward_part_a(e, c.s, p, false, true, true));
+    RC(forward_part_a(e, c.s, p, false, true, true, entry));
   } else {
-    RC(run_graphed(e, (training & 1) ? 1 : 0, c.s, [&]() { return forward_part_a(e, c.s, p, false, tcur); }));
+    RC(run_graphed(e, (training & 1) ? 1 : 0, c.s, [&]() { return forward_part_a(e, c.s, p, false, tcur, false, entry); }));
   }
   {
     const int Md = e->Bd * e->Lt, V = cfg.main.vocab;
@@ -1788,14 +1820,19 @@
     e->inv_n_ready = false;
     float* loss_dst = e->loss_out && !e->use_graph ? e->loss_out : e->loss;
     e->loss_out = nullptr;
+    const bool clear_dxn = want_grad && !e->use_graph && !e->denc_in_dxn;
+    e->dxn_cleared = clear_dxn;
+    float* const clr = clear_dxn ? e->dxn : nullptr;
+    const long clr_n = clear_dxn ? (long)Md * d : 0;
     if (!loss_w && e->loss_eps == 0.f && e->loss_z == 0.f) {
       RC(run_graphed(e, want_grad ? 3 : 2, c.s, [&]() {
-        return klab_ce_fwd(e->logits, V, c.dt, e->tgt_buf, Md, V, e->inv_n, e->loss_row, loss_dst, (want_grad ? 1 : 0) | (counted ? 2 : 0), c.ws());
+        return klab_ce_fwd_clear(e->logits, V, c.dt, e->tgt_buf, Md, V, e->inv_n, e->loss_row, loss_dst, (want_grad ? 1 : 0) | (counted ? 2 : 0),
+                                 clr, clr_n, c.ws());
       }));
     } else {
       RC(klab_ce_wsum(e->tgt_buf, loss_w, Md, e->inv_w, c.ws()));
-      RC(klab_ce_fwd_opts(e->logits, V, c.dt, e->tgt_buf, loss_w, Md, V, e->loss_eps, e->loss_z, e->inv_w, e->loss_row, loss_dst,
-                          (want_grad ? 1 : 0) | 2, c.ws()));
+      RC(klab_ce_fwd_opts_clear(e->logits, V, c.dt, e->tgt_buf, loss_w, Md, V, e->loss_eps, e->loss_z, e->inv_w, e->loss_row, loss_dst,
+                                (want_grad ? 1 : 0) | 2, clr, clr_n, c.ws()));
     }
   }
   return leave_stream(e, (hipStream_t)stream, xs);
@@ -2355,7 +2392,8 @@
       RC((int)hipMemsetAsync(Gm + e->seg_off[0], 0, (size_t)e->seg_len[0] * 4, c.s));
     }
     {
-      RC((int)hipMemsetAsync(e->dxn, 0, (size_t)Md * d * 4, c.s));
+      if (e->dxn_cleared && !e->use_graph) e->dxn_cleared = false;
+      else RC((int)hipMemsetAsync(e->dxn, 0, (size_t)Md * d * 4, c.s));
       klab_gemm_args g = G0(c, Md, d, V, e->logits, V, 1, woff(c, e->P[2][e->mi.head].warena_off), d, 0, e->dxn, d, KLAB_F32);
       g.alpha = alpha; g.alpha_dev = dloss_dev; g.accumulate = 1; g.atomic_ok = 1;
       RC(klab_gemm(&g, c.ws()));
@@ -2382,6 +2420,7 @@
   }
   if (segment == 1) {
     e->ev_next = 0;
+    e->dxn_cleared = false;
     if (!wgrad_write_plan_current(e)) { wgrad_write_plan(e); e->seg1_zeroed = false; }
     if (e->seg1_zeroed) e->seg1_zeroed = false;
     else if (e->wplan.any_store) RC(clear_planned(e, 1, 1, false, c.s));
diff --git a/klab_multimodalmodel_amd/csrc/misc.hip b/klab_multimodalmodel_amd/csrc/misc.hip
--- a/klab_multimodalmodel_amd/csrc/misc.hip
+++ b/klab_multimodalmodel_amd/csrc/misc.hip
@@ -181,6 +181,89 @@
   for (int i = threadIdx.x; i < nb; i += blockDim.x) atomicAdd(dtable + i * H + h, acc[i]);
 }
 
+constexpr int ST_ROWS = 2, ST_SLANES = 16;
+__global__ __launch_bounds__(256) void stack_tail_kernel(const bf16_t* __restrict__ ds, int nslab, float* __restrict__ dbias,
+                                                         const int* __restrict__ bucket, float* __restrict__ dtable, int H, int Lq, int Lk,
+                                                         int Lkp, int nb, int nbias, const float* __restrict__ part, long call_stride,
+                                                         int nparts, int d, float* const* __restrict__ dst, int dblocks) {
+  __shared__ float sm[ST_ROWS * ST_SLANES * 64];
+  __shared__ float acc[64];
+  __shared__ int met[64];
+  const int tid = threadIdx.x;
+  if ((int)blockIdx.x >= nbias) {
+    float(*red)[64] = reinterpret_cast<float(*)[64]>(sm);
+    const int j = blockIdx.x - nbias, bx = j % dblocks, by = j / dblocks;
+    const int col = bx * 64 + (tid & 63), rl = tid >> 6;
+    float a = 0.f;
+    if (col < d) {
+      const float* src = part + (long)by * call_stride + col;
+#pragma unroll 8
+      for (int b = rl; b < nparts; b += 4) a += src[(long)b * d];
+    }
+    red[rl][tid & 63] = a;
+    __syncthreads();
+    if (rl == 0 && col < d) dst[by][col] += (red[0][tid] + red[1][tid]) + (red[2][tid] + red[3][tid]);
+    return;
+  }
+  const int chunks = (Lq + ST_ROWS - 1) / ST_ROWS;
+  const int h = blockIdx.x / chunks, q0 = (blockIdx.x % chunks) * ST_ROWS;
+  if (tid < 64) { acc[tid] = 0.f; met[tid] = 0; }
+  {
+    const int r = tid >> 7, s = (tid >> 3) & (ST_SLANES - 1), k0 = (tid & 7) * 8, q = q0 + r;
+    float a[8];
+#pragma unroll
+    for (int u = 0; u < 8; ++u) a[u] = 0.f;
+    if (q < Lq && k0 < Lk) {
+      const long slab = (long)H * Lq * Lkp;
+      const bf16_t* p = ds + ((long)h * Lq + q) * Lkp + k0;
+      if (k0 + 8 <= Lk) {
+#pragma unroll 8
+        for (int b = s; b < nslab; b += ST_SLANES) {
+          const bf16x8 v = *reinterpret_cast<const bf16x8*>(p + (long)b * slab);
+#pragma unroll
+          for (int u = 0; u < 8; ++u) a[u] += (float)v[u];
+        }
+      } else {
+        const int nv = Lk - k0;
+        for (int b = s; b < nslab; b += 4 * ST_SLANES) {
+          bf16_t t[4][8];
+#pragma unroll
+          for (int j = 0; j < 4; ++j)
+#pragma unroll
+            for (int u = 0; u < 8; ++u)
+              if (u < nv && b + j * ST_SLANES < nslab) t[j][u] = p[(long)(b + j * ST_SLANES) * slab + u];
+#pragma unroll
+          for (int j = 0; j < 4; ++j)
+#pragma unroll
+            for (int u = 0; u < 8; ++u)
+              if (u < nv && b + j * ST_SLANES < nslab) a[u] += (float)t[j][u];
+        }
+      }
+    }
+#pragma unroll
+    for (int u = 0; u < 8; ++u) sm[(r * ST_SLANES + s) * 64 + k0 + u] = a[u];
+  }
+  __syncthreads();
+  if (tid < ST_ROWS * 64) {
+    const int r = tid >> 6, k = tid & 63, q = q0 + r;
+    if (q < Lq && k < Lk) {
+      float t = 0.f;
+#pragma unroll
+      for (int s = 0; s < ST_SLANES; ++s) t += sm[(r * ST_SLANES + s) * 64 + k];
+      const long idx = ((long)h * Lq + q) * Lk + k;
+      const float v = dbias[idx] + t;
+      dbias[idx] = v;
+      const int bk = bucket[q * Lk + k];
+      if ((unsigned)bk < 64u) {
+        atomicAdd(&acc[bk], v);
+        met[bk] = 1;
+      }
+    }
+  }
+  __syncthreads();
+  if (tid < nb && met[tid]) atomicAdd(dtable + tid * H + h, acc[tid]);
+}
+
 __global__ void ce_count_kernel(const long long* __restrict__ labels, int rows, float* __restrict__ inv_n) {
   __shared__ int red[4];
   int c = 0;
@@ -196,7 +279,8 @@
 
 template <typename T>
 __global__ __launch_bounds__(256) void ce_fwd_kernel(T* __restrict__ logits, long ld, const long long* __restrict__ labels, int V,
-                                                     const float* __restrict__ inv_n, float* __restrict__ loss_row, int write_grad) {
+                                                     const float* __restrict__ inv_n, float* __restrict__ loss_row, int write_grad,
+                                                     float* __restrict__ clear, long clear_n) {
   constexpr int VEC = Vec16<T>::N;
   using VT = typename Vec16<T>::type;
   __shared__ float red[8];
@@ -204,6 +288,7 @@
   const int tid = threadIdx.x;
   T* x = logits + row * ld;
   const long long lab = labels[row];
+  if (write_grad) grid_clear_f32(clear, clear_n);
   float m = -INFINITY, s = 0.f;
   for (int c = tid * VEC; c < V; c += 256 * VEC) {
     VT v = *reinterpret_cast<const VT*>(x + c);
@@ -246,7 +331,8 @@
 
 template <typename T, int NIT>
 __global__ __launch_bounds__(256) void ce_fwd_onepass_kernel(T* __restrict__ logits, long ld, const long long* __restrict__ labels, int V,
-                                                             const float* __restrict__ inv_n, float* __restrict__ loss_row, int write_grad) {
+                                                             const float* __restrict__ inv_n, float* __restrict__ loss_row, int write_grad,
+                                                             float* __restrict__ clear, long clear_n) {
   constexpr int VEC = Vec16<T>::N;
   using VT = typename Vec16<T>::type;
   __shared__ float red[8];
@@ -261,6 +347,7 @@
     const int c = (it * 256 + tid) * VEC;
     if (c < V) v[it] = *reinterpret_cast<const VT*>(x + c);
   }
+  if (write_grad) grid_clear_f32(clear, clear_n);
   float m = -INFINITY;
 #pragma unroll
   for (int it = 0; it < NIT; ++it) {
@@ -313,7 +400,17 @@
 __global__ void ce_reduce_kernel(const float* __restrict__ loss_row, int rows, const float* __restrict__ inv_n, float* __restrict__ loss) {
   __shared__ float red[4];
   float a = 0.f;
-  for (int i = threadIdx.x; i < rows; i += blockDim.x) a += loss_row[i];
+  for (int i0 = threadIdx.x; i0 < rows; i0 += 16 * (int)blockDim.x) {
+    float v[16];
+#pragma unroll
+    for (int u = 0; u < 16; ++u) {
+      const int i = i0 + u * (int)blockDim.x;
+      v[u] = i < rows ? loss_row[i] : 0.f;
+    }
+#pragma unroll
+    for (int u = 0; u < 16; ++u)
+      if (i0 + u * (int)blockDim.x < rows) a += v[u];
+  }
   a = wave_sum(a);
   if ((threadIdx.x & 63) == 0) red[threadIdx.x >> 6] = a;
   __syncthreads();
@@ -579,6 +676,21 @@
   return KLAB_OK;
 }
 
+extern "C" int klab_stack_tail(const void* ds_ws, int dtype, int nslab, float* dbias, const int* bucket, float* dtable, int heads, int Lq, int Lk,
+                               int nbuckets, const float* part, long call_stride, int nparts, int d, float* const* dst_dev, int ncalls,
+                               void* stream) {
+  if (!dbias || !bucket || !dtable || heads <= 0 || Lq <= 0 || Lk <= 0 || nbuckets <= 0 || nslab < 0 || ncalls < 0) return KLAB_ERR_BADARG;
+  if (nslab > 0 && (!ds_ws || dtype != KLAB_BF16)) return KLAB_ERR_BADARG;
+  if (ncalls > 0 && (!part || !dst_dev || nparts <= 0 || d <= 0)) return KLAB_ERR_BADARG;
+  const int Lkp = (Lk + 31) & ~31;
+  if (Lkp > 64 || nbuckets > 64 || ((uintptr_t)ds_ws & 15)) return KLAB_ERR_UNSUPPORTED;
+  const int nbias = heads * ((Lq + ST_ROWS - 1) / ST_ROWS), dblocks = ncalls > 0 ? (d + 63) / 64 : 0;
+  hipLaunchKernelGGL(stack_tail_kernel, dim3((unsigned)(nbias + dblocks * ncalls)), dim3(256), 0, (hipStream_t)stream, (const bf16_t*)ds_ws, nslab,
+                     dbias, bucket, dtable, heads, Lq, Lk, Lkp, nbuckets, nbias, part, call_stride, nparts, d, dst_dev, dblocks);
+  KLAB_LAUNCH_CHECK();
+  return KLAB_OK;
+}
+
 extern "C" int klab_ce_count(const long long* labels, int rows, float* inv_n, void* stream) {
   if (!labels || !inv_n || rows <= 0) return KLAB_ERR_BADARG;
   hipLaunchKernelGGL(ce_count_kernel, dim3(1), dim3(256), 0, (hipStream_t)stream, labels, rows, inv_n);
@@ -586,8 +698,8 @@
   return KLAB_OK;
 }
 
-extern "C" int klab_ce_fwd(void* logits, long ld, int dtype, const long long* labels, int rows, int V, float* inv_n, float* loss_row,
-                           float* loss, int write_grad, void* stream) {
+static int ce_fwd_launch(void* logits, long ld, int dtype, const long long* labels, int rows, int V, float* inv_n, float* loss_row,
+                         float* loss, int write_grad, float* clear, long clear_n, void* stream) {
   if (!logits || !labels || !inv_n || !loss_row || !loss) return KLAB_ERR_BADARG;
   const int vec = dtype == KLAB_BF16 ? 8 : 4;
   if (V % vec || ld % vec) return KLAB_ERR_UNSUPPORTED;
@@ -598,17 +710,28 @@
   }
   write_grad &= 1;
   if (dtype == KLAB_BF16 && V <= 256 * 8 * 16 && V > 256 * 8 * 8)
-    hipLaunchKernelGGL((ce_fwd_onepass_kernel<bf16_t, 16>), dim3(rows), dim3(256), 0, s, (bf16_t*)logits, ld, labels, V, inv_n, loss_row, write_grad);
+    hipLaunchKernelGGL((ce_fwd_onepass_kernel<bf16_t, 16>), dim3(rows), dim3(256), 0, s, (bf16_t*)logits, ld, labels, V, inv_n, loss_row, write_grad, clear, clear_n);
   else if (dtype == KLAB_BF16 && V <= 256 * 8 * 8)
-    hipLaunchKernelGGL((ce_fwd_onepass_kernel<bf16_t, 8>), dim3(rows), dim3(256), 0, s, (bf16_t*)logits, ld, labels, V, inv_n, loss_row, write_grad);
+    hipLaunchKernelGGL((ce_fwd_onepass_kernel<bf16_t, 8>), dim3(rows), dim3(256), 0, s, (bf16_t*)logits, ld, labels, V, inv_n, loss_row, write_grad, clear, clear_n);
   else if (dtype == KLAB_BF16)
-    hipLaunchKernelGGL(ce_fwd_kernel<bf16_t>, dim3(rows), dim3(256), 0, s, (bf16_t*)logits, ld, labels, V, inv_n, loss_row, write_grad);
+    hipLaunchKernelGGL(ce_fwd_kernel<bf16_t>, dim3(rows), dim3(256), 0, s, (bf16_t*)logits, ld, labels, V, inv_n, loss_row, write_grad, clear, clear_n);
   else
-    hipLaunchKernelGGL(ce_fwd_kernel<float>, dim3(rows), dim3(256), 0, s, (float*)logits, ld, labels, V, inv_n, loss_row, write_grad);
+    hipLaunchKernelGGL(ce_fwd_kernel<float>, dim3(rows), dim3(256), 0, s, (float*)logits, ld, labels, V, inv_n, loss_row, write_grad, clear, clear_n);
   KLAB_LAUNCH_CHECK();
   hipLaunchKernelGGL(ce_reduce_kernel, dim3(1), dim3(256), 0, s, loss_row, rows, inv_n, loss);
   KLAB_LAUNCH_CHECK();
   return KLAB_OK;
+}
+
+extern "C" int klab_ce_fwd(void* logits, long ld, int dtype, const long long* labels, int rows, int V, float* inv_n, float* loss_row,
+                           float* loss, int write_grad, void* stream) {
+  return ce_fwd_launch(logits, ld, dtype, labels, rows, V, inv_n, loss_row, loss, write_grad, nullptr, 0, stream);
+}
+
+extern "C" int klab_ce_fwd_clear(void* logits, long ld, int dtype, const long long* labels, int rows, int V, float* inv_n, float* loss_row,
+                                 float* loss, int write_grad, float* clear, long clear_n, void* stream) {
+  if (clear_n < 0 || (clear_n > 0 && !clear)) return KLAB_ERR_BADARG;
+  return ce_fwd_launch(logits, ld, dtype, labels, rows, V, inv_n, loss_row, loss, write_grad, clear, clear_n, stream);
 }
 
 extern "C" int klab_im2col_patch(const float* pixels, void* out, int dtype, int B, int Cin, int Himg, int P, void* stream) {
diff --git a/klab_multimodalmodel_amd/ops.py b/klab_multimodalmodel_amd/ops.py
--- a/klab_multimodalmodel_amd/ops.py
+++ b/klab_multimodalmodel_amd/ops.py
@@ -437,6 +437,22 @@
                                  L.stream_ptr()), "klab_ce_fwd_opts")
 
 
+def ce_fwd_clear(logits, labels, inv_n, loss_row, loss, clear, clear_n, write_grad=True):
+    lib = L.load()
+    rows, V = logits.shape
+    L.check(lib.klab_ce_fwd_clear(logits.data_ptr(), logits.stride(0), L.dtype_code(logits.dtype), labels.data_ptr(), rows, V,
+                                  inv_n.data_ptr(), loss_row.data_ptr(), loss.data_ptr(), int(write_grad), L.ptr(clear), int(clear_n),
+                                  L.stream_ptr()), "klab_ce_fwd_clear")
+
+
+def ce_fwd_opts_clear(logits, labels, weights, inv_w, loss_row, loss, clear, clear_n, *, eps=0.0, z=0.0, write_grad=True):
+    lib = L.load()
+    rows, V = logits.shape
+    L.check(lib.klab_ce_fwd_opts_clear(logits.data_ptr(), logits.stride(0), L.dtype_code(logits.dtype), labels.data_ptr(), L.ptr(weights), rows,
+                                       V, float(eps), float(z), inv_w.data_ptr(), loss_row.data_ptr(), loss.data_ptr(), int(write_grad),
+                                       L.ptr(clear), int(clear_n), L.stream_ptr()), "klab_ce_fwd_opts_clear")
+
+
 def embed_fwd(ids, table, out, *, shift_right=False, L_seq=1, start_id=0, pad_id=0, drop_p=0.0, seed=None, tag=0, err=None):
     lib = L.load()
     rows, d = out.shape
@@ -462,6 +478,16 @@
     H, Lq, Lk = dbias.shape
     L.check(lib.klab_relbias_bwd(dbias.data_ptr(), bucket.data_ptr(), dtable.data_ptr(), H, Lq, Lk, dtable.shape[0],
                                  L.stream_ptr()), "klab_relbias_bwd")
+
+
+def stack_tail(ds_ws, dbias, bucket, dtable, *, nslab, part=None, call_stride=0, nparts=0, d=0, dsts=()):
+    lib = L.load()
+    H, Lq, Lk_ = dbias.shape
+    table = torch.tensor([t.data_ptr() for t in dsts], dtype=torch.int64).to(dbias.device) if len(dsts) else None
+    L.check(lib.klab_stack_tail(L.ptr(ds_ws), L.BF16 if ds_ws is None else L.dtype_code(ds_ws.dtype), int(nslab), dbias.data_ptr(),
+                                bucket.data_ptr(), dtable.data_ptr(), H, Lq, Lk_, dtable.shape[0], L.ptr(part), int(call_stride), int(nparts),
+                                int(d), L.ptr(table), len(dsts), L.stream_ptr()), "klab_stack_tail")
+    return table
 
 
 def im2col_patch(pixels, out, P):
```

Result: no change. 12150 samples/s (median of 6 runs) (+0.6%).
